# punch-mission/regularizepsf

Measured on AMD Instinct MI355X. Metric: corrected Mpixels/sec + fraction of HBM roofline, 4096^2 image / 256-patch, higher is better.
Workload: dtype f32; 1 GPU; 4096x4096 starfield, 256x256 patches, 1089 patches (whole image on one GPU), coma PSF grid -> Gaussian target, alpha=3 eps=0.1, pad symmetric; patch=256, patches=1089, device= (gfx950:sramecc+:xnack-), compute_units=256, resident=image, output and packed transfer kernel in HBM before the timed region, in_flight=1, frames_in_rotation=1, sync=none (one rank)

## Files before the change

### __graft_entry__.py

```python

from __future__ import annotations

import pathlib
import shutil
import subprocess
import sys

ROOT = pathlib.Path(__file__).resolve().parent
sys.path.insert(0, str(ROOT))


def build() -> None:
    from regularizepsf_amd import build as hip_build

    hip_build.build()
    cores = [ROOT / "regularizepsf_amd" / "csrc" / n for n in ("rpsf_core.hpp", "rpsf_core2.hpp", "rpsf_core3.hpp", "rpsf_plan3.hpp", "rpsf_lattice.hpp", "rpsf_core_builder.hpp", "rpsf_core_builder_sub.hpp", "rpsf_core_builder_wide.hpp", "rpsf_core_cleanup.hpp", "rpsf_core_cleanup_wide.hpp", "rpsf_core_stars.hpp", "rpsf_core_stars_deblend.hpp", "rpsf_core_stars_shape.hpp", "rpsf_core_stars_photometry.hpp", "rpsf_core_stars_refine.hpp", "rpsf_core_stars_fit.hpp", "rpsf_core_stars_fit_weighted.hpp", "rpsf_core_stars_fitpos.hpp", "rpsf_core_stars_render.hpp", "rpsf_core_stars_mesh.hpp", "rpsf_core_saturation.hpp", "rpsf_core_saturation_batch.hpp", "rpsf_core_convert.hpp", "rpsf_core_scale.hpp")]
    for stem in ("emu", "emu2", "emu3", "emu_lattice", "emu_builder", "emu_builder_sub", "emu_builder_wide", "emu_cleanup_wide", "emu_stars", "emu_deblend", "emu_shapes", "emu_photometry", "emu_refine", "emu_fit", "emu_fit_weighted", "emu_fitpos", "emu_render", "emu_stars_mesh", "emu_cleanup", "emu_saturation", "emu_saturation_batch", "emu_mask", "emu_convert", "emu_scale"):
        emu_src = ROOT / "tests" / "emu" / f"{stem}.cpp"
        emu_out = ROOT / "tests" / "emu" / f"lib{stem}.so"
        if not emu_out.exists() or emu_out.stat().st_mtime < max(emu_src.stat().st_mtime, *(c.stat().st_mtime for c in cores)):
            clang = "/opt/rocm/lib/llvm/bin/clang++"
            if not pathlib.Path(clang).exists():
                clang = shutil.which("clang++") or shutil.which("hipcc")
            subprocess.run([clang, "-std=c++20", "-O1", "-shared", "-fPIC", "-o", str(emu_out), str(emu_src)], check=True)
    import regularizepsf_amd
    from regularizepsf_amd import _native

    _native.lib()


def smoke() -> None:
    import numpy as np

    import regularizepsf_amd as rp
    from oracle import regpsf_oracle as orc

    for h, w, n in ((512, 512, 256), (512, 512, 32)):
        coords, k = orc.synthetic_transfer(h, w, n, alpha=3.0, epsilon=0.1)
        image = orc.starfield(h, w, seed=7)
        out = rp.ArrayPSFTransform(rp.IndexedCube(coords, k)).apply(image)
        ref = orc.apply_transfer(image, coords, k)
        d = out - ref
        rel_max = float(np.abs(d).max() / np.abs(ref).max())
        rel_l2 = float(np.linalg.norm(d) / np.linalg.norm(ref))
        print(f"smoke: {h}x{w}/N={n}, {len(coords)} patches: max|d|/max|ref| = {rel_max:.3e}, rel-L2 = {rel_l2:.3e}")
        if not (rel_max <= 1e-5 and rel_l2 <= 1e-5):
            msg = "smoke parity failed"
            raise AssertionError(msg)


if __name__ == "__main__":
    build()
    if "--smoke" in sys.argv:
        smoke()
```

### include/rpsf.h

```cpp
#ifndef RPSF_H
#define RPSF_H

#include <stddef.h>
#include <stdint.h>

#ifdef __cplusplus
extern "C" {
#endif

#define RPSF_OK 0
#define RPSF_E_BADARG (-1)
#define RPSF_E_UNSUPPORTED (-2)
#define RPSF_E_HIP (-3)
#define RPSF_E_NOMEM (-4)
#define RPSF_E_RCCL (-5)
#define RPSF_E_STATE (-6)

#define RPSF_PAD_CONSTANT 0
#define RPSF_PAD_SYMMETRIC 1
#define RPSF_PAD_REFLECT 2
#define RPSF_PAD_EDGE 3
#define RPSF_PAD_WRAP 4

typedef struct rpsf_plan rpsf_plan;

const char* rpsf_last_error(void);
int rpsf_device_count(int* count);
int rpsf_device_info(int device, int* compute_units, char* name, size_t name_len);

int rpsf_plan_create(rpsf_plan** out, int device, int patch_size, int n_patches, const int32_t* coords_rc);
void rpsf_plan_destroy(rpsf_plan* plan);

int rpsf_plan_set_transfer(rpsf_plan* plan, const float* k_c64_host);
int rpsf_plan_set_transfer_device(rpsf_plan* plan, const void* k_c64_device);
int rpsf_plan_set_transfer_spectra_device(rpsf_plan* plan, const void* s_c64_dev, const void* t_c64_dev, double alpha, double epsilon);
int rpsf_plan_set_overlap_mode(rpsf_plan* plan, int mode);
int rpsf_plan_set_sweep_regions(rpsf_plan* plan, int target_regions);
enum {
  RPSF_OPT_PERSIST = 1,
  RPSF_OPT_FUSE = 2,
  RPSF_OPT_K_CACHED = 3,
  RPSF_OPT_PLANE_NT = 4,
  RPSF_OPT_HOST_BANDS = 5,
  RPSF_OPT_STREAM_GROUP = 6,
  RPSF_OPT_STREAM_DEPTH = 7,
  RPSF_OPT_DEBUG_ORPHAN = 8,
  RPSF_OPT_HEAD_KPREFETCH = 9,
  RPSF_OPT_SAT_GROUP = 10
};
int rpsf_plan_set_option(rpsf_plan* plan, int option, int value);
int rpsf_plan_sweep_info(const rpsf_plan* plan, int* regions, long* jobs, long* patch_slots, int* slabs_per_phase);
int rpsf_plan_host_bands(const rpsf_plan* plan, int* bands);
int rpsf_plan_set_stagger(rpsf_plan* plan, int microseconds);
int rpsf_plan_set_reserved_cus(rpsf_plan* plan, int cus);
int rpsf_plan_set_cu_mask(rpsf_plan* plan, const uint32_t* mask, int words);
int rpsf_stream_create(int device, const uint32_t* mask, int words, void** stream);
int rpsf_stream_destroy(void* stream);
int rpsf_plan_set_image_prefetch(rpsf_plan* plan, int on);
int rpsf_plan_debug_stamps(rpsf_plan* plan, unsigned long long* host, size_t count);
int rpsf_plan_transfer_bytes(const rpsf_plan* plan, size_t* bytes);

typedef struct rpsf_geometry {
  int height, width;
  int pad_mode;
  float pad_value;
  int origin_row, origin_col;
  int image_row0, image_rows, ld_image;
  int out_row0, out_rows, ld_out;
} rpsf_geometry;

int rpsf_apply(rpsf_plan* plan, const float* image_host, int height, int width, int pad_mode, float pad_value,
               float* out_host);
int rpsf_apply_host(rpsf_plan* plan, const void* image_host, int image_is_f64, int height, int width, int pad_mode,
                    float pad_value, void* out_host, int out_is_f64);
int rpsf_apply_host_saturated(rpsf_plan* plan, const void* image_host, int image_is_f64, int height, int width, int pad_mode,
                              double threshold, int dilation, int neighborhood_width, void* out_host, int out_is_f64);
int rpsf_apply_frames_host_saturated(rpsf_plan* plan, const void* const* images_host, int image_is_f64, int n_frames, int height,
                                     int width, int pad_mode, double threshold, int dilation, int neighborhood_width,
                                     void* const* outs_host, int out_is_f64);
int rpsf_apply_device_saturated(rpsf_plan* plan, const void* image_dev, void* out_dev, int height, int width, int pad_mode,
                                double threshold, int dilation, int neighborhood_width, void* stream, size_t* n_masked_or_null);
int rpsf_apply_host_saturated_device(rpsf_plan* plan, const void* image_host, int image_is_f64, int height, int width, int pad_mode,
                                     double threshold, int dilation, int neighborhood_width, void* out_host, int out_is_f64);
int rpsf_saturation_kernel_ms(rpsf_plan* plan, double ms[5]);
int rpsf_saturation_fill_device(rpsf_plan* plan, const float* image_host, int height, int width, int pad_mode, double threshold,
                                int dilation, int neighborhood_width, int reverse_groups, float* padded_host, uint8_t* mask_host,
                                int* n_groups_or_null);
int rpsf_apply_batch_device_saturated(rpsf_plan* plan, const void* images_dev, void* outs_dev, int n_frames, size_t image_stride,
                                      size_t out_stride, int height, int width, int pad_mode, double threshold, int dilation,
                                      int neighborhood_width, void* stream, size_t* n_masked_per_frame_or_null);
int rpsf_apply_frames_host_saturated_device(rpsf_plan* plan, const void* const* images_host, int image_is_f64, int n_frames, int height,
                                            int width, int pad_mode, double threshold, int dilation, int neighborhood_width,
                                            void* const* outs_host, int out_is_f64);
int rpsf_saturation_batch_info(rpsf_plan* plan, int info[4]);
int rpsf_saturation_fill_batch_device(rpsf_plan* plan, const float* images_host, int n_frames, int height, int width, int pad_mode,
                                      double threshold, int dilation, int neighborhood_width, int order, float* padded_host,
                                      uint8_t* masks_host, int* groups_per_frame_or_null);
int rpsf_apply_device(rpsf_plan* plan, const void* image_dev, void* out_dev, const rpsf_geometry* geom, void* stream);
int rpsf_apply_device_timed(rpsf_plan* plan, const void* image_dev, void* out_dev, const rpsf_geometry* geom,
                            int iters, float* total_ms, float* kernel_ms);
int rpsf_apply_device_loop_ms(rpsf_plan* plan, const void* image_dev, void* out_dev, const rpsf_geometry* geom, int iters,
// ... 254 lines not shown
```

### regularizepsf_amd/_native.py

```python

from __future__ import annotations

import ctypes
import pathlib
from ctypes import POINTER, c_char_p, c_double, c_float, c_int, c_size_t, c_void_p

import numpy as np

import os

LIB_PATH = pathlib.Path(os.environ.get("RPSF_LIB") or pathlib.Path(__file__).resolve().parent / "librpsf_hip.so")

PAD_MODES = {"constant": 0, "symmetric": 1, "reflect": 2, "edge": 3, "wrap": 4}
SUPPORTED_PATCH_SIZES = (16, 32, 64, 128, 256)

E_BADARG, E_UNSUPPORTED, E_HIP, E_NOMEM, E_RCCL, E_STATE = -1, -2, -3, -4, -5, -6


class NativeError(RuntimeError):

    def __init__(self, code: int, message: str) -> None:
        super().__init__(f"librpsf_hip error {code}: {message}")
        self.code = code

# ... 253 lines not shown
            msg = "upload larger than the device buffer"
            raise ValueError(msg)
        check(lib().rpsf_memcpy_h2d(self.device, c_void_p(self.ptr.value + offset_bytes), _ptr(a), a.nbytes))
        return self

    def download(self, shape, dtype=np.float32, offset_bytes: int = 0) -> np.ndarray:
        out = np.empty(shape, dtype)
        if offset_bytes + out.nbytes > self.nbytes:
            msg = "download larger than the device buffer"
            raise ValueError(msg)
        check(lib().rpsf_memcpy_d2h(self.device, _ptr(out), c_void_p(self.ptr.value + offset_bytes), out.nbytes))
        return out

    def at(self, offset_bytes: int) -> c_void_p:
        return c_void_p(self.ptr.value + offset_bytes)

    def free(self) -> None:
        if self.ptr is not None and self.ptr.value:
            lib().rpsf_dev_free(self.device, self.ptr)
            self.ptr = None

    def __del__(self) -> None:
        try:
            self.free()
        except Exception:
            pass


class Plan:

    def __init__(self, patch_size: int, coordinates, device: int = 0) -> None:
        coords = np.ascontiguousarray(np.asarray(coordinates, dtype=np.int64).reshape(-1, 2).astype(np.int32))
        self.patch_size, self.n_patches, self.device = int(patch_size), len(coords), device
        self._handle = c_void_p()
        check(lib().rpsf_plan_create(ctypes.byref(self._handle), device, self.patch_size, self.n_patches, _ptr(coords)))

    def set_transfer(self, kernel: np.ndarray) -> None:
        k = np.ascontiguousarray(kernel, dtype=np.complex64)
        if k.shape != (self.n_patches, self.patch_size, self.patch_size):
            msg = f"transfer kernel has shape {k.shape}, expected {(self.n_patches, self.patch_size, self.patch_size)}"
            raise ValueError(msg)
        check(lib().rpsf_plan_set_transfer(self._handle, _ptr(k)))

    def set_transfer_device(self, ptr: c_void_p) -> None:
        check(lib().rpsf_plan_set_transfer_device(self._handle, ptr))

    def set_transfer_spectra_device(self, s_ptr: c_void_p, t_ptr: c_void_p, alpha: float, epsilon: float) -> None:
        check(lib().rpsf_plan_set_transfer_spectra_device(self._handle, s_ptr, t_ptr, float(alpha), float(epsilon)))

    def set_overlap_mode(self, mode: str) -> None:
        check(lib().rpsf_plan_set_overlap_mode(self._handle, {"auto": 0, "atomic": 1, "planes": 2, "direct": 3, "sweep": 4}[mode]))

    OPTIONS = {"persist": 1, "fuse": 2, "k_cached": 3, "plane_nt": 4, "host_bands": 5, "stream_group": 6, "stream_depth": 7, "debug_orphan": 8,
               "head_kprefetch": 9, "sat_group": 10}

    def set_option(self, name: str, value: int) -> None:
        check(lib().rpsf_plan_set_option(self._handle, self.OPTIONS[name], int(value)))

    def set_sweep_regions(self, target_regions: int) -> None:
        check(lib().rpsf_plan_set_sweep_regions(self._handle, int(target_regions)))

    def sweep_info(self) -> dict:
        regions, slabs = c_int(0), c_int(0)
        jobs, slots = ctypes.c_long(0), ctypes.c_long(0)
        check(lib().rpsf_plan_sweep_info(self._handle, ctypes.byref(regions), ctypes.byref(jobs), ctypes.byref(slots), ctypes.byref(slabs)))
        return {"regions": regions.value, "jobs": jobs.value, "patch_slots": slots.value, "slabs_per_phase": slabs.value}

    def host_bands(self) -> int:
        n = c_int(0)
        check(lib().rpsf_plan_host_bands(self._handle, ctypes.byref(n)))
        return n.value

    def debug_stamps(self) -> np.ndarray:
        out = np.zeros((self.n_patches, 16), np.uint64)
        check(lib().rpsf_plan_debug_stamps(self._handle, _ptr(out), out.size))
        return out

    def set_stagger(self, microseconds: int) -> None:
        check(lib().rpsf_plan_set_stagger(self._handle, int(microseconds)))

    def set_image_prefetch(self, on: bool) -> None:
        check(lib().rpsf_plan_set_image_prefetch(self._handle, 1 if on else 0))

    def set_reserved_cus(self, cus: int) -> None:
        check(lib().rpsf_plan_set_reserved_cus(self._handle, int(cus)))

    def set_cu_mask(self, mask: np.ndarray) -> None:
        m = np.ascontiguousarray(mask, dtype=np.uint32)
        check(lib().rpsf_plan_set_cu_mask(self._handle, _ptr(m), m.size))

    @property
    def transfer_bytes(self) -> int:
        n = c_size_t(0)
        check(lib().rpsf_plan_transfer_bytes(self._handle, ctypes.byref(n)))
        return n.value

    @property
    def stream(self) -> c_void_p:
        return c_void_p(lib().rpsf_plan_stream(self._handle))

    def apply(self, image: np.ndarray, pad_mode: int, pad_value: float = 0.0) -> np.ndarray:
        img = np.ascontiguousarray(image, dtype=np.float32)
        out = np.empty_like(img)
        check(lib().rpsf_apply(self._handle, _ptr(img), img.shape[0], img.shape[1], pad_mode, pad_value, _ptr(out)))
        return out

    def apply_host(self, image: np.ndarray, pad_mode: int, pad_value: float = 0.0, out_dtype=np.float64,
# ... 573 lines not shown
```

### regularizepsf_amd/csrc/rpsf.hip

```cpp
#include <hip/hip_runtime.h>

#include <dlfcn.h>

#include <algorithm>
#include <cmath>
#include <cstdio>
#include <cstdlib>
#include <cstring>
#include <memory>
#include <mutex>
#include <string>
#include <utility>
#include <vector>

#include "rpsf_plan.hpp"
#include "rpsf_kernels_plan.hpp"

static thread_local std::string g_err;
int rpsf_detail_fail(int code, const std::string& msg) {
  g_err = msg;
  return code;
}

extern "C" const char* rpsf_last_error(void) { return g_err.c_str(); }

template <class F>
static int dispatch_v3(int N, F&& f) {
  switch (N) {
    case 64: return f.template operator()<Cfg3_64>();
    case 32: return f.template operator()<Cfg3_32>();
    case 16: return f.template operator()<Cfg3_16>();
    default: return fail(RPSF_E_UNSUPPORTED, "no third-generation plan for this patch size");
  }
}
static bool has_v3(int N) { return sweep_patch_size(N); }

static int build_sweep_lists(rpsf_plan* p, int target_regions) {
  const int nli = p->nti - 1, nlj = p->ntj - 1;
  Plan3 plan;
  const bool built = dispatch_v3(p->N, [&]<class C>() -> int {
    return plan3_build(C::N, C::KSMAX, C::WAVES, nli, nlj, p->sweep.slot.data(), p->sweep.par_j, target_regions, plan) ? RPSF_OK : RPSF_E_STATE;
  }) == RPSF_OK;
  if (!built) return RPSF_OK;
  SweepPath& sw = p->sweep;
  sw.ok = false;
  HIP_TRY(sw.d_jobs.upload(plan.jobs.data(), plan.jobs.size()));
  HIP_TRY(sw.d_regions.upload(plan.regions.data(), plan.regions.size()));
  if (!sw.d_zero) {
    HIP_TRY(sw.d_zero.alloc(16));
    HIP_TRY(hipMemset(sw.d_zero, 0, 64));
  }
  if (!p->parent && !sw.err) {
    HIP_TRY(hipHostMalloc(reinterpret_cast<void**>(&sw.err.p), 64, hipHostMallocMapped));
    std::memset(sw.err, 0, 64);
    HIP_TRY(hipHostGetDevicePointer(reinterpret_cast<void**>(&sw.d_err), sw.err, 0));
  }
  p->sweep.n_regions = (int)plan.regions.size(), p->sweep.ks = plan.ks, p->sweep.slabs = plan.slabs, p->sweep.patch_slots = plan.patch_slots;
  p->sweep.ok = true;
#if defined(RPSF3_STAMPS) || defined(RPSF3_DUMP)
  HIP_TRY(p->sweep.d_stamps.alloc((size_t)std::max(512, p->sweep.n_regions) * 8 * 8 * 16));
  HIP_TRY(hipMemset(p->sweep.d_stamps, 0, (size_t)std::max(512, p->sweep.n_regions) * 8 * 8 * 16 * sizeof(unsigned long long)));
#endif
  return RPSF_OK;
}

static int setup_lattice(rpsf_plan* p) {
  LatticeKnobs knobs;
  if (const char* e = dev_env("RPSF_STRIPS")) knobs.strips = std::max(1, std::atoi(e));
  if (const char* e = dev_env("RPSF_ORDER_MEET")) knobs.meet = std::atoi(e) != 0;
  if (dev_env("RPSF_NO_RIM_FIRST")) knobs.rim_first = false;
  if (const char* e = dev_env("RPSF_RIM_LAST")) knobs.rim_last = std::atoi(e) != 0;
  const LatticeParent parent = p->parent ? LatticeParent{p->parent->lat_r0, p->parent->lat_c0, p->parent->lattice} : LatticeParent{};
  LatticeTables t = lattice_build(p->N, p->n_patches, p->h_coords.data(), p->k_index.empty() ? nullptr : p->k_index.data(), p->patch.v2,
                                  p->parent ? &parent : nullptr, knobs);
  const size_t n = (size_t)p->n_patches;
  p->lattice = t.lattice, p->patch.direct_ok = t.direct_ok;
  p->h_order = std::move(t.order);
  static_assert(sizeof(PatchDesc) == sizeof(int4) && sizeof(QuadWords) == sizeof(uint4), "uploaded as they are");
  HIP_TRY(p->d_desc.upload(reinterpret_cast<const int4*>(t.desc.data()), n));
  if (!t.lattice) return RPSF_OK;
  p->lat_r0 = t.r0, p->lat_c0 = t.c0, p->nti = t.nti, p->ntj = t.ntj;
  if (!t.sweep_slot.empty()) {
    p->sweep.slot = std::move(t.sweep_slot);
    p->sweep.par_j = t.par_j;
    const int rc3 = build_sweep_lists(p, std::max(8, p->cu_count));
    if (rc3 != RPSF_OK) return rc3;
  }
  HIP_TRY(p->d_cover.upload(t.cover.data(), t.cover.size()));
  if (p->patch.v2) {
    HIP_TRY(p->patch.d_sum_order.upload(t.sum_order.data(), t.sum_order.size()));
    HIP_TRY(p->patch.d_tile_done.alloc(t.sum_order.size()));
    HIP_TRY(hipMemset(p->patch.d_tile_done, 0, t.sum_order.size() * sizeof(uint32_t)));
    HIP_TRY(p->patch.d_sum_queue.alloc(1));
    HIP_TRY(hipMemset(p->patch.d_sum_queue, 0, sizeof(uint32_t)));
    HIP_TRY(p->patch.d_xq.alloc(8 * 32));
    HIP_TRY(hipMemset(p->patch.d_xq, 0, 8 * 32 * sizeof(uint32_t)));
    std::copy_n(t.prefetch_first, 9, p->patch.prefetch_first);
    HIP_TRY(p->patch.d_prefetch_tiles.alloc(std::max<size_t>(1, t.prefetch_tiles.size())));
    HIP_TRY(hipMemcpy(p->patch.d_prefetch_tiles, t.prefetch_tiles.data(), t.prefetch_tiles.size() * sizeof(uint32_t), hipMemcpyHostToDevice));
  }
  if (p->patch.direct_ok) {
    HIP_TRY(p->patch.d_quads.upload(reinterpret_cast<const uint4*>(t.quads.data()), n));
    HIP_TRY(p->patch.d_tile_info.upload(t.tile_info.data(), t.tile_info.size()));
    HIP_TRY(p->patch.d_chunk_xcc.alloc(8));
    HIP_TRY(hipMemset(p->patch.d_chunk_xcc, 0, 8 * sizeof(uint32_t)));
  }
  return RPSF_OK;
}

template <class F>
static int dispatch_patch(bool v2, int N, F&& f) {
  if (!v2) return dispatch_n(N, [&]<class C>() -> int { return f.template operator()<PatchPlan<C, false>>(); });
  switch (N) {
    case 256: return f.template operator()<PatchPlan<Cfg256v2, true>>();
    case 128: return f.template operator()<PatchPlan<Cfg128v2, true>>();
    default: return fail(RPSF_E_UNSUPPORTED, "no second-generation plan for this patch size");
  }
}
static bool has_v2(int N) { return (N == 256 || N == 128) && !dev_env("RPSF_V1"); }

extern "C" int rpsf_device_count(int* count) {
  if (!count) return fail(RPSF_E_BADARG, "count is null");
  HIP_TRY(hipGetDeviceCount(count));
  return RPSF_OK;
}

extern "C" int rpsf_device_info(int device, int* compute_units, char* name, size_t name_len) {
  hipDeviceProp_t prop;
  HIP_TRY(hipGetDeviceProperties(&prop, device));
  if (compute_units) *compute_units = prop.multiProcessorCount;
  if (name && name_len) {
    std::snprintf(name, name_len, "%s (%s)", prop.name, prop.gcnArchName);
  }
  return RPSF_OK;
}


static bool generic_colours(int N, const int32_t* coords_rc, int n, std::vector<uint8_t>& colours) {
  int res[2][2], nres[2] = {0, 0};
  colours.assign((size_t)n, 0);
  std::vector<std::pair<int32_t, int32_t>> seen((size_t)n);
  for (int i = 0; i < n; ++i) {
    seen[(size_t)i] = {coords_rc[2 * i], coords_rc[2 * i + 1]};
    for (int axis = 0; axis < 2; ++axis) {
      const int r = ((coords_rc[2 * i + axis] % N) + N) % N;
      int cls = -1;
      for (int k = 0; k < nres[axis]; ++k)
        if (res[axis][k] == r) cls = k;
      if (cls < 0) {
// ... 105 lines not shown
    }
    {
      hipDeviceProp_t prop;
      HIP_TRY(hipGetDeviceProperties(&prop, device));
      p->cu_count = prop.multiProcessorCount;
    }
    HIP_TRY(p->d_coords.upload(coords_rc, 2 * (size_t)n_patches));
    p->h_coords.assign(coords_rc, coords_rc + 2 * (size_t)n_patches);
    set_corner_extremes(p);
    HIP_TRY(p->patch.d_sink.alloc(128));
#if defined(RPSF_STAMPS)
#if defined(RPSF_WAVE_STAMPS)
    constexpr size_t STAMP_WAVES = 8;
#else
    constexpr size_t STAMP_WAVES = 1;
#endif
    HIP_TRY(p->patch.d_stamps.alloc(16 * STAMP_WAVES * (size_t)n_patches));
    HIP_TRY(hipMemset(p->patch.d_stamps, 0, sizeof(unsigned long long) * 16 * STAMP_WAVES * (size_t)n_patches));
#endif
    p->patch.v2 = has_v2(N);
    p->patch.sum_first = -1;
    if (const char* e = dev_env("RPSF_SUM_FIRST")) p->patch.sum_first = std::max(0, std::atoi(e)) / 8 * 8;
    if (const char* e = dev_env("RPSF_HEAD_PATCHES")) p->patch.head_patches = std::atoi(e) > 0 ? 1 : 0;
    if (const char* e = dev_env("RPSF_PREFETCH")) p->patch.prefetch = std::atoi(e) != 0;
    if (const char* e = dev_env("RPSF_STAGGER_US")) p->patch.stagger_us = std::max(0, std::atoi(e));
    if (const char* e = dev_env("RPSF_RESERVED_CUS")) p->patch.reserved_cus = std::min(128, std::max(0, std::atoi(e)));
    p->patch.fuse_pays = N >= 128 || dev_env("RPSF_FUSE_ALWAYS") != nullptr;
    p->patch.persist = N == 256 || N == 128;
    if (p->patch.persist) {
      if (N == 256)
        HIP_TRY(hipFuncSetAttribute(reinterpret_cast<const void*>(&patch_kernel2_256p), hipFuncAttributeMaxDynamicSharedMemorySize,
                                    (int)Launch2<Cfg256v2>::LDS_BYTES));
      else {
        HIP_TRY(hipFuncSetAttribute(reinterpret_cast<const void*>(&patch_kernel2_128p), hipFuncAttributeMaxDynamicSharedMemorySize,
                                    (int)Launch2<Cfg128v2>::LDS_BYTES));
        HIP_TRY(hipFuncSetAttribute(reinterpret_cast<const void*>(&patch_kernel2_128pc), hipFuncAttributeMaxDynamicSharedMemorySize,
                                    (int)Launch2<Cfg128v2>::LDS_BYTES));
        HIP_TRY(hipFuncSetAttribute(reinterpret_cast<const void*>(&patch_kernel2_128pcs), hipFuncAttributeMaxDynamicSharedMemorySize,
                                    (int)Launch2<Cfg128v2>::LDS_BYTES));
        p->patch.k_cached = (size_t)(parent ? parent->n_patches : n_patches) * Cfg128v2::G_PER_PATCH * sizeof(cf) <= ((size_t)96 << 20);
      }
    }
    int rl = dispatch_patch(p->patch.v2, N, [&]<class T>() -> int {
      HIP_TRY(hipFuncSetAttribute(reinterpret_cast<const void*>(T::kernel()), hipFuncAttributeMaxDynamicSharedMemorySize, (int)T::LDS_BYTES));
      int per_cu = 0;
      HIP_TRY(hipOccupancyMaxActiveBlocksPerMultiprocessor(&per_cu, T::kernel(), T::WG, T::LDS_BYTES));
      p->patch.round_capacity = p->cu_count * std::max(1, per_cu) * T::TEAMS;
      return RPSF_OK;
    });
    if (rl != RPSF_OK) return rl;
    HIP_TRY(hipEventCreateWithFlags(&p->ev_busy, hipEventDisableTiming));
    rl = setup_lattice(p);
    if (rl != RPSF_OK) return rl;
    if (p->sweep.ok) {
      rl = dispatch_v3(N, [&]<class C>() -> int {
        HIP_TRY(hipFuncSetAttribute(reinterpret_cast<const void*>(&sweep_kernel<C>), hipFuncAttributeMaxDynamicSharedMemorySize, (int)C::LDS_BYTES));
        HIP_TRY(hipFuncSetAttribute(reinterpret_cast<const void*>(&sweep_kernel_kc<C>), hipFuncAttributeMaxDynamicSharedMemorySize, (int)C::LDS_BYTES));
        if (!parent) {
          p->sweep.k3_floats = (size_t)C::K_FLOATS * n_patches;
          HIP_TRY(p->sweep.d_k3.alloc(p->sweep.k3_floats));
        }
        return RPSF_OK;
      });
      if (rl != RPSF_OK) return rl;
      if (parent && !parent->sweep.d_k3) p->sweep.ok = false;
    }
    if (parent) {
      p->have_k = parent->have_k;
      p->overlap_mode = parent->overlap_mode, p->patch.stagger_us = parent->patch.stagger_us, p->patch.k_prefetch = parent->patch.k_prefetch;
      return RPSF_OK;
    }
    return dispatch_patch(p->patch.v2, N, [&]<class T>() -> int {
      int r2 = upload_tables<T>(device, p->patch.d_tab, p->patch.d_tw, &p->d_win, &p->patch.d_pairtab);
      if (r2 != RPSF_OK) return r2;
      p->patch.g_elems = (size_t)T::Cfg::G_PER_PATCH * n_patches;
      p->patch.gs_elems = (size_t)T::Cfg::GS_PER_PATCH * n_patches;
      HIP_TRY(p->patch.d_g.alloc(p->patch.g_elems));
      HIP_TRY(p->patch.d_gs.alloc(p->patch.gs_elems + 1));
      return RPSF_OK;
    });
  };
  const int rc = body();
  if (rc != RPSF_OK) {
    std::string keep = g_err;
    delete p;
    g_err = keep;
    return rc;
  }
  *out = p;
  return RPSF_OK;
}

extern "C" int rpsf_plan_create(rpsf_plan** out, int device, int patch_size, int n_patches, const int32_t* coords_rc) {
  return rpsf_detail_plan_create_impl(out, device, patch_size, n_patches, coords_rc, nullptr, nullptr);
}

extern "C" void* rpsf_plan_stream(rpsf_plan* p) { return p ? (void*)p->stream : nullptr; }

extern "C" void rpsf_plan_destroy(rpsf_plan* p) { delete p; }

void rpsf_detail_drop_bands(rpsf_plan* p) {
  p->bands.clear(), p->band_rows.clear(), p->band_in_rows.clear();
  p->bands_h = p->bands_w = 0, p->bands_mode = -1, p->bands_want = -1;
}

struct KSource {
  const cf* k = nullptr;
  hipMemcpyKind k_kind = hipMemcpyDeviceToDevice;
  const cf *s = nullptr, *t = nullptr;
  double alpha = 0.0, epsilon = 0.0;
};

static int install_transfer(rpsf_plan* p, const KSource& src, int first, int count) {
  if (p->parent) return fail(RPSF_E_STATE, "a view shares its parent's transfer kernel");
  const size_t at = (size_t)first * p->N * p->N;
  const cf *k = src.k, *s = src.s, *t = src.t;
  const float alpha = (float)src.alpha, epsilon = (float)src.epsilon;
  auto grid = [](size_t total) { return dim3((unsigned)((total + 255) / 256)); };
  int rc = RPSF_OK;
  if (p->generic) {
    const size_t elems = (size_t)p->N * p->N * count;
    if (k) HIP_TRY(hipMemcpy(p->fft.d_kfull + at, k, elems * sizeof(cf), src.k_kind));
    else rc = rpsf_build_transfer_device(p->device, elems, s, t, 0, src.alpha, src.epsilon, p->fft.d_kfull + at, p->stream);
  } else {
    if (p->sweep.d_k3)
      rc = dispatch_v3(p->N, [&]<class C>() -> int {
        cf* k3 = reinterpret_cast<cf*>(p->sweep.d_k3 + (size_t)first * C::K_FLOATS);
        const dim3 g = grid((size_t)(C::K_FLOATS / 2) * count);
        if (k) pack_kernel3<C><<<g, dim3(256), 0, p->stream>>>(k, count, k3);
        else pack_spectra_kernel3<C><<<g, dim3(256), 0, p->stream>>>(s, t, alpha, epsilon, count, k3);
        HIP_TRY(hipGetLastError());
        return RPSF_OK;
      });
    if (rc == RPSF_OK)
      rc = dispatch_patch(p->patch.v2, p->N, [&]<class T>() -> int {
        using C = typename T::Cfg;
        cf *g = p->patch.d_g + (size_t)first * C::G_PER_PATCH, *gs = p->patch.d_gs + (size_t)first * C::GS_PER_PATCH;
        const dim3 gr = grid(T::PACK_PER_PATCH * count);
        if (k) T::pack()<<<gr, dim3(256), 0, p->stream>>>(k, count, p->patch.d_tab, p->patch.d_pairtab, g, gs);
        else T::pack_spectra()<<<gr, dim3(256), 0, p->stream>>>(s, t, alpha, epsilon, count, p->patch.d_tab, p->patch.d_pairtab, g, gs);
        HIP_TRY(hipGetLastError());
        return RPSF_OK;
      });
  }
  if (rc != RPSF_OK) return rc;
  HIP_TRY(hipStreamSynchronize(p->stream));
  if (first + count == p->n_patches) {
    p->have_k = true;
    for (auto& band : p->bands) band->have_k = true;
  }
  return RPSF_OK;
}

extern "C" int rpsf_plan_set_transfer(rpsf_plan* p, const float* k_host) {
  if (!p || !k_host) return fail(RPSF_E_BADARG, "null argument");
  HIP_TRY(hipSetDevice(p->device));
  const cf* k = reinterpret_cast<const cf*>(k_host);
  if (p->generic) return install_transfer(p, KSource{k, hipMemcpyHostToDevice}, 0, p->n_patches);
  const size_t per = (size_t)p->N * p->N;
  const int chunk = std::min(p->n_patches, (int)std::max<size_t>(1, (size_t)(64u << 20) / (per * sizeof(cf))));
  DevBuf<cf> d_tmp;
  HIP_TRY(d_tmp.alloc(per * chunk));
  for (int first = 0; first < p->n_patches; first += chunk) {
    const int cnt = std::min(chunk, p->n_patches - first);
    HIP_TRY(hipMemcpyAsync(d_tmp, k + (size_t)first * per, per * sizeof(cf) * cnt, hipMemcpyHostToDevice, p->stream));
    const int rc = install_transfer(p, KSource{d_tmp}, first, cnt);
    if (rc != RPSF_OK) return rc;
  }
  return RPSF_OK;
}

extern "C" int rpsf_plan_set_transfer_device(rpsf_plan* p, const void* k_dev) {
  if (!p || !k_dev) return fail(RPSF_E_BADARG, "null argument");
  HIP_TRY(hipSetDevice(p->device));
  return install_transfer(p, KSource{reinterpret_cast<const cf*>(k_dev)}, 0, p->n_patches);
}

extern "C" int rpsf_plan_set_transfer_spectra_device(rpsf_plan* p, const void* s_c64_dev, const void* t_c64_dev, double alpha, double epsilon) {
  if (!p || !s_c64_dev || !t_c64_dev) return fail(RPSF_E_BADARG, "null argument");
  HIP_TRY(hipSetDevice(p->device));
  return install_transfer(p, KSource{nullptr, hipMemcpyDeviceToDevice, reinterpret_cast<const cf*>(s_c64_dev), reinterpret_cast<const cf*>(t_c64_dev),
                                     alpha, epsilon}, 0, p->n_patches);
}

extern "C" int rpsf_plan_transfer_bytes(const rpsf_plan* p, size_t* bytes) {
  if (!p || !bytes) return fail(RPSF_E_BADARG, "null argument");
  if (p->generic) *bytes = (size_t)p->N * p->N * p->n_patches * sizeof(cf);
  else if (p->sweep.ok && rpsf_detail_overlap_kind(p) == OV_SWEEP) *bytes = p->sweep.k3_floats * sizeof(float);
  else *bytes = (p->patch.g_elems + p->patch.gs_elems) * sizeof(cf);
  return RPSF_OK;
}

int rpsf_detail_check_geometry(const rpsf_plan* p, const rpsf_geometry* g) {
  if (!g) return fail(RPSF_E_BADARG, "geometry is null");
  if (g->height <= 0 || g->width <= 0) return fail(RPSF_E_BADARG, "image shape must be positive");
  if (g->pad_mode < 0 || g->pad_mode > RPSF_PAD_WRAP) return fail(RPSF_E_BADARG, "unknown pad mode");
  if (g->ld_image < g->width || g->ld_out < g->width) return fail(RPSF_E_BADARG, "row stride smaller than the image width");
  if (g->image_row0 < 0 || g->image_rows <= 0 || g->image_row0 + g->image_rows > g->height || g->out_row0 < 0 ||
      g->out_rows <= 0 || g->out_row0 + g->out_rows > g->height)
    return fail(RPSF_E_BADARG, "resident row window lies outside the image");
  const int N = p->N;
  const long rlo = (long)p->corner_min[0] + g->origin_row, rhi = (long)p->corner_max[0] + g->origin_row;
  const long clo = (long)p->corner_min[1] + g->origin_col, chi = (long)p->corner_max[1] + g->origin_col;
  if (rlo < -2L * N || rhi > (long)g->height + N || clo < -2L * N || chi > (long)g->width + N) {
    for (int i = 0; i < p->n_patches; ++i) {
      long r = (long)p->h_coords[2 * i] + g->origin_row, c = (long)p->h_coords[2 * i + 1] + g->origin_col;
      if (r < -2L * N || r > (long)g->height + N || c < -2L * N || c > (long)g->width + N)
        return fail(RPSF_E_BADARG, "patch corner (" + std::to_string(r) + ", " + std::to_string(c) +
                                       ") lies outside the 2N-padded image");
    }
  }
  return RPSF_OK;
}

bool rpsf_detail_lattice_covers_window(const rpsf_plan* p, const rpsf_geometry& g) {
  return lattice_covers_window(p->N, p->lat_r0, p->lat_c0, p->nti, p->ntj, g);
}

static int clear_window(float* d_out, const rpsf_geometry& g, Batch b, hipStream_t st) {
  for (int f = 0; f < b.frames; ++f)
    HIP_TRY(hipMemset2DAsync(d_out + (size_t)f * b.out_stride, (size_t)g.ld_out * sizeof(float), 0, (size_t)g.width * sizeof(float), g.out_rows, st));
  return RPSF_OK;
}

template <class F>
static void for_frame_slices(int frames, F&& launch) {
  for (int f0 = 0; f0 < frames; f0 += 65535) launch(f0, (unsigned)std::min(65535, frames - f0));
}

template <class P>
static void fill_plane_sum(P& s, const rpsf_plan* p, float* d_out, const rpsf_geometry& g, Batch b) {
  s.planes = p->patch.d_planes, s.plane_stride = p->patch.planes_floats, s.planes_frame_floats = 4 * p->patch.planes_floats, s.ld_planes = g.width;
  s.out = d_out, s.ld_out = g.ld_out, s.out_frame_floats = b.out_stride;
  s.rows = g.out_rows, s.W = g.width, s.row0 = g.out_row0;
  s.lat_r0 = p->lat_r0 + g.origin_row, s.lat_c0 = p->lat_c0 + g.origin_col, s.ntj = p->ntj;
}

static int sum_first_for(const rpsf_plan* p, int frames) {
  if (p->patch.sum_first >= 0) return p->patch.sum_first;
  const long work = (long)p->n_patches * frames;
  if (p->N == 128) return work >= 4096 ? 160 : work >= 2048 ? 128 : work >= 512 ? 8 : 0;
  return work >= 2048 ? 32 : work >= 1024 ? 16 : work >= 512 ? 8 : 0;
}

static bool hot_geometry(const rpsf_plan* p, const float* d_img, const rpsf_geometry& g, size_t im_stride) {
  const bool aligned16 = im_stride % 4 == 0 && (reinterpret_cast<uintptr_t>(d_img) & 15) == 0 && p->patch.planes_floats % 4 == 0;
  return hot_geometry(g, p->lattice, p->lat_c0, aligned16);
}

struct PatchLaunch {
  enum Form { GEN1, GEN2, FUSED, PERSISTENT } form;
  enum Variant { PLAIN, K_CACHED, K_CACHED_PLANES_NT } variant;
  unsigned grid;
  int chunk;
  int patch_blocks;
  int stagger_ticks, stagger_blocks;
  int sum_first, frame_major, plane_nt;
  int rows, head_patches, prefetch;
  int k_prefetch;
  uint32_t xq_base[8], xq_draws[8];
  uint32_t sum_queue_base, sum_queue_draws;
};

static bool patch_launch_too_large(const rpsf_plan* p, int frames) {
  const int teams = patch_teams(p->N);
  return (size_t)8 * (chunk_patches(p->n_patches, teams) / teams) * frames > 0x7fffffffu;
}

template <class T>
static PatchLaunch patch_launch_for(const rpsf_plan* p, const float* d_img, const rpsf_geometry& g, Batch b, bool fused) {
  constexpr bool N256 = T::V2 && T::Cfg::N == 256, N128 = T::V2 && T::Cfg::N == 128;
  PatchLaunch L{};
  L.chunk = chunk_patches(p->n_patches, T::TEAMS);
  L.stagger_ticks = std::max(0, p->patch.stagger_us) * 100;
  L.grid = (unsigned)((size_t)8 * (L.chunk / T::TEAMS) * b.frames);
  L.form = T::V2 ? PatchLaunch::GEN2 : PatchLaunch::GEN1;
  L.stagger_blocks = T::V2 ? p->patch.round_capacity : p->cu_count * std::max(1, 512 / T::WG);
  L.patch_blocks = T::V2 ? (int)L.grid : 0;
  if (!fused) return L;
  const int count = p->nti * p->ntj * b.frames;
  bool frame_major = N256 && p->patch.persist && b.frames > 1 && p->n_patches >= 1024 &&
                     16.0 * (double)p->patch.planes_floats * b.frames > 256.0 * 1048576.0;
  if (const char* e = dev_env("RPSF_FRAME_MAJOR"))
    frame_major = std::atoi(e) == 2 ? (p->patch.persist && b.frames > 1) : (frame_major && std::atoi(e) != 0);
  L.frame_major = frame_major ? 1 : 0;
  L.plane_nt = N128 && p->patch.k_cached && b.frames > 1 && !frame_major && 16.0 * (double)p->patch.planes_floats * b.frames > 300.0 * 1048576.0;
  if (p->patch.plane_nt_opt >= 0) L.plane_nt = p->patch.plane_nt_opt != 0 && N128 && p->patch.k_cached;
  const int tune_frames = b.frames;
  L.sum_first = sum_first_for(p, tune_frames);
  L.sum_queue_base = p->patch.sum_queue_base;
  const int rows = std::min(L.chunk * b.frames, std::max(1, (p->patch.round_capacity - L.sum_first - p->patch.reserved_cus) / 8));
  if (!(p->patch.persist && rows > 0 && hot_geometry(p, d_img, g, b.im_stride))) {
    L.form = PatchLaunch::FUSED;
    const int nsum = std::max(8, std::min(count, p->patch.round_capacity)) + L.sum_first;
    L.sum_queue_draws = (uint32_t)(count + nsum);
    L.grid += (unsigned)nsum;
    return L;
  }
  L.form = PatchLaunch::PERSISTENT, L.rows = rows;
  L.variant = !p->patch.k_cached ? PatchLaunch::PLAIN : L.plane_nt ? PatchLaunch::K_CACHED_PLANES_NT : PatchLaunch::K_CACHED;
  L.head_patches = p->patch.head_patches;
  L.prefetch = p->patch.prefetch && p->patch.d_prefetch_tiles ? 1 : 0;
  L.k_prefetch = N256 && !L.head_patches ? p->patch.k_prefetch : 0;
  if (p->patch.stagger_us < 0 && (long)p->n_patches * tune_frames >= 256) {
    const long work = (long)p->n_patches * tune_frames;
    L.stagger_ticks = work >= 2048 ? 2400 : (work >= 1024 && N256) ? 1600 : 1200;
    if (N128) L.stagger_ticks = tune_frames == 1 && p->n_patches >= 4096 ? 600 : 0;
  }
  for (int x = 0; x < 8; ++x) {
    L.xq_base[x] = p->patch.xq_base[x];
    const int slots_x = std::min(L.chunk, std::max(0, p->n_patches - x * L.chunk)) * b.frames;
    L.xq_draws[x] = (uint32_t)(std::max(0, slots_x - (L.head_patches ? L.sum_first / 8 : 0)) + rows);
  }
  const int wgs = L.sum_first + 8 * rows;
  L.sum_queue_draws = (uint32_t)(count + wgs);
  L.grid = (unsigned)wgs;
  return L;
}

static PatchParams patch_params(const rpsf_plan* p, const PatchLaunch& L, const float* d_img, float* d_out, const rpsf_geometry& g, OverlapKind kind,
                                Batch b) {
  PatchParams pp{};
  pp.im = ImageView{d_img, g.height, g.width, g.ld_image, g.pad_mode, g.pad_value, g.image_row0, g.image_rows};
  if (kind != OV_ATOMIC)
    pp.ov = OutView{p->patch.d_planes, g.height, g.width, g.width, g.out_row0, g.out_rows, p->patch.planes_floats, p->patch.d_sink};
  else
    pp.ov = OutView{d_out, g.height, g.width, g.ld_out, g.out_row0, g.out_rows, 0, p->patch.d_sink};
  pp.origin_row = g.origin_row, pp.origin_col = g.origin_col;
  pp.desc = p->d_desc, pp.n_patches = p->n_patches, pp.seq_base = 0;
  const rpsf_plan* o = owner(p);
  pp.tab = o->patch.d_tab, pp.pairtab = o->patch.d_pairtab, pp.tw = o->patch.d_tw, pp.win = o->d_win, pp.g = o->patch.d_g, pp.gs = o->patch.d_gs;
  pp.stamps = p->patch.d_stamps;
  pp.chunk = L.chunk, pp.slot0 = 0, pp.patch_blocks = L.patch_blocks;
  pp.stagger_ticks = L.stagger_ticks, pp.stagger_blocks = L.stagger_blocks;
  pp.n_frames = b.frames, pp.im_frame_floats = b.im_stride;
  pp.ov_frame_floats = kind != OV_ATOMIC ? 4 * p->patch.planes_floats : b.out_stride;
  pp.dv = OutView{nullptr, 0, 0, 0, 0, 0, 0, nullptr};
  if (kind == OV_DIRECT) {
    pp.dv = OutView{d_out, g.height, g.width, g.ld_out, g.out_row0, g.out_rows, 0, p->patch.d_sink};
    pp.dv_frame_floats = b.out_stride;
    pp.quads = p->patch.d_quads, pp.flags = p->patch.d_flags, pp.dyn_side = p->patch.d_dyn, pp.chunk_xcc = p->patch.d_chunk_xcc;
    pp.flag_epoch = p->patch.epoch, pp.n_tiles = (uint32_t)(p->nti * p->ntj), pp.orphan_mod = p->patch.orphan_mod;
  }
  if (L.form != PatchLaunch::FUSED && L.form != PatchLaunch::PERSISTENT) return pp;
  const int n_tiles = p->nti * p->ntj;
  pp.tile_done = p->patch.d_tile_done, pp.quads = p->patch.d_quads, pp.n_tiles = (uint32_t)n_tiles;
  pp.sum_first = L.sum_first, pp.frame_major = L.frame_major, pp.plane_nt = L.plane_nt;
  TileSum& ts = pp.ts;
  fill_plane_sum(ts, p, d_out, g, b);
  ts.half = p->N / 2, ts.cover = p->d_cover, ts.tiles = p->patch.d_sum_order, ts.count = n_tiles * b.frames;
  ts.done = p->patch.d_tile_done, ts.epoch = p->patch.done_epoch;
  ts.n_frames = b.frames, ts.n_tiles = (uint32_t)n_tiles, ts.n_tiles_listed = (uint32_t)n_tiles, ts.frame_major = L.frame_major;
  ts.queue = p->patch.d_sum_queue, ts.queue_base = L.sum_queue_base;
  if (L.form != PatchLaunch::PERSISTENT) return pp;
  pp.persist = L.rows, pp.xq = p->patch.d_xq;
  pp.head_patches = L.head_patches, pp.prefetch = L.prefetch, pp.prefetch_tiles = p->patch.d_prefetch_tiles;
  pp.k_prefetch = L.k_prefetch, pp.k_patches = o->n_patches;
  for (int x = 0; x < 9; ++x) pp.prefetch_first[x] = p->patch.prefetch_first[x];
  for (int x = 0; x < 8; ++x) pp.xq_base[x] = L.xq_base[x];
  return pp;
}

static int launch_patches(const rpsf_plan* p, const PatchLaunch& L, const float* d_img, float* d_out, const rpsf_geometry& g, OverlapKind kind,
                          hipStream_t st, Batch b) {
  const PatchParams pp = patch_params(p, L, d_img, d_out, g, kind, b);
  return dispatch_patch(p->patch.v2, p->N, [&]<class T>() -> int {
    const dim3 grid(L.grid), wg(T::WG);
    if (L.form != PatchLaunch::PERSISTENT) T::kernel()<<<grid, wg, T::LDS_BYTES, st>>>(pp);
    else if constexpr (T::V2) {
      using Persistent = PersistentKernel2<typename T::Cfg>;
      switch (L.variant) {
        case PatchLaunch::PLAIN: Persistent::fn<<<grid, wg, T::LDS_BYTES, st>>>(pp); break;
        case PatchLaunch::K_CACHED: Persistent::fn_k_cached<<<grid, wg, T::LDS_BYTES, st>>>(pp); break;
        case PatchLaunch::K_CACHED_PLANES_NT: Persistent::fn_k_cached_planes_nt<<<grid, wg, T::LDS_BYTES, st>>>(pp); break;
      }
    }
    HIP_TRY(hipGetLastError());
    return RPSF_OK;
  });
}

static int launch_fixup(const rpsf_plan* p, float* d_out, const rpsf_geometry& g, hipStream_t st, Batch b) {
  FixParams fp{};
  fill_plane_sum(fp, p, d_out, g, b);
  fp.half = p->N / 2;
  fp.tile_info = p->patch.d_tile_info, fp.flags = p->patch.d_flags, fp.dyn_side = p->patch.d_dyn;
  fp.epoch = p->patch.epoch, fp.n_tiles = (uint32_t)(p->nti * p->ntj);
  for_frame_slices(b.frames, [&](int f0, unsigned frames) {
    FixParams q = fp;
    q.planes += (size_t)f0 * q.planes_frame_floats, q.out += (size_t)f0 * q.out_frame_floats;
    q.flags += (size_t)f0 * q.n_tiles, q.dyn_side += (size_t)f0 * q.n_tiles;
    fixup_kernel<<<dim3(fp.n_tiles * FIX_SUB, frames), dim3(256), 0, st>>>(q);
  });
  HIP_TRY(hipGetLastError());
  return RPSF_OK;
}

static int launch_sum(const rpsf_plan* p, float* d_out, const rpsf_geometry& g, hipStream_t st, Batch b) {
  SumParams sp{};
  fill_plane_sum(sp, p, d_out, g, b);
  sp.row_begin = 0, sp.nti = p->nti, sp.cover = p->d_cover;
  sp.half_shift = 0;
  while ((1 << (sp.half_shift + 1)) < p->N) ++sp.half_shift;
  const size_t total = (size_t)((g.width + 3) / 4) * sp.rows;
  for_frame_slices(b.frames, [&](int f0, unsigned frames) {
    SumParams q = sp;
    q.planes += (size_t)f0 * q.planes_frame_floats, q.out += (size_t)f0 * q.out_frame_floats;
    sum_planes_kernel<<<dim3((unsigned)((total + 255) / 256), frames), dim3(256), 0, st>>>(q);
// ... 41 lines not shown
      generic_multiply_kernel<<<dim3(grid), dim3(256), 0, st>>>(p->fft.d_buf, p->fft.d_kfull + (size_t)first * per, total, scale);
      if (g_hipfft.exec_c2c(p->fft.plan.get(), p->fft.d_buf, p->fft.d_buf,  1) != 0)
        return fail(RPSF_E_HIP, "hipfftExecC2C (inverse) failed");
      if (p->fft.d_colour && rpsf_detail_overlap_kind(p) != OV_ATOMIC) {
        for (int colour = 0; colour < 4; ++colour)
          generic_scatter_kernel<<<dim3(grid), dim3(256), 0, st>>>(gg, p->d_coords, p->fft.d_win, p->fft.d_buf, p->fft.d_colour, colour);
      } else {
        generic_scatter_kernel<<<dim3(grid), dim3(256), 0, st>>>(gg, p->d_coords, p->fft.d_win, p->fft.d_buf, nullptr, -1);
      }
      HIP_TRY(hipGetLastError());
    }
  }
  if (ev_k1) HIP_TRY(hipEventRecord(ev_k1, st));
  if (st != p->stream) {
    HIP_TRY(hipStreamSynchronize(st));
    if (g_hipfft.set_stream(p->fft.plan.get(), p->stream) != 0) return fail(RPSF_E_HIP, "hipfftSetStream failed");
  }
  return RPSF_OK;
}

static int launch_sweep(rpsf_plan* p, const float* d_img, float* d_out, const rpsf_geometry& g, hipStream_t st, hipEvent_t ev_k0, hipEvent_t ev_k1,
                        Batch b) {
  const long r0 = (long)p->lat_r0 + g.origin_row, c0 = (long)p->lat_c0 + g.origin_col;
  if (const int rc = rpsf_detail_lattice_covers_window(p, g) ? RPSF_OK : clear_window(d_out, g, b, st); rc != RPSF_OK) return rc;
  SweepParams sp{};
  sp.im = ImageView{d_img, g.height, g.width, g.ld_image, g.pad_mode, g.pad_value, g.image_row0, g.image_rows};
  const bool col_aligned = (c0 & 3) == 0;
  sp.aligned_in = col_aligned && g.ld_image % 4 == 0 && b.im_stride % 4 == 0 && (reinterpret_cast<uintptr_t>(d_img) & 15) == 0;
  const int aligned_out = col_aligned && g.ld_out % 4 == 0 && b.out_stride % 4 == 0 && (reinterpret_cast<uintptr_t>(d_out) & 15) == 0;
  sp.fl = Flush3{d_out, g.ld_out, g.out_row0, g.out_rows, g.height, g.width, aligned_out};
  sp.lat_r0 = (int)r0, sp.lat_c0 = (int)c0;
  sp.jobs = p->sweep.d_jobs, sp.regions = p->sweep.d_regions, sp.n_regions = p->sweep.n_regions, sp.group = (p->sweep.n_regions + 7) / 8;
  const rpsf_plan* o = owner(p);
  sp.k3 = o->sweep.d_k3, sp.win = o->d_win, sp.zeros = p->sweep.d_zero, sp.err = o->sweep.d_err, sp.stamps = p->sweep.d_stamps;
  sp.im_frame_floats = b.im_stride, sp.out_frame_floats = b.out_stride;
  const bool k_plain = b.frames > 1 || o->sweep.k3_floats * sizeof(float) <= ((size_t)96 << 20);
  if (ev_k0) HIP_TRY(hipEventRecord(ev_k0, st));
  for_frame_slices(b.frames, [&](int f0, unsigned frames) {
    SweepParams q = sp;
    q.im.img += (size_t)f0 * b.im_stride, q.fl.out += (size_t)f0 * b.out_stride;
    const dim3 grid((unsigned)(8 * sp.group), frames);
    (void)dispatch_v3(p->N, [&]<class C>() -> int {
      if (k_plain) sweep_kernel_kc<C><<<grid, dim3(C::WG), C::LDS_BYTES, st>>>(q);
      else sweep_kernel<C><<<grid, dim3(C::WG), C::LDS_BYTES, st>>>(q);
      return RPSF_OK;
    });
  });
  HIP_TRY(hipGetLastError());
  if (ev_k1) HIP_TRY(hipEventRecord(ev_k1, st));
  return RPSF_OK;
}

int rpsf_detail_launch_apply(rpsf_plan* p, const float* d_img, float* d_out, const rpsf_geometry& g, hipStream_t st,
                             hipEvent_t ev_k0, hipEvent_t ev_k1, Batch b) {
  if (p->generic) return launch_apply_generic(p, d_img, d_out, g, st, ev_k0, ev_k1, b);
  const OverlapKind kind = rpsf_detail_overlap_kind(p);
  if (kind == OV_SWEEP) {
    if (!p->sweep.ok) return fail(RPSF_E_STATE, "the sweep kernel needs a 16-, 32- or 64-pixel patch on a complete lattice of at least 2 x 2 patches");
    return launch_sweep(p, d_img, d_out, g, st, ev_k0, ev_k1, b);
  }
  if (kind != OV_ATOMIC && !p->lattice) return fail(RPSF_E_STATE, "colour planes need a regular half-overlap lattice of patch corners");
  if (kind == OV_DIRECT && !p->patch.direct_ok) return fail(RPSF_E_STATE, "direct overlap-add needs a lattice and a 128- or 256-pixel patch");
  if (kind == OV_DIRECT && (size_t)g.out_rows * g.ld_out * sizeof(float) >= ((size_t)1 << 32))
    return fail(RPSF_E_UNSUPPORTED, "direct overlap-add addresses the output through a 32-bit buffer offset: frame too large");
  if (patch_launch_too_large(p, b.frames)) return fail(RPSF_E_BADARG, "batch too large for one launch");
  const bool fused = kind == OV_PLANES && p->patch.v2 && p->patch.fuse_pays && p->patch.d_tile_done && !p->patch.no_fuse && b.frames <= 255 &&
                     fused_geometry(g, p->lat_c0, (reinterpret_cast<uintptr_t>(d_out) & 15) == 0);
  const size_t n_tiles = (size_t)p->nti * p->ntj;
  if (p->busy_valid && st != p->last_stream) {
    if (p->multi_stream) HIP_TRY(hipStreamWaitEvent(st, p->ev_busy, 0));
    else {
      HIP_TRY(hipDeviceSynchronize());
      p->multi_stream = true;
    }
  }
  if (kind != OV_ATOMIC) {
    const size_t need = plane_floats_needed(g);
    if (need > p->patch.planes_floats || (size_t)b.frames > p->patch.planes_frames) {
      const size_t per = std::max(need, p->patch.planes_floats), frames = std::max((size_t)b.frames, p->patch.planes_frames);
      HIP_TRY(hipDeviceSynchronize());
      p->patch.planes_floats = 0, p->patch.planes_frames = 0;
      HIP_TRY(p->patch.d_planes.alloc(4 * per * frames));
      p->patch.planes_floats = per, p->patch.planes_frames = frames;
    }
  }
  if (kind == OV_DIRECT && (size_t)b.frames > p->patch.flag_frames) {
    HIP_TRY(hipDeviceSynchronize());
    p->patch.d_flags.reset(), p->patch.d_dyn.reset(), p->patch.flag_frames = 0;
    HIP_TRY(p->patch.d_flags.alloc(n_tiles * b.frames));
    HIP_TRY(p->patch.d_dyn.alloc(n_tiles * b.frames));
    HIP_TRY(hipMemset(p->patch.d_flags, 0, n_tiles * b.frames * sizeof(uint32_t)));
    HIP_TRY(hipMemset(p->patch.d_dyn, 0, n_tiles * b.frames * sizeof(uint32_t)));
    p->patch.flag_frames = (size_t)b.frames;
  }
  if (fused && (size_t)b.frames > p->patch.done_frames) {
    HIP_TRY(hipDeviceSynchronize());
    HIP_TRY(p->patch.d_tile_done.alloc(n_tiles * b.frames));
    HIP_TRY(hipMemset(p->patch.d_tile_done, 0, n_tiles * b.frames * sizeof(uint32_t)));
    p->patch.done_frames = (size_t)b.frames;
  }
  PatchLaunch L{};
  (void)dispatch_patch(p->patch.v2, p->N, [&]<class T>() -> int {
    L = patch_launch_for<T>(p, d_img, g, b, fused);
    return RPSF_OK;
  });
  if (kind == OV_DIRECT && ++p->patch.epoch >= (1u << 24) - 1) {
    HIP_TRY(hipMemsetAsync(p->patch.d_flags, 0, n_tiles * p->patch.flag_frames * sizeof(uint32_t), st));
    HIP_TRY(hipMemsetAsync(p->patch.d_chunk_xcc, 0, 8 * sizeof(uint32_t), st));
    p->patch.epoch = 1;
  }
  if (fused) {
    const bool restart = b.frames != p->patch.done_last_frames || p->patch.done_epoch + 1 >= (1u << 29);
    if (restart) HIP_TRY(hipMemsetAsync(p->patch.d_tile_done, 0, n_tiles * p->patch.done_frames * sizeof(uint32_t), st));
    p->patch.done_last_frames = b.frames;
    p->patch.done_epoch = restart ? 1 : p->patch.done_epoch + 1;
  }
  for (int x = 0; x < 8; ++x) p->patch.xq_base[x] += L.xq_draws[x];
  p->patch.sum_queue_base += L.sum_queue_draws;
  const bool clear = kind == OV_ATOMIC || ((kind == OV_DIRECT || fused) && !rpsf_detail_lattice_covers_window(p, g));
  if (const int rc = clear ? clear_window(d_out, g, b, st) : RPSF_OK; rc != RPSF_OK) return rc;
  if (ev_k0) HIP_TRY(hipEventRecord(ev_k0, st));
  int rc = launch_patches(p, L, d_img, d_out, g, kind, st, b);
  if (rc != RPSF_OK) return rc;
  if (ev_k1) HIP_TRY(hipEventRecord(ev_k1, st));
  if (kind == OV_PLANES && !fused) rc = launch_sum(p, d_out, g, st, b);
  if (kind == OV_DIRECT) rc = launch_fixup(p, d_out, g, st, b);
  if (rc != RPSF_OK) return rc;
  if (p->multi_stream) HIP_TRY(hipEventRecord(p->ev_busy, st));
  p->last_stream = st, p->busy_valid = true;
  return RPSF_OK;
}

extern "C" int rpsf_plan_set_overlap_mode(rpsf_plan* p, int mode) {
  if (!p || mode < 0 || mode > 4) return fail(RPSF_E_BADARG, "mode must be 0 (auto), 1 (atomics), 2 (colour planes), 3 (direct) or 4 (sweep)");
  if (mode == 4 && !p->sweep.ok) return fail(RPSF_E_STATE, "the sweep kernel needs a 16-, 32- or 64-pixel patch on a complete lattice of at least 2 x 2 patches");
  if (mode == 2 && !p->lattice) return fail(RPSF_E_STATE, "colour planes need a regular half-overlap lattice of patch corners");
  if (mode == 3 && !p->patch.direct_ok) return fail(RPSF_E_STATE, "direct overlap-add needs a regular half-overlap lattice and a 128- or 256-pixel patch");
  p->overlap_mode = mode;
  rpsf_detail_drop_bands(p);
  return RPSF_OK;
}

extern "C" int rpsf_plan_set_option(rpsf_plan* p, int option, int value) {
  if (!p) return fail(RPSF_E_BADARG, "null plan");
  switch (option) {
    case RPSF_OPT_PERSIST:
      if (value != 0 && value != 1) return fail(RPSF_E_BADARG, "RPSF_OPT_PERSIST takes 0 or 1");
      p->patch.persist = value != 0 && (p->N == 256 || p->N == 128);
      break;
    case RPSF_OPT_FUSE:
      if (value != 0 && value != 1) return fail(RPSF_E_BADARG, "RPSF_OPT_FUSE takes 0 or 1");
      p->patch.no_fuse = value == 0;
      break;
    case RPSF_OPT_K_CACHED:
      if (value != 0 && value != 1) return fail(RPSF_E_BADARG, "RPSF_OPT_K_CACHED takes 0 or 1");
      p->patch.k_cached = value != 0;
      break;
    case RPSF_OPT_PLANE_NT:
      if (value < -1 || value > 1) return fail(RPSF_E_BADARG, "RPSF_OPT_PLANE_NT takes -1 (automatic), 0 or 1");
      p->patch.plane_nt_opt = value;
      break;
    case RPSF_OPT_HOST_BANDS:
      if (value < -1 || value > 64) return fail(RPSF_E_BADARG, "RPSF_OPT_HOST_BANDS takes -1 (automatic) or 0..64");
      p->host_bands_opt = value;
      break;
    case RPSF_OPT_STREAM_GROUP:
      if (value < 0 || value > 64) return fail(RPSF_E_BADARG, "RPSF_OPT_STREAM_GROUP takes 0 (automatic) or 1..64");
      p->stream_group_opt = value;
      break;
    case RPSF_OPT_STREAM_DEPTH:
      if (value < 0 || value > 16) return fail(RPSF_E_BADARG, "RPSF_OPT_STREAM_DEPTH takes 0 (automatic) or 1..16");
      p->stream_depth_opt = value;
      break;
    case RPSF_OPT_HEAD_KPREFETCH:
      if (value != 0 && value != 1) return fail(RPSF_E_BADARG, "RPSF_OPT_HEAD_KPREFETCH takes 0 or 1");
      p->patch.k_prefetch = p->N == 256 ? value : 0;
      break;
    case RPSF_OPT_SAT_GROUP:
      if (value < 0 || value > 65535) return fail(RPSF_E_BADARG, "RPSF_OPT_SAT_GROUP takes 0 (automatic) or 1..65535");
      p->sat_group_opt = value;
      return RPSF_OK;
    case RPSF_OPT_DEBUG_ORPHAN:
      if (value < 0) return fail(RPSF_E_BADARG, "RPSF_OPT_DEBUG_ORPHAN takes 0 (off) or a positive modulus");
      p->patch.orphan_mod = value;
      break;
    default: return fail(RPSF_E_BADARG, "unknown plan option");
  }
  rpsf_detail_drop_bands(p);
  return RPSF_OK;
}

extern "C" int rpsf_plan_set_sweep_regions(rpsf_plan* p, int target_regions) {
  if (!p || target_regions < 1 || target_regions > (1 << 20)) return fail(RPSF_E_BADARG, "target_regions must be 1..2^20");
  if (!p->sweep.ok) return fail(RPSF_E_STATE, "the sweep kernel needs a 16-, 32- or 64-pixel patch on a complete lattice of at least 2 x 2 patches");
  HIP_TRY(hipSetDevice(p->device));
  HIP_TRY(hipStreamSynchronize(p->stream));
  HIP_TRY(hipDeviceSynchronize());
  rpsf_detail_drop_bands(p);
  return build_sweep_lists(p, target_regions);
}
extern "C" int rpsf_plan_host_bands(const rpsf_plan* p, int* bands) {
  if (!p || !bands) return fail(RPSF_E_BADARG, "null argument");
  *bands = p->last_host_bands;
  return RPSF_OK;
}
extern "C" int rpsf_plan_sweep_info(const rpsf_plan* p, int* regions, long* jobs, long* patch_slots, int* slabs_per_phase) {
  if (!p) return fail(RPSF_E_BADARG, "null plan");
  if (regions) *regions = p->sweep.ok ? p->sweep.n_regions : 0;
  if (jobs) *jobs = p->sweep.ok ? p->sweep.slabs : 0;
  if (patch_slots) *patch_slots = p->sweep.ok ? p->sweep.patch_slots : 0;
  if (slabs_per_phase) *slabs_per_phase = p->sweep.ok ? p->sweep.ks : 0;
  return RPSF_OK;
}

extern "C" int rpsf_plan_debug_stamps(rpsf_plan* p, unsigned long long* host, size_t count) {
  if (!p || !host) return fail(RPSF_E_BADARG, "null argument");
  if (p->sweep.d_stamps) {
    HIP_TRY(hipSetDevice(p->device));
    HIP_TRY(hipDeviceSynchronize());
    count = std::min(count, (size_t)std::max(512, p->sweep.n_regions) * 8 * 8 * 16);
    HIP_TRY(hipMemcpy(host, p->sweep.d_stamps, count * sizeof(unsigned long long), hipMemcpyDeviceToHost));
    return RPSF_OK;
  }
  if (!p->patch.d_stamps) return fail(RPSF_E_STATE, "phase timestamps exist only in builds with -DRPSF_STAMPS");
  HIP_TRY(hipSetDevice(p->device));
  HIP_TRY(hipDeviceSynchronize());
#if defined(RPSF_WAVE_STAMPS)
  count = std::min(count, (size_t)16 * 8 * p->n_patches);
#else
  count = std::min(count, (size_t)16 * p->n_patches);
#endif
  HIP_TRY(hipMemcpy(host, p->patch.d_stamps, count * sizeof(unsigned long long), hipMemcpyDeviceToHost));
  return RPSF_OK;
}


extern "C" int rpsf_plan_set_reserved_cus(rpsf_plan* p, int cus) {
  if (!p || cus < 0 || cus > 128) return fail(RPSF_E_BADARG, "reserved CUs must be 0..128");
  p->patch.reserved_cus = cus;
  return RPSF_OK;
}

extern "C" int rpsf_plan_set_cu_mask(rpsf_plan* p, const uint32_t* mask, int words) {
  if (!p || !mask || words <= 0) return fail(RPSF_E_BADARG, "bad argument");
  if (p->parent) return fail(RPSF_E_STATE, "a view runs on its parent's stream");
  int cus = 0;
  for (int i = 0; i < words; ++i) cus += __builtin_popcount(mask[i]);
  if (cus < 8) return fail(RPSF_E_BADARG, "the mask must leave the plan at least 8 compute units");
  HIP_TRY(hipSetDevice(p->device));
  HIP_TRY(hipStreamSynchronize(p->stream));
  rpsf_detail_drop_bands(p);
  hipStream_t masked = nullptr;
  HIP_TRY(hipExtStreamCreateWithCUMask(&masked, (uint32_t)words, mask));
  if (p->generic && g_hipfft.set_stream(p->fft.plan.get(), masked) != 0) {
    (void)hipStreamDestroy(masked);
    return fail(RPSF_E_HIP, "hipfftSetStream failed");
  }
  (void)hipStreamDestroy(p->stream);
  p->stream = masked;
  p->busy_valid = false;
  if (p->cu_count > 0) p->patch.round_capacity = p->patch.round_capacity / p->cu_count * cus;
  p->cu_count = cus;
  return RPSF_OK;
}

extern "C" int rpsf_stream_create(int device, const uint32_t* mask, int words, void** stream) {
  if (!stream) return fail(RPSF_E_BADARG, "null argument");
  HIP_TRY(hipSetDevice(device));
  hipStream_t st = nullptr;
  if (mask && words > 0)
    HIP_TRY(hipExtStreamCreateWithCUMask(&st, (uint32_t)words, mask));
  else
    HIP_TRY(hipStreamCreateWithFlags(&st, hipStreamNonBlocking));
  *stream = st;
  return RPSF_OK;
}
extern "C" int rpsf_stream_destroy(void* stream) {
  if (stream) HIP_TRY(hipStreamDestroy(reinterpret_cast<hipStream_t>(stream)));
  return RPSF_OK;
}

extern "C" int rpsf_plan_set_image_prefetch(rpsf_plan* p, int on) {
  if (!p) return fail(RPSF_E_BADARG, "null plan");
  p->patch.prefetch = on != 0;
  return RPSF_OK;
}

extern "C" int rpsf_plan_set_stagger(rpsf_plan* p, int microseconds) {
  if (!p || microseconds < 0 || microseconds > 1000) return fail(RPSF_E_BADARG, "stagger must be 0..1000 us");
  p->patch.stagger_us = microseconds;
  rpsf_detail_drop_bands(p);
  return RPSF_OK;
}


extern "C" int rpsf_apply_device(rpsf_plan* p, const void* image_dev, void* out_dev, const rpsf_geometry* geom,
                                 void* stream) {
  if (!p || !image_dev || !out_dev) return fail(RPSF_E_BADARG, "null argument");
  if (!p->have_k) return fail(RPSF_E_STATE, "no transfer kernel installed (call rpsf_plan_set_transfer first)");
  int rc = rpsf_detail_check_geometry(p, geom);
  if (rc != RPSF_OK) return rc;
  HIP_TRY(hipSetDevice(p->device));
  hipStream_t st = stream ? reinterpret_cast<hipStream_t>(stream) : p->stream;
  return rpsf_detail_launch_apply(p, reinterpret_cast<const float*>(image_dev), reinterpret_cast<float*>(out_dev), *geom, st, nullptr);
}


static int batch_group_frames(const rpsf_plan* p, const rpsf_geometry& g, int n_frames) {
  if (n_frames == 1 || p->generic || rpsf_detail_overlap_kind(p) == OV_ATOMIC || rpsf_detail_overlap_kind(p) == OV_SWEEP) return n_frames;
  size_t free_b = 0, total_b = 0;
  if (hipMemGetInfo(&free_b, &total_b) != hipSuccess) total_b = (size_t)64 << 30;
  const size_t per_frame = 16 * plane_floats_needed(g);
  return (int)std::max<size_t>(1, std::min<size_t>((size_t)n_frames, (total_b / 4) / per_frame));
}

static int check_batch(rpsf_plan* p, const void* a, const void* b, int n_frames, size_t im_stride, size_t out_stride,
                       const rpsf_geometry* geom) {
  if (!p || !a || !b) return fail(RPSF_E_BADARG, "null argument");
  if (n_frames <= 0) return fail(RPSF_E_BADARG, "n_frames must be positive");
  if (!p->have_k) return fail(RPSF_E_STATE, "no transfer kernel installed (call rpsf_plan_set_transfer first)");
  int rc = rpsf_detail_check_geometry(p, geom);
  if (rc != RPSF_OK) return rc;
  if (n_frames > 1 && (im_stride < (size_t)(geom->image_rows - 1) * geom->ld_image + geom->width ||
                       out_stride < (size_t)(geom->out_rows - 1) * geom->ld_out + geom->width))
    return fail(RPSF_E_BADARG, "frame stride smaller than one frame");
  return RPSF_OK;
}

int rpsf_detail_launch_batch(rpsf_plan* p, const float* d_imgs, float* d_outs, int n_frames, size_t im_stride, size_t out_stride,
                             const rpsf_geometry& g, hipStream_t st, hipEvent_t ev_k0, hipEvent_t ev_k1) {
  const int group = batch_group_frames(p, g, n_frames);
  for (int f0 = 0; f0 < n_frames; f0 += group) {
    Batch b;
    b.frames = std::min(group, n_frames - f0), b.im_stride = im_stride, b.out_stride = out_stride;
    const bool first = f0 == 0, last = f0 + group >= n_frames;
    int rc = rpsf_detail_launch_apply(p, d_imgs + (size_t)f0 * im_stride, d_outs + (size_t)f0 * out_stride, g, st,
                          first ? ev_k0 : nullptr, last ? ev_k1 : nullptr, b);
    if (rc != RPSF_OK) return rc;
  }
  return RPSF_OK;
}

extern "C" int rpsf_apply_batch_device(rpsf_plan* p, const void* images_dev, void* outs_dev, int n_frames,
                                       size_t image_stride, size_t out_stride, const rpsf_geometry* geom, void* stream) {
  int rc = check_batch(p, images_dev, outs_dev, n_frames, image_stride, out_stride, geom);
  if (rc != RPSF_OK) return rc;
  HIP_TRY(hipSetDevice(p->device));
  hipStream_t st = stream ? reinterpret_cast<hipStream_t>(stream) : p->stream;
  return rpsf_detail_launch_batch(p, reinterpret_cast<const float*>(images_dev), reinterpret_cast<float*>(outs_dev), n_frames,
                      image_stride, out_stride, *geom, st);
}

template <class Launch>
static int timed_loop(rpsf_plan* p, int iters, float* total_ms, float* kernel_ms, Launch&& launch) {
  std::vector<hipEvent_t> ev((size_t)4 * iters, nullptr);
  auto cleanup = [&] {
    for (auto e : ev)
      if (e) (void)hipEventDestroy(e);
  };
  int rc = RPSF_OK;
  hipError_t err = hipSuccess;
  for (auto& e : ev)
    if (err == hipSuccess) err = hipEventCreate(&e);
  for (int i = 0; i < iters && err == hipSuccess && rc == RPSF_OK; ++i) {
    err = hipEventRecord(ev[4 * i], p->stream);
    if (err == hipSuccess) rc = launch(ev[4 * i + 1], ev[4 * i + 2]);
    if (err == hipSuccess && rc == RPSF_OK) err = hipEventRecord(ev[4 * i + 3], p->stream);
  }
  if (err == hipSuccess && rc == RPSF_OK) err = hipStreamSynchronize(p->stream);
  for (int i = 0; i < iters && err == hipSuccess && rc == RPSF_OK; ++i) {
    float ms = 0.f;
    if (total_ms) {
      err = hipEventElapsedTime(&ms, ev[4 * i], ev[4 * i + 3]);
      total_ms[i] = ms;
    }
    if (kernel_ms && err == hipSuccess) {
      err = hipEventElapsedTime(&ms, ev[4 * i + 1], ev[4 * i + 2]);
      kernel_ms[i] = ms;
    }
  }
  if (err != hipSuccess || rc != RPSF_OK) (void)hipStreamSynchronize(p->stream);
  cleanup();
  if (rc != RPSF_OK) return rc;
  if (err != hipSuccess) return fail(RPSF_E_HIP, std::string("timed applies: ") + hipGetErrorString(err));
  return RPSF_OK;
}

extern "C" int rpsf_apply_batch_device_timed(rpsf_plan* p, const void* images_dev, void* outs_dev, int n_frames,
                                             size_t image_stride, size_t out_stride, const rpsf_geometry* geom, int iters,
                                             float* total_ms, float* kernel_ms) {
  if (iters <= 0) return fail(RPSF_E_BADARG, "bad argument");
  int rc = check_batch(p, images_dev, outs_dev, n_frames, image_stride, out_stride, geom);
  if (rc != RPSF_OK) return rc;
  HIP_TRY(hipSetDevice(p->device));
  return timed_loop(p, iters, total_ms, kernel_ms, [&](hipEvent_t k0, hipEvent_t k1) {
    return rpsf_detail_launch_batch(p, reinterpret_cast<const float*>(images_dev), reinterpret_cast<float*>(outs_dev), n_frames, image_stride,
                        out_stride, *geom, p->stream, k0, k1);
  });
}

int rpsf_detail_sweep_check(rpsf_plan* p) {
  volatile uint32_t* word = owner(p)->sweep.err;
  if (!word || *word == 0) return RPSF_OK;
  *word = 0;
  return fail(RPSF_E_HIP, "sweep kernel: a job waited for the jobs it follows beyond the bound (internal protocol error; the output of this apply is not valid)");
}

int rpsf_detail_drain_after_error(rpsf_plan* p, hipError_t err, const char* where) {
  (void)hipStreamSynchronize(p->pipe->st_in);
  (void)hipStreamSynchronize(p->stream);
  (void)hipStreamSynchronize(p->pipe->st_out);
  if (err == hipErrorUnknown && !g_err.empty()) return RPSF_E_HIP;
  return fail(RPSF_E_HIP, std::string(where) + ": " + hipGetErrorString(err));
}

extern "C" int rpsf_apply_device_timed(rpsf_plan* p, const void* image_dev, void* out_dev, const rpsf_geometry* geom,
                                       int iters, float* total_ms, float* kernel_ms) {
  if (!p || !image_dev || !out_dev || iters <= 0) return fail(RPSF_E_BADARG, "bad argument");
  if (!p->have_k) return fail(RPSF_E_STATE, "no transfer kernel installed (call rpsf_plan_set_transfer first)");
  int rc = rpsf_detail_check_geometry(p, geom);
  if (rc != RPSF_OK) return rc;
  HIP_TRY(hipSetDevice(p->device));
  return timed_loop(p, iters, total_ms, kernel_ms, [&](hipEvent_t k0, hipEvent_t k1) {
    return rpsf_detail_launch_apply(p, reinterpret_cast<const float*>(image_dev), reinterpret_cast<float*>(out_dev), *geom, p->stream, k0, k1);
  });
}

extern "C" int rpsf_apply_device_loop_ms(rpsf_plan* p, const void* image_dev, void* out_dev, const rpsf_geometry* geom, int iters,
                                         double* ms_per_apply) {
  if (!p || !image_dev || !out_dev || iters <= 0 || !ms_per_apply) return fail(RPSF_E_BADARG, "bad argument");
  if (!p->have_k) return fail(RPSF_E_STATE, "no transfer kernel installed (call rpsf_plan_set_transfer first)");
  int rc = rpsf_detail_check_geometry(p, geom);
  if (rc != RPSF_OK) return rc;
  HIP_TRY(hipSetDevice(p->device));
  HIP_TRY(hipEventRecord(p->ev[0], p->stream));
  for (int i = 0; i < iters; ++i) {
    rc = rpsf_detail_launch_apply(p, reinterpret_cast<const float*>(image_dev), reinterpret_cast<float*>(out_dev), *geom, p->stream, nullptr);
    if (rc != RPSF_OK) return rc;
  }
  HIP_TRY(hipEventRecord(p->ev[3], p->stream));
  HIP_TRY(hipEventSynchronize(p->ev[3]));
  float ms = 0.f;
  HIP_TRY(hipEventElapsedTime(&ms, p->ev[0], p->ev[3]));
  *ms_per_apply = (double)ms / iters;
  return rpsf_detail_sweep_check(p);
}
```

### regularizepsf_amd/csrc/rpsf_device.hpp

```cpp
#pragma once
#include <hip/hip_runtime.h>

#include <string>
#include <type_traits>

#include "../../include/rpsf.h"
#include "rpsf_core.hpp"
#include "rpsf_core2.hpp"
#include "rpsf_core3.hpp"
#include "rpsf_plan3.hpp"

using namespace rpsf;

#include "rpsf_kernels.hpp"
#include "rpsf_kernels2.hpp"
#include "rpsf_kernels3.hpp"

#define RPSF_PLANS_V1(X) X(Cfg256) X(Cfg128) X(Cfg64) X(Cfg32) X(Cfg16)
#define RPSF_PLANS_V2(X) X(Cfg256v2) X(Cfg128v2)
#define RPSF_PLANS_V3(X) X(Cfg3_64) X(Cfg3_32) X(Cfg3_16)
#define RPSF_DECL_V1(C)                                                                                        \
  extern template __global__ void patch_kernel<C>(PatchParams);                                                \
  extern template __global__ void pack_kernel<C>(const cf*, int, const uint16_t*, const uint32_t*, cf*, cf*);  \
  extern template __global__ void pack_spectra_kernel<C>(const cf*, const cf*, float, float, int, const uint16_t*, const uint32_t*, cf*, cf*); \
  extern template __global__ void psf_fft_kernel<C>(const float*, int, const uint16_t*, const cf*, cf*);
#define RPSF_DECL_V2(C)                                           \
  extern template __global__ void patch_kernel2<C>(PatchParams); \
  extern template __global__ void pack_kernel2<C>(const cf*, int, const uint16_t*, const uint32_t*, cf*, cf*); \
  extern template __global__ void pack_spectra_kernel2<C>(const cf*, const cf*, float, float, int, const uint16_t*, const uint32_t*, cf*, cf*);
#define RPSF_INST_V1(C)                                                                                \
  template __global__ void patch_kernel<C>(PatchParams);                                               \
  template __global__ void pack_kernel<C>(const cf*, int, const uint16_t*, const uint32_t*, cf*, cf*); \
  template __global__ void pack_spectra_kernel<C>(const cf*, const cf*, float, float, int, const uint16_t*, const uint32_t*, cf*, cf*); \
  template __global__ void psf_fft_kernel<C>(const float*, int, const uint16_t*, const cf*, cf*);
#define RPSF_INST_V2(C)                                    \
  template __global__ void patch_kernel2<C>(PatchParams); \
  template __global__ void pack_kernel2<C>(const cf*, int, const uint16_t*, const uint32_t*, cf*, cf*); \
  template __global__ void pack_spectra_kernel2<C>(const cf*, const cf*, float, float, int, const uint16_t*, const uint32_t*, cf*, cf*);
#define RPSF_DECL_V3(C)                                                                  \
  extern template __global__ void sweep_kernel<C>(SweepParams);                          \
  extern template __global__ void sweep_kernel_kc<C>(SweepParams);                       \
  extern template __global__ void pack_kernel3<C>(const cf*, int, cf*);                  \
  extern template __global__ void pack_spectra_kernel3<C>(const cf*, const cf*, float, float, int, cf*);
#define RPSF_INST_V3(C)                                                           \
  template __global__ void sweep_kernel<C>(SweepParams);                          \
  template __global__ void sweep_kernel_kc<C>(SweepParams);                       \
  template __global__ void pack_kernel3<C>(const cf*, int, cf*);                  \
  template __global__ void pack_spectra_kernel3<C>(const cf*, const cf*, float, float, int, cf*);
```

### regularizepsf_amd/csrc/rpsf_host.hip

```cpp
#include <hip/hip_runtime.h>

#include <algorithm>
#include <atomic>
#include <cctype>
#include <chrono>
#include <cstdio>
#include <cstdlib>
#include <cstring>
#include <memory>
#include <string>
#include <thread>
#include <utility>
#include <vector>

#include "rpsf_plan.hpp"

using rpsf_host::HostPipe;
using rpsf_host::HostPool;

int rpsf_detail_pipe_ensure(rpsf_plan* p, size_t slot_floats, int depth) {
  if (!p->pipe) p->pipe.reset(new HostPipe);
  HostPipe& q = *p->pipe;
  if (!q.st_in) {
    HIP_TRY(hipStreamCreateWithFlags(&q.st_in, hipStreamNonBlocking));
// ... 138 lines not shown
          gb.out_row0 = R0, gb.out_rows = R1 - R0;
          err = hipEventRecord(q.ev_band_in[b], q.st_in);
          if (err == hipSuccess) err = hipStreamWaitEvent(p->stream, q.ev_band_in[b], 0);
          float* const host_out = direct_out ? static_cast<float*>(out) : q.h_out[0];
          if (err == hipSuccess && rpsf_detail_launch_apply(p->bands[b].get(), q.d_in[0], q.d_out[0] + (size_t)R0 * W, gb, p->stream, nullptr) != RPSF_OK)
            err = hipErrorUnknown;
          if (err == hipSuccess) err = hipEventRecord(q.ev_band_k[b], p->stream);
          const hipStream_t so = q.st_out;
          if (err == hipSuccess) err = hipStreamWaitEvent(so, q.ev_band_k[b], 0);
          const int sub = (b + 1 == B && !direct_out) ? 4 : 1;
          const int rows_per_piece = (R1 - R0 + sub - 1) / sub;
          for (int s0 = R0; s0 < R1 && err == hipSuccess; s0 += rows_per_piece) {
            const size_t plo = (size_t)s0 * W, phi = (size_t)std::min(R1, s0 + rows_per_piece) * W;
            err = hipMemcpyAsync(host_out + plo, q.d_out[0] + plo, (phi - plo) * sizeof(float), hipMemcpyDeviceToHost, so);
            if (err == hipSuccess) err = hipEventRecord(q.ev_chunk[landed.size()], so);
            landed.push_back({plo, phi});
          }
        }
        if (++c == chunks.size()) t_enqueued = ms_since(t_start);
        progress = true;
      }
      if (err == hipSuccess && published < landed.size()) {
        const hipError_t qe = c < chunks.size() ? hipEventQuery(q.ev_chunk[published]) : hipEventSynchronize(q.ev_chunk[published]);
        if (qe == hipSuccess) {
          if (published == 0) t_first_out = ms_since(t_start);
          if (!direct_out && inline_mode) {
            rpsf_host::widen_or_copy(out, out_f64 != 0, q.h_out[0], landed[published].lo, landed[published].hi);
          } else if (!direct_out) {
            for (size_t a = landed[published].lo; a < landed[published].hi; a += PIECE) out_pieces[n_avail++] = {a, std::min(landed[published].hi, a + PIECE)};
            out_avail.store(n_avail, std::memory_order_release);
          }
          ++published, progress = true;
        } else if (qe != hipErrorNotReady) {
          err = qe;
        }
      }
      if (!progress) __builtin_ia32_pause();
    }
    t_last_out = ms_since(t_start);
    closed.store(1, std::memory_order_release);
  };
  if (direct_in && direct_out) conductor();
  else if (inline_mode) {
    for (size_t i = 0; i < n_in; ++i) {
      rpsf_host::narrow_or_copy(q.h_in[0], image, in_f64 != 0, in_pieces[i].lo, in_pieces[i].hi);
      chunk_done[piece_chunk[i]].fetch_add(1, std::memory_order_release);
    }
    conductor();
  } else {
    const int every = frame_every > 0 ? frame_every : (pool.width() >= 16 ? 2 : 1);
    pool.run(std::max(1, (frame_workers > 0 ? std::min(frame_workers, pool.width()) : pool.width()) / every), worker, conductor, every);
  }
  if (trace)
    std::fprintf(stderr, "[rpsf host frame] %zu chunks, %d bands, %zu + %zu pieces: last chunk enqueued %.3f ms, first piece back %.3f, last %.3f, total %.3f ms\\n",
                 chunks.size(), B, n_in, (size_t)out_avail.load(), t_enqueued, t_first_out, t_last_out, ms_since(t_start));
  if (err != hipSuccess) return rpsf_detail_drain_after_error(p, err, "host frame");
  return rpsf_detail_sweep_check(p);
}

static int host_one_frame(rpsf_plan* p, const void* image, int in_f64, void* out, int out_f64, const rpsf_geometry& g) {
  const size_t count = (size_t)g.height * g.width, bytes = count * sizeof(float);
  int rc = rpsf_detail_pipe_ensure(p, count, 1);
  if (rc != RPSF_OK) return rc;
  HostPipe& q = *p->pipe;
  HostPool& pool = HostPool::get(p->device);
  const int T = rpsf_detail_host_parts_for(bytes / std::max<size_t>(1, std::min<size_t>(HostPipe::MAX_CHUNKS, std::max<size_t>(1, bytes >> 22))));
  const int n_chunks = (int)std::min<size_t>(HostPipe::MAX_CHUNKS, std::max<size_t>(1, bytes >> 22));
  const size_t per_chunk = ((count + n_chunks - 1) / n_chunks + 1023) & ~(size_t)1023;
  auto chunk_range = [&](int c, size_t& lo, size_t& hi) { lo = std::min(count, c * per_chunk), hi = std::min(count, lo + per_chunk); };
  hipError_t err = hipSuccess;
  static const bool trace = dev_env("RPSF_HOST_TRACE") != nullptr;
  const auto t_start = std::chrono::steady_clock::now();
  auto ms_since = [&](std::chrono::steady_clock::time_point t0) {
    return std::chrono::duration<double, std::milli>(std::chrono::steady_clock::now() - t0).count();
  };
  double t_conv_in = 0.0, t_conv_out = 0.0, t_wait_out = 0.0;
  const bool direct_in = !in_f64 && is_pinned_host(image), direct_out = !out_f64 && is_pinned_host(out);
  int want_bands = bytes >= ((size_t)24 << 20) ? (int)std::min<size_t>(8, bytes >> 23) : 0;
  if (p->host_bands_opt >= 0) want_bands = p->host_bands_opt;
  const int B = ensure_bands(p, g, want_bands);
  p->last_host_bands = B;
  struct OutChunk {
    size_t lo, hi;
  };
  std::vector<OutChunk> out_chunks;
  if (B >= 2) return host_one_frame_banded(p, image, in_f64, out, out_f64, g, B, direct_in, direct_out);
  {
  const bool one_stream = n_chunks == 1;
  const hipStream_t s_in = one_stream ? p->stream : q.st_in, s_out = one_stream ? p->stream : q.st_out;
  if (direct_in) err = hipMemcpyAsync(q.d_in[0], image, bytes, hipMemcpyHostToDevice, s_in);
  for (int c = 0; c < n_chunks && err == hipSuccess && !direct_in; ++c) {
    size_t lo, hi;
    chunk_range(c, lo, hi);
    const auto t0 = std::chrono::steady_clock::now();
    pool.run(T, [&](int t) {
      size_t a, b;
      rpsf_host::split_range(lo, hi, t, T, a, b);
      rpsf_host::narrow_or_copy(q.h_in[0], image, in_f64 != 0, a, b);
    });
    t_conv_in += ms_since(t0);
    if (hi > lo) err = hipMemcpyAsync(q.d_in[0] + lo, q.h_in[0] + lo, (hi - lo) * sizeof(float), hipMemcpyHostToDevice, s_in);
  }
  if (!one_stream) {
    if (err == hipSuccess) err = hipEventRecord(q.ev_in[0], s_in);
    if (err == hipSuccess) err = hipStreamWaitEvent(p->stream, q.ev_in[0], 0);
  }
  float* zc_out = nullptr;
// ... 139 lines not shown
    if (err != hipSuccess) break;
    t_wait += ms_since(t_phase), t_phase = std::chrono::steady_clock::now();
    const int si = next_in % depth, so = next_out % depth;
    const int fi = can_in ? frames_of(next_in) : 0, fo = out_ready ? frames_of(next_out) : 0;
    const int ci = direct_in ? 0 : fi, co = direct_out ? 0 : fo;
    const int to_enqueue = staged;
    double t_meanwhile = 0.0;
    pool.run(ci + co > 0 ? T : 0,
             [&](int t) {
               const size_t total_in = (size_t)ci * count, total_out = (size_t)co * count;
               size_t a, b;
               rpsf_host::split_range(0, total_in, t, T, a, b);
               while (a < b) {
                 const size_t f = a / count, lo = a % count, hi = std::min(count, lo + (b - a));
                 rpsf_host::narrow_or_copy(q.h_in[si] + f * count, images[first[next_in] + f], in_f64 != 0, lo, hi);
                 a += hi - lo;
               }
               rpsf_host::split_range(0, total_out, t, T, a, b);
               while (a < b) {
                 const size_t f = a / count, lo = a % count, hi = std::min(count, lo + (b - a));
                 rpsf_host::widen_or_copy(outs[first[next_out] + f], out_f64 != 0, q.h_out[so] + f * count, lo, hi);
                 a += hi - lo;
               }
             },
             [&] {
               if (to_enqueue >= 0) {
                 const auto t0 = std::chrono::steady_clock::now();
                 enqueue(to_enqueue);
                 t_meanwhile = ms_since(t0);
               }
             });
    if (to_enqueue >= 0) staged = -1, next_enq = to_enqueue + 1;
    t_enqueue += t_meanwhile;
    t_jobs += ms_since(t_phase) - t_meanwhile;
    if (can_in) staged = next_in++;
    if (out_ready) ++next_out;
  }
  if (trace)
    std::fprintf(stderr, "[rpsf streamed] %d frames in %d groups of up to %d, depth %d, %d parts per job: staging jobs %.3f ms, enqueues %.3f ms, waits %.3f ms, total %.3f ms\n",
                 n_frames, n_groups, G, depth, T, t_jobs, t_enqueue, t_wait, ms_since(t_start));
  if (err != hipSuccess) return rpsf_detail_drain_after_error(p, err, "streamed frames");
  return rpsf_detail_sweep_check(p);
}

static int check_host_call(rpsf_plan* p, const void* a, const void* b, int n_frames, int height, int width, int pad_mode, float pad_value,
                           rpsf_geometry* g) {
  if (!p || !a || !b) return fail(RPSF_E_BADARG, "null argument");
  if (n_frames <= 0) return fail(RPSF_E_BADARG, "n_frames must be positive");
  if (!p->have_k) return fail(RPSF_E_STATE, "no transfer kernel installed (call rpsf_plan_set_transfer first)");
  *g = rpsf_geometry{height, width, pad_mode, pad_value, 0, 0, 0, height, width, 0, height, width};
  int rc = rpsf_detail_check_geometry(p, g);
  if (rc != RPSF_OK) return rc;
  HIP_TRY(hipSetDevice(p->device));
  return RPSF_OK;
}

extern "C" int rpsf_apply_frames_host(rpsf_plan* p, const void* const* images_host, int image_is_f64, int n_frames, int height,
                                      int width, int pad_mode, float pad_value, void* const* outs_host, int out_is_f64) {
  rpsf_geometry g;
  int rc = check_host_call(p, images_host, outs_host, n_frames, height, width, pad_mode, pad_value, &g);
  if (rc != RPSF_OK) return rc;
  for (int f = 0; f < n_frames; ++f)
    if (!images_host[f] || !outs_host[f]) return fail(RPSF_E_BADARG, "null frame pointer");
  return host_frames(p, images_host, image_is_f64, outs_host, out_is_f64, n_frames, g);
}

extern "C" int rpsf_apply_batch_host(rpsf_plan* p, const void* images_host, int image_is_f64, int n_frames, int height, int width,
                                     int pad_mode, float pad_value, void* outs_host, int out_is_f64) {
  rpsf_geometry g;
  int rc = check_host_call(p, images_host, outs_host, n_frames, height, width, pad_mode, pad_value, &g);
  if (rc != RPSF_OK) return rc;
  const size_t count = (size_t)height * width;
  std::vector<const void*> in(n_frames);
  std::vector<void*> out(n_frames);
  for (int f = 0; f < n_frames; ++f) {
    in[f] = static_cast<const char*>(images_host) + (size_t)f * count * (image_is_f64 ? 8 : 4);
    out[f] = static_cast<char*>(outs_host) + (size_t)f * count * (out_is_f64 ? 8 : 4);
  }
  return host_frames(p, in.data(), image_is_f64, out.data(), out_is_f64, n_frames, g);
}

extern "C" int rpsf_apply_batch(rpsf_plan* p, const float* images_host, int n_frames, int height, int width, int pad_mode,
                                float pad_value, float* outs_host) {
  return rpsf_apply_batch_host(p, images_host, 0, n_frames, height, width, pad_mode, pad_value, outs_host, 0);
}

extern "C" int rpsf_apply_host(rpsf_plan* p, const void* image_host, int image_is_f64, int height, int width, int pad_mode,
                               float pad_value, void* out_host, int out_is_f64) {
  rpsf_geometry g;
  int rc = check_host_call(p, image_host, out_host, 1, height, width, pad_mode, pad_value, &g);
  if (rc != RPSF_OK) return rc;
  return host_one_frame(p, image_host, image_is_f64, out_host, out_is_f64, g);
}

extern "C" int rpsf_apply(rpsf_plan* p, const float* image_host, int height, int width, int pad_mode, float pad_value,
                          float* out_host) {
  return rpsf_apply_host(p, image_host, 0, height, width, pad_mode, pad_value, out_host, 0);
}

extern "C" int rpsf_host_alloc(int device, size_t bytes, void** out) {
  if (!out) return fail(RPSF_E_BADARG, "null argument");
  HIP_TRY(hipSetDevice(device));
  HIP_TRY(hipHostMalloc(out, bytes ? bytes : 1, hipHostMallocDefault));
  return RPSF_OK;
}
extern "C" int rpsf_host_free(void* ptr) {
// ... 94 lines not shown
```

### regularizepsf_amd/csrc/rpsf_kernels.hpp

```cpp
#pragma once

struct TileSum {
  const float* planes;
  size_t plane_stride;
  int ld_planes;
  float* out;
  int ld_out;
  int rows, W, row0;
  int lat_r0, lat_c0, half;
  int ntj;
  const uint8_t* cover;
  const uint32_t* tiles;
  int count;
  const uint32_t* done;
  uint32_t epoch;
  uint32_t* queue;
  uint32_t queue_base;
  int n_frames;
  uint32_t n_tiles;
  size_t planes_frame_floats, out_frame_floats;
  int frame_major;
  uint32_t n_tiles_listed;
};
__device__ __forceinline__ uint32_t sum_entry(const TileSum& p, uint32_t i) {
  if (p.n_frames <= 1) return p.tiles[i];
  if (p.frame_major) return ((i / p.n_tiles_listed) << 24) | p.tiles[i % p.n_tiles_listed];
  return ((i % (uint32_t)p.n_frames) << 24) | p.tiles[i / (uint32_t)p.n_frames];
}

typedef float rpsf_f4 __attribute__((ext_vector_type(4)));
typedef int rpsf_i4 __attribute__((ext_vector_type(4)));
__device__ __forceinline__ __amdgpu_buffer_rsrc_t plane_rsrc(const float* base) {
  const uint64_t b = reinterpret_cast<uint64_t>(base);
  const uint32_t lo = __builtin_amdgcn_readfirstlane((uint32_t)b), hi = __builtin_amdgcn_readfirstlane((uint32_t)(b >> 32));
  return __builtin_amdgcn_make_buffer_rsrc(reinterpret_cast<float*>(((uint64_t)hi << 32) | lo), 0, -1, 0x00020000);
}
constexpr int PLANE_AUX_STORE = 16;
constexpr int PLANE_AUX_LOAD = 16 | 2;
__device__ __forceinline__ rpsf_f4 plane_load16_wt(__amdgpu_buffer_rsrc_t r, size_t float_offset) {
  const rpsf_i4 q = __builtin_amdgcn_raw_buffer_load_b128(r, (int)(float_offset * sizeof(float)), 0, PLANE_AUX_LOAD);
  return rpsf_f4{__int_as_float(q.x), __int_as_float(q.y), __int_as_float(q.z), __int_as_float(q.w)};
}
template <int AUX>
__device__ __forceinline__ void plane_store16_aux(__amdgpu_buffer_rsrc_t r, size_t float_offset, rpsf_f4 v) {
  const rpsf_i4 q = {__float_as_int(v.x), __float_as_int(v.y), __float_as_int(v.z), __float_as_int(v.w)};
  __builtin_amdgcn_raw_buffer_store_b128(q, r, (int)(float_offset * sizeof(float)), 0, AUX);
}
__device__ __forceinline__ void plane_store16_wt(__amdgpu_buffer_rsrc_t r, size_t float_offset, rpsf_f4 v) {
  const rpsf_i4 q = {__float_as_int(v.x), __float_as_int(v.y), __float_as_int(v.z), __float_as_int(v.w)};
  __builtin_amdgcn_raw_buffer_store_b128(q, r, (int)(float_offset * sizeof(float)), 0, PLANE_AUX_STORE);
}

template <int UN = 8, bool KNOWN_FUSED = false>
__device__ __forceinline__ void sum_tile(const TileSum& p0, uint32_t entry_any_lane, int tid, int nthreads, bool known_complete = false) {
  typedef float f4 __attribute__((ext_vector_type(4)));
#if defined(__HIP_DEVICE_COMPILE__)
  const uint32_t entry = __builtin_amdgcn_readfirstlane(entry_any_lane);
#else
  const uint32_t entry = entry_any_lane;
#endif
  const uint32_t tile = entry & 0xffffffu, frame = entry >> 24;
  TileSum p = p0;
  p.planes += (size_t)frame * p0.planes_frame_floats;
  p.out += (size_t)frame * p0.out_frame_floats;
  if (p.done) p.done += (size_t)frame * p0.n_tiles;
  const int ti = tile / p.ntj, tj = tile % p.ntj;
  const int cov_all = p.cover[tile];
#if defined(RPSF2_SKEL_PRESUM)
  const int cov = cov_all & ((tj & 1) ? 10 : 5);
#else
  const int cov = cov_all;
#endif
  const bool fused = KNOWN_FUSED || p.done != nullptr;
  if (fused && !known_complete) {
    if (tid == 0) {
      const uint32_t want = p.epoch * (uint32_t)__builtin_popcount(cov_all & 15);
      while (__hip_atomic_load(p.done + tile, __ATOMIC_RELAXED, __HIP_MEMORY_SCOPE_AGENT) != want) __builtin_amdgcn_s_sleep(4);
    }
    __syncthreads();
  }
  const int y0 = max(p.lat_r0 + ti * p.half, p.row0), y1 = min(p.lat_r0 + (ti + 1) * p.half, p.row0 + p.rows);
  const int x0 = max(p.lat_c0 + tj * p.half, 0), x1 = min(p.lat_c0 + (tj + 1) * p.half, p.W);
  if (y0 >= y1 || x0 >= x1) return;
  const bool vec = ((x0 | x1 | p.ld_planes | p.ld_out) & 3) == 0 && (p.plane_stride & 3) == 0 &&
                   ((reinterpret_cast<uintptr_t>(p.planes) | reinterpret_cast<uintptr_t>(p.out)) & 15) == 0;
  const int gw = (x1 - x0) >> 2;
  if (vec) {
    const __amdgpu_buffer_rsrc_t rsrc = plane_rsrc(p.planes);
    const int total = gw * (y1 - y0);
    if ((gw & (gw - 1)) == 0) {
      const int sh = 31 - __builtin_clz((unsigned)gw);
      auto row_of = [&](int i) RPSF_AI { return i >> sh; };
      auto col_of = [&](int i) RPSF_AI { return i & (gw - 1); };
      for (int i0 = tid; i0 < total; i0 += UN * nthreads) {
        f4 v[UN][4];
#pragma unroll
        for (int u = 0; u < UN; ++u) {
          const int i = min(i0 + u * nthreads, total - 1);
          const size_t off = (size_t)(y0 + row_of(i) - p.row0) * p.ld_planes + x0 + (col_of(i) << 2);
#pragma unroll
          for (int k = 0; k < 4; ++k) {
            const size_t o = ((cov >> k) & 1) ? off + k * p.plane_stride : off;
            v[u][k] = fused ? plane_load16_wt(rsrc, o) : __builtin_nontemporal_load(reinterpret_cast<const f4*>(p.planes + o));
          }
        }
#pragma unroll
        for (int u = 0; u < UN; ++u) {
          const int i = i0 + u * nthreads;
          if (i >= total) break;
          f4 acc = {0.f, 0.f, 0.f, 0.f};
#pragma unroll
          for (int k = 0; k < 4; ++k)
            if ((cov >> k) & 1) acc += v[u][k];
          __builtin_nontemporal_store(acc, reinterpret_cast<f4*>(p.out + (size_t)(y0 + row_of(i) - p.row0) * p.ld_out + x0 + (col_of(i) << 2)));
        }
      }
    } else {
      for (int i = tid; i < total; i += nthreads) {
        const int row = i / gw, col = i - row * gw;
        const size_t off = (size_t)(y0 + row - p.row0) * p.ld_planes + x0 + (col << 2);
        f4 acc = {0.f, 0.f, 0.f, 0.f};
#pragma unroll
        for (int k = 0; k < 4; ++k)
          if ((cov >> k) & 1) {
            const size_t o = off + k * p.plane_stride;
            acc += fused ? plane_load16_wt(rsrc, o) : __builtin_nontemporal_load(reinterpret_cast<const f4*>(p.planes + o));
          }
        __builtin_nontemporal_store(acc, reinterpret_cast<f4*>(p.out + (size_t)(y0 + row - p.row0) * p.ld_out + x0 + (col << 2)));
      }
    }
  } else {
    const int w = x1 - x0, total = w * (y1 - y0);
    for (int i = tid; i < total; i += nthreads) {
      const size_t yl = (size_t)(y0 + i / w - p.row0);
      const int x = x0 + i % w;
      float acc = 0.f;
#pragma unroll
      for (int k = 0; k < 4; ++k)
        if ((cov >> k) & 1) {
          const float* src = p.planes + k * p.plane_stride + yl * p.ld_planes + x;
          acc += fused ? __uint_as_float(__hip_atomic_load(reinterpret_cast<const unsigned*>(src), __ATOMIC_RELAXED, __HIP_MEMORY_SCOPE_AGENT)) : *src;
        }
      p.out[yl * p.ld_out + x] = acc;
    }
  }
}
struct NoSideJob {
  __device__ __forceinline__ bool operator()() const { return false; }
};
template <class BETWEEN = NoSideJob, int UN = 8, bool KNOWN_FUSED = false>
__device__ __forceinline__ void sum_tiles_worker(const TileSum& p, int block, int nblocks, BETWEEN&& between = BETWEEN()) {
  if (!p.queue) {
    for (int i = block; i < p.count; i += nblocks) sum_tile<UN, KNOWN_FUSED>(p, p.tiles[i], threadIdx.x, blockDim.x);
    return;
  }
#define RPSF_SUM_LOOKAHEAD 4
  constexpr int SUM_LOOKAHEAD = RPSF_SUM_LOOKAHEAD;
  __shared__ uint32_t pend[SUM_LOOKAHEAD];
  __shared__ uint32_t pick;
  int npend = 0;
  bool exhausted = false;
  bool side_job = true;
  for (;;) {
    if (side_job) side_job = between();
    if (threadIdx.x == 0) {
      uint32_t chosen = 0xffffffffu;
      for (;;) {
        for (int j = 0; j < npend; ++j) {
          const uint32_t tile = pend[j];
          const uint32_t want = p.epoch * (uint32_t)__builtin_popcount(p.cover[tile & 0xffffffu] & 15);
          if (__hip_atomic_load(p.done + (size_t)(tile >> 24) * p.n_tiles + (tile & 0xffffffu), __ATOMIC_RELAXED, __HIP_MEMORY_SCOPE_AGENT) == want) {
            chosen = tile;
            for (int m = j + 1; m < npend; ++m) pend[m - 1] = pend[m];
            --npend;
            break;
          }
        }
        if (chosen != 0xffffffffu) break;
        if (!exhausted && npend < SUM_LOOKAHEAD) {
          const uint32_t i = __hip_atomic_fetch_add(p.queue, 1u, __ATOMIC_RELAXED, __HIP_MEMORY_SCOPE_AGENT) - p.queue_base;
          if (i >= (uint32_t)p.count) exhausted = true; else pend[npend++] = sum_entry(p, i);
          continue;
        }
        if (npend == 0) break;
        if (side_job) {
          chosen = 0xfffffffeu;
          break;
        }
        __builtin_amdgcn_s_sleep(4);
      }
      pick = chosen;
    }
    __syncthreads();
    const uint32_t tile = pick;
    __syncthreads();
    if (tile == 0xffffffffu) return;
    if (tile == 0xfffffffeu) continue;
    sum_tile<UN, KNOWN_FUSED>(p, tile, threadIdx.x, blockDim.x, true);
  }
}

struct PatchParams {
  ImageView im;
  OutView ov;
  int origin_row, origin_col;
  const int4* desc;
  int chunk;
  int seq_base;
  int slot0;
  int sum_first;
  int patch_blocks;
  TileSum ts;
  uint32_t* tile_done;
  unsigned long long* stamps;
  int stagger_ticks;
  int stagger_blocks;
  int n_patches;
  int n_frames;
  size_t im_frame_floats;
  size_t ov_frame_floats;
  const uint16_t* tab;
  const uint32_t* pairtab;
  const cf* tw;
  const float* win;
  const cf* g;
  const cf* gs;
  OutView dv;
  size_t dv_frame_floats;
  const uint4* quads;
  uint32_t* flags;
  uint32_t* dyn_side;
  uint32_t* chunk_xcc;
  uint32_t flag_epoch;
  uint32_t n_tiles;
  int orphan_mod;
  int frame_major;
  int plane_nt;
  int persist;
  uint32_t* xq;
  uint32_t xq_base[8];
  int prefetch;
  const uint32_t* prefetch_tiles;
  uint32_t prefetch_first[9];
  int head_patches;
  int k_prefetch;
  int k_patches;
};

template <class C>
struct Launch {
  static constexpr int WG = C::T < 64 ? 64 : C::T;
// ... 406 lines not shown
```

### regularizepsf_amd/csrc/rpsf_kernels2.hpp

```cpp
#pragma once

template <class C>
struct Launch2 {
  static constexpr int WG = C::T;
  static constexpr int OT_WORDS = C::ORBIT_ROUNDS * 64;
  static constexpr int TABLE_FLOATS = 3 * C::N + OT_WORDS;
  static constexpr size_t LDS_BYTES = (size_t)TABLE_FLOATS * sizeof(float) + (size_t)C::LDS_UNITS * sizeof(cf);
  static_assert(TABLE_FLOATS % 4 == 0, "the exchange buffer must stay 16-byte aligned");
};

__device__ __forceinline__ f32x4 load16_sc1(const float* base, size_t span_bytes, const float* p) {
  typedef int i32x4 __attribute__((ext_vector_type(4)));
  const __amdgpu_buffer_rsrc_t r = __builtin_amdgcn_make_buffer_rsrc(const_cast<float*>(base), 0, span_bytes < 0x7fffffffu ? (int)span_bytes : -1, 0x00020000);
  const i32x4 q = __builtin_amdgcn_raw_buffer_load_b128(r, (int)((p - base) * sizeof(float)), 0,  16);
  return f32x4{__int_as_float(q.x), __int_as_float(q.y), __int_as_float(q.z), __int_as_float(q.w)};
}

namespace dev {
#if defined(RPSF2_ABL_NOGATHER)
constexpr bool NOGATHER = true;
#else
constexpr bool NOGATHER = false;
#endif
#if defined(RPSF2_ABL_NOK)
// ... 125 lines not shown
__device__ __forceinline__ void prefetch_first_round_k(const PatchParams& p, int blk) {
  constexpr int PF = 8;
  constexpr int CHUNK_FLOATS = C::KCH * C::T * 4;
  constexpr int GS_LINES = C::GS_PER_PATCH * 8 / 128;
  static_assert(CHUNK_FLOATS == C::T * 32, "one 128-byte line per thread, patch and word chunk");
  static_assert(C::GS_PER_PATCH * 8 % 128 == 0 && C::T % GS_LINES == 0, "whole lines; whole patches per pass over the side arrays");
  const int x = blk & 7, e0 = blk >> 3, step = p.sum_first >> 3;
  int cnt = p.n_frames <= 1 || p.frame_major ? p.persist : (p.persist + p.n_frames - 1) / p.n_frames;
  cnt = min(cnt, min(p.chunk - p.slot0, p.n_patches - x * p.chunk - p.slot0));
  const int mine = cnt > e0 ? (cnt - e0 + step - 1) / step : 0;
  typedef const int __attribute__((address_space(4))) cint_as4;
  auto patch_of = [&](int i) RPSF_AI {
    const int seq = x * p.chunk + p.slot0 + e0 + i * step;
    const int patch = ((const cint_as4*)(const void*)(p.desc + (p.seq_base + seq)))[2];
    return patch >= 0 && patch < p.k_patches ? patch : -1;
  };
  auto touch = [](const float* a) RPSF_AI {
    return *reinterpret_cast<const volatile float*>(a);
  };
  float d[PF] = {};
  float sink = 0.f;
  const int t = (int)threadIdx.x;
  for (int i0 = 0; i0 < mine; i0 += C::T / GS_LINES) {
    const int i = i0 + t / GS_LINES;
    const int patch = i < mine ? patch_of(i) : -1;
    if (patch >= 0) sink += touch(reinterpret_cast<const float*>(p.gs + (size_t)patch * C::GS_PER_PATCH) + (t % GS_LINES) * 32);
  }
  for (int c = 0; c < C::NCHUNK; ++c)
    for (int i0 = 0; i0 < mine; i0 += PF)
      StaticFor<0, PF>::run([&]<int U>() RPSF_AI {
        const int patch = i0 + U < mine ? patch_of(i0 + U) : -1;
        sink += d[U], d[U] = 0.f;
        if (patch >= 0) d[U] = touch(reinterpret_cast<const float*>(p.g + (size_t)patch * C::G_PER_PATCH) + (size_t)c * CHUNK_FLOATS + t * 32);
      });
  StaticFor<0, PF>::run([&]<int U>() RPSF_AI { sink += d[U]; });
  asm volatile("" ::"v"(sink));
}



template <class C>
__global__ void pack_spectra_kernel2(const cf* __restrict__ s_fft, const cf* __restrict__ t_fft, float alpha, float eps, int n_patches,
                                     const uint16_t* __restrict__ tab, const uint32_t* __restrict__ ot, cf* __restrict__ g, cf* __restrict__ gs);

template <class C, class REENTER, bool HOT = false, bool KNT = true, bool PLANE_NT = false>
__device__ __forceinline__ void patch_body2(const PatchParams& p, REENTER&& reenter) {
  extern __shared__ __attribute__((aligned(16))) float smem[];
  constexpr int T = C::T, N = C::N;
  constexpr bool PERSIST = std::remove_reference_t<REENTER>::enabled;
  const int tu = threadIdx.x, t = tu;
  if constexpr (dev::STAMPS)
    if (threadIdx.x == 0) *reinterpret_cast<unsigned long long*>(reinterpret_cast<cf*>(smem + Launch2<C>::TABLE_FLOATS) + C::BUF_UNITS + 4) = __builtin_amdgcn_s_memrealtime();
  constexpr bool SUM_KNOWN_FUSED = HOT;
  const bool again = PERSIST && ((blockIdx.x >> 30) & 1u);
  if constexpr (dev::STAMPS)
    if (threadIdx.x == 0 && !again) reinterpret_cast<uint32_t*>(smem + 3 * C::N)[Launch2<C>::OT_WORDS - 1] = blockIdx.x;
  const int blk = (int)(blockIdx.x & 0x3fffffffu);
  const bool head_patch = PERSIST && !again && blk < p.sum_first && p.head_patches > 0;
  const int pb = head_patch ? (blk & 7) : blk - p.sum_first;
  bool patchy = pb >= 0 && pb < p.patch_blocks;
  int frame = 0, xrow = 0, seq = 0;
  if (patchy) {
    xrow = p.slot0 + (pb >> 3);
    if constexpr (PERSIST) {
      if (head_patch) {
        xrow = blk >> 3;
      } else if (!again) {
        unsigned* const word = reinterpret_cast<unsigned*>(reinterpret_cast<cf*>(smem + Launch2<C>::TABLE_FLOATS) + C::BUF_UNITS);
        if (tu == 0) *word = __hip_atomic_fetch_add(p.xq + (pb & 7) * 32, 1u, __ATOMIC_RELAXED, __HIP_MEMORY_SCOPE_AGENT) - p.xq_base[pb & 7];
        lds_barrier();
        xrow = (int)__builtin_amdgcn_readfirstlane(*word);
        if (xrow < 0 || xrow > 0x0fffffff) xrow = 0x0fffffff;
        xrow += p.head_patches ? p.sum_first >> 3 : 0;
      }
    }
    if (p.n_frames > 1) {
      if (p.frame_major) {
        const int left = p.n_patches - (pb & 7) * p.chunk, mine = left < p.chunk ? (left > 0 ? left : 1) : p.chunk;
        frame = xrow / mine;
        xrow = frame < p.n_frames ? xrow % mine : p.chunk;
      } else {
        frame = xrow % p.n_frames;
        xrow /= p.n_frames;
      }
    }
    seq = (pb & 7) * p.chunk + xrow;
    if (xrow >= p.chunk || seq >= p.n_patches) {
      if constexpr (!PERSIST) return;
      patchy = false;
    }
  }
  cf* const lds = reinterpret_cast<cf*>(smem + Launch2<C>::TABLE_FLOATS);
  cf* const park = lds + C::BUF_UNITS;
  [[maybe_unused]] auto count_previous = [&]() RPSF_AI {
    if (tu < 4) __hip_atomic_fetch_add(p.tile_done + reinterpret_cast<const unsigned*>(park)[1 + t], 1u, __ATOMIC_RELAXED, __HIP_MEMORY_SCOPE_AGENT);
  };
  if (!patchy) {
    if constexpr (PERSIST) {
      if (again) {
        asm volatile("s_waitcnt vmcnt(0)" ::: "memory");
        lds_barrier();
        count_previous();
      }
    }
    if constexpr (PERSIST && C::T == 512) {
      if (!again && blk < p.sum_first) {
        if (p.k_prefetch && p.head_patches == 0) prefetch_first_round_k<C>(p, blk);
        ImagePrefetch<C> prefetch(p, blk, p.prefetch && p.n_frames <= 1);
        sum_tiles_worker<ImagePrefetch<C>&, 8, SUM_KNOWN_FUSED>(p.ts, 0, 1, prefetch);
        prefetch.finish();
        return;
      }
    }
    sum_tiles_worker<NoSideJob, 8, SUM_KNOWN_FUSED>(p.ts, 0, 1);
    return;
  }
  ImageView im = p.im;
  OutView ov = p.ov;
  im.img += (size_t)frame * p.im_frame_floats;
  ov.out += (size_t)frame * p.ov_frame_floats;
  typedef const int __attribute__((address_space(4))) cint_as4;
  const cint_as4* dptr = (const cint_as4*)(const void*)(p.desc + (p.seq_base + seq));
  const int4 dsc = make_int4(dptr[0], dptr[1], dptr[2], dptr[3]);
  const int patch = dsc.z;
  if (p.stagger_ticks > 0 && pb < p.stagger_blocks && !again && !head_patch) {
    const unsigned long long t0 = __builtin_amdgcn_s_memrealtime();
    const unsigned long long wait = (unsigned long long)(__brev((unsigned)pb >> 3) >> 22) * p.stagger_ticks >> 10;
    while (__builtin_amdgcn_s_memrealtime() - t0 < wait) __builtin_amdgcn_s_sleep(32);
  }
  STAMP(0);
  if constexpr (dev::STAMPS) {
    if (threadIdx.x == 0) p.stamps[(size_t)patch * 16 + 14] = *reinterpret_cast<const unsigned long long*>(reinterpret_cast<cf*>(smem + Launch2<C>::TABLE_FLOATS) + C::BUF_UNITS + 4);
    if (threadIdx.x == 0) p.stamps[(size_t)patch * 16 + 15] = 1 + (again ? reinterpret_cast<const uint32_t*>(smem + 3 * C::N)[Launch2<C>::OT_WORDS - 1] : blockIdx.x);
  }
  const int pr = dsc.x + p.origin_row, pc = dsc.y + p.origin_col;
  const int kpatch = patch;
  const cf* g = p.g + (size_t)kpatch * C::G_PER_PATCH;
  cf* tw = reinterpret_cast<cf*>(smem);
  float* win = smem + 2 * N;
  uint32_t* ot = reinterpret_cast<uint32_t*>(smem + 3 * N);
  static_assert(N <= 2 * T && Launch2<C>::OT_WORDS <= T, "one or two table entries per thread");
  cf tw0 = {0.f, 0.f}, tw1 = {0.f, 0.f};
  float wn0 = 0.f, wn1 = 0.f;
  uint32_t ot0 = 0;
  if (!again) {
    tw0 = p.tw[t < N ? t : 0], tw1 = p.tw[t + T < N ? t + T : 0];
    wn0 = p.win[t < N ? t : 0], wn1 = p.win[t + T < N ? t + T : 0];
    ot0 = p.pairtab[t < Launch2<C>::OT_WORDS ? t : 0];
  }
  GroupIds<C> gids;
  gids.load(p.tab, t);
  cf v[64];
  const bool fast = patch_inside2<C>(pr, pc, im.H, im.W, im.row0, im.rows) && quads_aligned(im.img, im.ld, pc);
  int* maps = reinterpret_cast<int*>(lds);
  if (!fast) {
    build_pad_maps<C>(t, maps, im, pr, pc);
    lds_barrier();
  }
  if constexpr (dev::NOGATHER) {
#pragma unroll
    for (int j = 0; j < 64; ++j) v[j] = cf{(float)(t + j), (float)(t - j)};
  } else {
    load_raw2<C, HOT>(t, v, im, pr, pc, fast, maps);
  }
  if (!again) {
    if (t < N) tw[t] = tw0, win[t] = wn0;
    if (t + T < N) tw[t + T] = tw1, win[t + T] = wn1;
    if (t < Launch2<C>::OT_WORDS) ot[t] = ot0;
  }
  if (!(PERSIST && again && fast)) lds_barrier();
  if constexpr (dev::STAMPS)
    if (PERSIST && !again && t == 0) ot[Launch2<C>::OT_WORDS - 1] = blockIdx.x & 0x3fffffffu;
  constexpr bool EARLY_DRAW = PERSIST && C::SPLIT_ROWS;
  constexpr bool MID_DRAW = PERSIST && !EARLY_DRAW;
  unsigned drawn = 0, qword = 0;
  [[maybe_unused]] auto draw_next = [&]() RPSF_AI {
    if constexpr (PERSIST) {
      if (HOT || p.tile_done) {
        if (tu < 4) qword = reinterpret_cast<const uint32_t*>(p.quads + (p.seq_base + seq))[tu];
        if (tu == 0 && !head_patch)
          drawn = __hip_atomic_fetch_add(p.xq + (pb & 7) * 32, 1u, __ATOMIC_RELAXED, __HIP_MEMORY_SCOPE_AGENT) - p.xq_base[pb & 7] +
                  (p.head_patches ? (unsigned)(p.sum_first >> 3) : 0u);
      }
    }
  };
  window_patch2<C>(t, v, win);
  STAMP(1);
  ABL_VALU(stage1h<C, 0, false>(t, v, tw));
  ABL_LDS(x1_write2<C, 0>(t, v, lds));
  ABL_VALU(stage1h<C, 1, false>(t, v, tw));
  wave_lds_sync();
  ABL_LDS(x1_read2<C, 0>(t, v, lds));
  asm volatile("" ::: "memory");
  ABL_LDS(x1_write2<C, 1>(t, v, lds));
  STAMP(2);
  ABL_VALU(stage2h<C, 0, false>(t, v, tw));
  wave_lds_sync();
  ABL_LDS(x1_read2<C, 1>(t, v, lds));
  STAMP(3);
  cf k[2 * C::KCH];
  if constexpr (dev::NOK) {
#pragma unroll
    for (int j = 0; j < 2 * C::KCH; ++j) k[j] = cf{1.0f + j, 0.5f * t};
  } else {
    load_k_chunk2<C, 0, KNT>(t, k, g);
  }
  cf ko[2 * C::ORBIT_ROUNDS];
  if (t < 64) {
    const cf* gs = p.gs + (size_t)kpatch * C::GS_PER_PATCH;
    StaticFor<0, C::ORBIT_ROUNDS>::run([&]<int R>() RPSF_AI { load_stream16(gs + (size_t)(R * 64 + t) * 2, ko[2 * R], ko[2 * R + 1]); });
  }
  asm volatile("" ::: "memory");
  ABL_LDS(x2_mid_write2<C, 0>(t, v, lds));
  ABL_VALU(stage2h<C, 1, false>(t, v, tw));
  ABL_BARI(2);
  if constexpr (PERSIST) {
    if (again) count_previous();
  }
  ABL_LDS(x2_last_read2<C, 0>(gids, v, lds));
  ABL_BARI(3);
  ABL_LDS(x2_mid_write2<C, 1>(t, v, lds));
  if constexpr (C::SPLIT_ROWS) ABL_VALU(stage3_rows<C, false, 0, 0>(t, gids, v));
  ABL_BARI(4);
  ABL_LDS(x2_last_read2<C, 1>(gids, v, lds));
  STAMP(4);
  if constexpr (C::SPLIT_ROWS) ABL_VALU(stage3_rows<C, false, 1, 0>(t, gids, v));
  ABL_VALU(freq_a<C>(t, gids, v, park));
  if (t < 64) {
    wave_lds_sync();
    StaticFor<0, C::ORBIT_ROUNDS>::run([&]<int R>() RPSF_AI { self_orbit<C>(t, R, ot, ko[2 * R], ko[2 * R + 1], tw, park); });
    wave_lds_sync();
  }
  STAMP(5);
  if constexpr (dev::NOVALU) {
    StaticFor<1, C::NCHUNK>::run([&]<int CI>() RPSF_AI {
// ... 26 lines not shown
  ABL_LDS(x2_mid_read2<C, 1>(t, v, lds));
  if constexpr (EARLY_DRAW) park_draw();
  if constexpr (MID_DRAW) draw_next();
  STAMP(7);
  asm volatile("" ::: "memory");
  ABL_LDS(x1_write2<C, 0>(t, v, lds));
  ABL_VALU(stage2h<C, 1, true>(t, v, tw));
  wave_lds_sync();
  ABL_LDS(x1_read2<C, 0>(t, v, lds));
  asm volatile("" ::: "memory");
  ABL_LDS(x1_write2<C, 1>(t, v, lds));
  STAMP(8);
  ABL_VALU(stage1h<C, 0, true>(t, v, tw));
  wave_lds_sync();
  ABL_LDS(x1_read2<C, 1>(t, v, lds));
  ABL_VALU(stage1h<C, 1, true>(t, v, tw));
  STAMP(9);
  if constexpr (dev::NOSTORE) {
    if (!p.tile_done) {
      float acc = 0.f;
#pragma unroll
      for (int j = 0; j < 64; ++j) acc += v[j].x * v[j].y;
      if (acc == 123456.789f) ov.out[threadIdx.x] = acc;
      return;
    }
  }
  const int plane = HOT || ov.plane_stride ? dsc.w : 0;
  auto add = [](float* a, float val) { unsafeAtomicAdd(a, val); };
  auto pstore4 = [](float* a, f32x4 val) RPSF_AI { __builtin_nontemporal_store(val, reinterpret_cast<f32x4*>(a)); };
  auto pstore1 = [](float* a, float val) RPSF_AI { *a = val; };
  if (!HOT && p.dv.out) {
    OutView dv = p.dv;
    dv.out += (size_t)frame * p.dv_frame_floats;
    uint32_t qw[4];
    direct_begin(p, frame, seq, qw, reinterpret_cast<uint32_t*>(park));
    STAMP(10);
    const float* dbase = dv.out;
    const size_t dspan = ((size_t)(dv.rows - 1) * dv.ld + dv.W) * sizeof(float);
    store_patch2<C>(
        t, v, ov, dv, plane, pr, pc, win, qw, add, [=]<int R1, int C1>(const float* a) RPSF_AI { return load16_sc1(dbase, dspan, a); },
        [](const float* a) { return __uint_as_float(__hip_atomic_load(reinterpret_cast<const unsigned*>(a), __ATOMIC_RELAXED, __HIP_MEMORY_SCOPE_AGENT)); },
        pstore4, pstore1);
    STAMP(11);
    direct_end(p, frame, plane, qw);
    STAMP(12);
  } else if (HOT || p.tile_done) {
    const float* pbase = ov.out;
    const __amdgpu_buffer_rsrc_t rsrc = plane_rsrc(pbase);
    if constexpr (!EARLY_DRAW && !MID_DRAW) draw_next();
    if constexpr (MID_DRAW) {
      if (tu == 0) *reinterpret_cast<unsigned*>(park) = drawn;
      if (tu < 4) reinterpret_cast<unsigned*>(park)[1 + tu] = (unsigned)frame * p.n_tiles + quad_tile(qword);
    }
    store_patch2<C, HOT>(
        t, v, ov, ov, plane, pr, pc, win, nullptr, add, []<int R1, int C1>(const float* a) RPSF_AI { return *reinterpret_cast<const f32x4*>(a); },
        [](const float* a) { return *a; },
        [=](float* a, f32x4 val) RPSF_AI {
          if constexpr (dev::NOSTORE) asm volatile("" ::"v"(val.x), "v"(val.y), "v"(val.z), "v"(val.w), "v"(a));
          else if constexpr (PLANE_NT) plane_store16_aux<16 | 2>(rsrc, (size_t)(a - pbase), val);
          else plane_store16_wt(rsrc, (size_t)(a - pbase), val);
        },
        [](float* a, float val) RPSF_AI { __hip_atomic_store(reinterpret_cast<unsigned*>(a), __float_as_uint(val), __ATOMIC_RELAXED, __HIP_MEMORY_SCOPE_AGENT); });
    STAMP(10);
    if constexpr (PERSIST) {
      if constexpr (!EARLY_DRAW && !MID_DRAW) {
        if (tu == 0) *reinterpret_cast<unsigned*>(park) = drawn;
        if (tu < 4) reinterpret_cast<unsigned*>(park)[1 + tu] = (unsigned)frame * p.n_tiles + quad_tile(qword);
      }
      lds_barrier();
      STAMP(12);
      const unsigned nx = __builtin_amdgcn_readfirstlane(*reinterpret_cast<const unsigned*>(park));
      const int left = p.n_patches - (pb & 7) * p.chunk;
      const bool more = (int)nx < (left < p.chunk ? left : p.chunk) * (p.n_frames > 1 ? p.n_frames : 1);
      reenter(0x40000000u | (head_patch ? (unsigned)blk : (unsigned)p.sum_first + (more ? ((nx << 3) | (unsigned)(pb & 7)) : (unsigned)p.patch_blocks)),
              (unsigned)tu);
    }
    asm volatile("s_waitcnt vmcnt(0)" ::: "memory");
    lds_barrier();
    if (t < 4) {
      const uint4 q4 = p.quads[p.seq_base + seq];
      const uint32_t w = t == 0 ? q4.x : t == 1 ? q4.y : t == 2 ? q4.z : q4.w;
      __hip_atomic_fetch_add(p.tile_done + (size_t)frame * p.n_tiles + quad_tile(w), 1u, __ATOMIC_RELAXED, __HIP_MEMORY_SCOPE_AGENT);
    }
    STAMP(12);
  } else {
    store_patch2<C>(t, v, ov, ov, plane, pr, pc, win, nullptr, add, []<int R1, int C1>(const float* a) RPSF_AI { return *reinterpret_cast<const f32x4*>(a); },
                    [](const float* a) { return *a; }, pstore4, pstore1);
  }
  STAMP(13);
}

template <class C>
__global__ __launch_bounds__(Launch2<C>::WG, 2) void patch_kernel2(PatchParams p) {
  patch_body2<C>(p, NoReenter());
}
#define RPSF_VGPR_ATTR
extern "C" __global__ __launch_bounds__(512, 2) RPSF_VGPR_ATTR void patch_kernel2_256p(PatchParams p);
extern "C" __global__ __launch_bounds__(128, 2) void patch_kernel2_128p(PatchParams p);
extern "C" __global__ __launch_bounds__(128, 2) void patch_kernel2_128pc(PatchParams p);
extern "C" __global__ __launch_bounds__(128, 2) void patch_kernel2_128pcs(PatchParams p);
template <class C>
struct PersistentKernel2;
template <>
struct PersistentKernel2<Cfg256v2> {
  static constexpr auto fn = &patch_kernel2_256p;
  static constexpr auto fn_k_cached = &patch_kernel2_256p;
// ... 45 lines not shown
```

### regularizepsf_amd/csrc/rpsf_plan.hpp

```cpp
#pragma once
#include <hip/hip_runtime.h>

#include <algorithm>
#include <cmath>
#include <cstdlib>
#include <memory>
#include <string>
#include <utility>
#include <vector>

#include "rpsf_device.hpp"
#include "rpsf_hostpipe.hpp"
#include "rpsf_lattice.hpp"
#include "rpsf_saturation.hpp"
#include "rpsf_side_unit.hpp"

RPSF_PLANS_V1(RPSF_DECL_V1)
RPSF_PLANS_V2(RPSF_DECL_V2)
RPSF_PLANS_V3(RPSF_DECL_V3)

static const char* dev_env(const char* name) {
#if defined(RPSF_DEV_ENV)
  return std::getenv(name);
#else
  (void)name;
  return nullptr;
#endif
}

template <class T, hipError_t (*Free)(void*) = hipFree>
struct DevBuf {
  T* p = nullptr;
  DevBuf() = default;
  DevBuf(DevBuf&& o) noexcept : p(std::exchange(o.p, nullptr)) {}
  DevBuf& operator=(DevBuf&& o) noexcept {
    std::swap(p, o.p);
    return *this;
  }
  ~DevBuf() { reset(); }
  void reset() {
    if (p) (void)Free(p);
    p = nullptr;
  }
  hipError_t alloc(size_t count) {
    reset();
    return hipMalloc(&p, count * sizeof(T));
  }
  hipError_t upload(const T* host, size_t count) {
    const hipError_t e = alloc(count);
    return e != hipSuccess ? e : hipMemcpy(p, host, count * sizeof(T), hipMemcpyHostToDevice);
  }
  operator T*() const { return p; }
};

struct PipeRelease {
  void operator()(rpsf_host::HostPipe* q) const {
    q->destroy();
    delete q;
  }
};
struct FftPlanRelease {
  void operator()(void* h) const;
};
struct SatDeviceRelease {
  void operator()(SatDevice* d) const { rpsf_sat_destroy(d); }
};

struct SatScratch {
  std::vector<double> padded;
  std::vector<uint8_t> mask;
  struct Raw {
    int64_t idx;
    double value;
  };
  std::vector<Raw> raw;
};

struct FftPath {
  DevBuf<cf> d_kfull;
  DevBuf<cf> d_buf;
  DevBuf<float> d_win;
  DevBuf<uint8_t> d_colour;
  std::unique_ptr<void, FftPlanRelease> plan;
  int chunk = 0;
};

struct PatchPath {
  DevBuf<uint16_t> d_tab;
  DevBuf<uint32_t> d_pairtab;
  DevBuf<cf> d_tw;
  DevBuf<cf> d_g, d_gs;
  size_t g_elems = 0, gs_elems = 0;
  DevBuf<unsigned long long> d_stamps;
  DevBuf<float> d_sink;
  int stagger_us = -1;
  int round_capacity = 0;
  bool direct_ok = false;
  bool v2 = false;
  DevBuf<uint32_t> d_tile_done;
  DevBuf<uint32_t> d_sum_order;
  uint32_t done_epoch = 0;
  size_t done_frames = 1;
  int done_last_frames = 1;
  DevBuf<uint32_t> d_sum_queue;
  uint32_t sum_queue_base = 0;
  bool no_fuse = false;
  int sum_first = -1;
  bool prefetch = false;
  DevBuf<uint32_t> d_prefetch_tiles;
  uint32_t prefetch_first[9] = {0, 0, 0, 0, 0, 0, 0, 0, 0};
  int k_prefetch = 0;
  int head_patches = 0;
  bool fuse_pays = false;
  bool persist = false;
  bool k_cached = false;
  int reserved_cus = 0;
  DevBuf<uint32_t> d_xq;
  uint32_t xq_base[8] = {0, 0, 0, 0, 0, 0, 0, 0};
  DevBuf<uint4> d_quads;
  DevBuf<uint8_t> d_tile_info;
  DevBuf<uint32_t> d_flags;
  DevBuf<uint32_t> d_dyn;
  DevBuf<uint32_t> d_chunk_xcc;
  size_t flag_frames = 0;
  uint32_t epoch = 0;
  int orphan_mod = 0;
  int plane_nt_opt = -1;
  DevBuf<float> d_planes;
  size_t planes_floats = 0;
  size_t planes_frames = 0;
};

struct SweepPath {
  bool ok = false;
  DevBuf<Job3> d_jobs;
  DevBuf<Region3> d_regions;
  int n_regions = 0, ks = 0, par_j = 0;
  std::vector<int32_t> slot;
  long slabs = 0, patch_slots = 0;
  DevBuf<float> d_k3;
  size_t k3_floats = 0;
  DevBuf<float> d_zero;
  DevBuf<uint32_t, hipHostFree> err;
  uint32_t* d_err = nullptr;
  DevBuf<unsigned long long> d_stamps;
};

struct PlanStream {
  hipStream_t stream = nullptr;
  bool borrowed_stream = false;
  hipEvent_t ev[4] = {nullptr, nullptr, nullptr, nullptr};
  hipEvent_t ev_busy = nullptr;
  ~PlanStream() {
    if (ev_busy) (void)hipEventDestroy(ev_busy);
    for (auto& e : ev)
      if (e) (void)hipEventDestroy(e);
    if (stream && !borrowed_stream) (void)hipStreamDestroy(stream);
  }
};

struct rpsf_plan : PlanStream {
  int device = 0, N = 0, n_patches = 0;
  DevBuf<int32_t> d_coords;
  DevBuf<float> d_win;
  std::unique_ptr<rpsf_host::HostPipe, PipeRelease> pipe;
  std::unique_ptr<SatDevice, SatDeviceRelease> sat_dev;
  std::vector<SatScratch> sat;
  rpsf_plan* parent = nullptr;
  std::vector<int32_t> k_index;
  std::vector<std::unique_ptr<rpsf_plan>> bands;
  std::vector<int> band_rows;
  std::vector<int> band_in_rows;
  int bands_h = 0, bands_w = 0, bands_mode = -1, bands_want = -1;
  bool have_k = false;
  std::vector<int32_t> h_coords;
  int overlap_mode = 0;
  int cu_count = 256;
  bool lattice = false;
  int host_bands_opt = -1, stream_group_opt = 0, stream_depth_opt = 0;
  int sat_group_opt = 0;
  int sat_batch_info[4] = {};
  DevBuf<float> d_view_in, d_view_out;
  size_t view_in_floats = 0, view_out_floats = 0;
  DevBuf<uint8_t> d_host_masks;
  size_t host_mask_bytes = 0;
  hipEvent_t ev_view = nullptr;
  hipStream_t view_stream = nullptr;
  bool view_busy = false;
  int last_host_bands = 0;
  hipStream_t last_stream = nullptr;
  bool busy_valid = false;
  bool multi_stream = false;
  int lat_r0 = 0, lat_c0 = 0, nti = 0, ntj = 0;
  DevBuf<uint8_t> d_cover;
  DevBuf<int4> d_desc;
  std::vector<int32_t> h_order;
  int corner_min[2] = {0, 0}, corner_max[2] = {0, 0};
  bool generic = false;
  FftPath fft;
  PatchPath patch;
  SweepPath sweep;

  ~rpsf_plan() {
    (void)hipSetDevice(device);
    if (stream) (void)hipStreamSynchronize(stream);
    if (ev_view) (void)hipEventDestroy(ev_view);
    bands.clear();
  }
};

static const rpsf_plan* owner(const rpsf_plan* p) { return p->parent ? p->parent : p; }

enum OverlapKind { OV_ATOMIC = 0, OV_PLANES = 1, OV_DIRECT = 2, OV_SWEEP = 3 };

template <class F>
static int dispatch_n(int N, F&& f) {
  switch (N) {
    case 256: return f.template operator()<Cfg256>();
    case 128: return f.template operator()<Cfg128>();
    case 64: return f.template operator()<Cfg64>();
    case 32: return f.template operator()<Cfg32>();
    case 16: return f.template operator()<Cfg16>();
    default: return fail(RPSF_E_UNSUPPORTED, "patch size " + std::to_string(N) + " has no compiled plan (16..256, powers of two)");
  }
}

template <class C, bool Gen2>
struct PatchPlan {
  using Cfg = C;
  using L = std::conditional_t<Gen2, Launch2<C>, Launch<C>>;
  static constexpr bool V2 = Gen2;
  static constexpr int WG = L::WG, TEAMS = WG / C::T;
  static constexpr size_t LDS_BYTES = L::LDS_BYTES;
  static constexpr size_t PACK_PER_PATCH = C::G_PER_PATCH + (Gen2 ? C::GS_PER_PATCH : 0);
  static_assert(TEAMS == patch_teams(C::N), "lattice_build cuts the chunks by patch_teams()");
  static constexpr auto kernel() { if constexpr (Gen2) return &patch_kernel2<C>; else return &patch_kernel<C>; }
  static constexpr auto pack() { if constexpr (Gen2) return &pack_kernel2<C>; else return &pack_kernel<C>; }
  static constexpr auto pack_spectra() { if constexpr (Gen2) return &pack_spectra_kernel2<C>; else return &pack_spectra_kernel<C>; }
};

static void host_tables(int N, std::vector<cf>& tw, std::vector<float>& win) {
  tw.resize(N);
  win.resize(N);
  for (int k = 0; k < N; ++k) {
    double a = -2.0 * M_PI * k / N;
    tw[k] = cf{(float)std::cos(a), (float)std::sin(a)};
    win[k] = (float)std::sin((k + 0.5) * (M_PI / N));
  }
}

template <class T>
static int upload_tables(int device, DevBuf<uint16_t>& d_tab, DevBuf<cf>& d_tw, DevBuf<float>* d_win = nullptr, DevBuf<uint32_t>* d_pairtab = nullptr) {
  using C = typename T::Cfg;
  std::vector<uint16_t> tab((size_t)C::T * C::NSLOT * 2);
  std::vector<uint32_t> pt;
  if constexpr (T::V2) {
    build_slot_table2<C>(tab.data());
    pt.resize((size_t)C::ORBIT_ROUNDS * 64);
    if (special_slots2<C>() > 64 || build_orbit_table2<C>(tab.data(), pt.data()) != C::NORBIT)
      return fail(RPSF_E_STATE, "slot / orbit table inconsistent (internal)");
  } else {
    build_slot_table<C>(tab.data());
    pt.resize((size_t)C::PT_WORDS + 1);
    if (d_pairtab && build_pair_table<C>(tab.data(), pt.data()) > C::NP) return fail(RPSF_E_STATE, "pair table overflow (internal)");
  }
  std::vector<cf> tw;
  std::vector<float> win;
  host_tables(C::N, tw, win);
  HIP_TRY(hipSetDevice(device));
  if (d_pairtab) HIP_TRY(d_pairtab->upload(pt.data(), pt.size()));
  HIP_TRY(d_tab.upload(tab.data(), tab.size()));
  HIP_TRY(d_tw.upload(tw.data(), tw.size()));
  if (d_win) HIP_TRY(d_win->upload(win.data(), win.size()));
  return RPSF_OK;
}

struct Batch {
  int frames = 1;
  size_t im_stride = 0, out_stride = 0;
};

RPSF_HIDDEN OverlapKind rpsf_detail_overlap_kind(const rpsf_plan* p);
RPSF_HIDDEN int rpsf_detail_check_geometry(const rpsf_plan* p, const rpsf_geometry* g);
RPSF_HIDDEN bool rpsf_detail_lattice_covers_window(const rpsf_plan* p, const rpsf_geometry& g);
RPSF_HIDDEN int rpsf_detail_launch_apply(rpsf_plan* p, const float* d_img, float* d_out, const rpsf_geometry& g, hipStream_t st,
                                         hipEvent_t ev_k0, hipEvent_t ev_k1 = nullptr, Batch b = Batch());
RPSF_HIDDEN int rpsf_detail_launch_batch(rpsf_plan* p, const float* d_imgs, float* d_outs, int n_frames, size_t im_stride, size_t out_stride,
                                         const rpsf_geometry& g, hipStream_t st, hipEvent_t ev_k0 = nullptr, hipEvent_t ev_k1 = nullptr);
RPSF_HIDDEN int rpsf_detail_plan_create_impl(rpsf_plan** out, int device, int patch_size, int n_patches, const int32_t* coords_rc, rpsf_plan* parent,
                                             const int32_t* k_index);
RPSF_HIDDEN void rpsf_detail_drop_bands(rpsf_plan* p);
RPSF_HIDDEN int rpsf_detail_sweep_check(rpsf_plan* p);
RPSF_HIDDEN int rpsf_detail_drain_after_error(rpsf_plan* p, hipError_t err, const char* where);
RPSF_HIDDEN int rpsf_detail_pipe_ensure(rpsf_plan* p, size_t slot_floats, int depth);
RPSF_HIDDEN int rpsf_detail_host_parts_for(size_t bytes);
```

### regularizepsf_amd/csrc/rpsf_saturated.hip

```cpp
#include <hip/hip_runtime.h>

#include <algorithm>
#include <cmath>
#include <cstdlib>
#include <cstring>
#include <limits>
#include <string>
#include <vector>

#include "rpsf_plan.hpp"
#include "rpsf_core_saturation_batch.hpp"
#include "rpsf_convert.hpp"
#include "rpsf_core_convert.hpp"

using rpsf_host::HostPipe;
using rpsf_host::HostPool;

static void py_slice(long start, long stop, long n, long* lo, long* hi) {
  if (start < 0) start = std::max(start + n, 0L);
  if (stop < 0) stop = std::max(stop + n, 0L);
  *lo = std::min(start, n);
  *hi = std::min(stop, n);
}

// ... 106 lines not shown
    }
    const size_t in_lo = (size_t)r_lo * PW, in_hi = (size_t)r_hi * PW;
    const int T = rpsf_detail_host_parts_for((in_hi - in_lo) * sizeof(float));
    pool.run(T, [&](int t) {
      size_t a, b;
      rpsf_host::split_range(in_lo, in_hi, t, T, a, b);
      rpsf_host::narrow_or_copy(q.h_in[s], padded, true, a, b);
    });
  }

  hipError_t enqueue(int s) {
    HostPipe& q = *p->pipe;
    const size_t in_lo = (size_t)r_lo * PW, in_hi = (size_t)r_hi * PW, out_lo = (size_t)o_lo * PW, out_hi = out_lo + (size_t)o_rows * PW;
    hipError_t err = hipMemcpyAsync(q.d_in[s], q.h_in[s] + in_lo, (in_hi - in_lo) * sizeof(float), hipMemcpyHostToDevice, p->stream);
    if (err == hipSuccess && rpsf_detail_launch_apply(p, q.d_in[s], q.d_out[s], g, p->stream, nullptr) != RPSF_OK) err = hipErrorUnknown;
    if (err == hipSuccess) err = hipMemcpyAsync(q.h_out[s] + out_lo, q.d_out[s], (out_hi - out_lo) * sizeof(float), hipMemcpyDeviceToHost, p->stream);
    if (err == hipSuccess) err = hipEventRecord(q.ev_out[s], p->stream);
    return err;
  }

  hipError_t finish(int s, void* out_host) {
    HostPipe& q = *p->pipe;
    HostPool& pool = HostPool::get(p->device);
    hipError_t err = hipEventSynchronize(q.ev_out[s]);
    if (err != hipSuccess) return err;
    const int rows_parts = std::min(H, pool.width() * 4);
    pool.run(rows_parts, [&](int part) {
      const long ra = (long)H * part / rows_parts, rb = (long)H * (part + 1) / rows_parts;
      for (long r = ra; r < rb; ++r) {
        const float* src = q.h_out[s] + (size_t)(2 * N + r) * PW + 2 * N;
        if (out_f64) {
          double* dst = static_cast<double*>(out_host) + (size_t)r * W;
          for (long c = 0; c < W; ++c) dst[c] = (double)src[c];
        } else {
          std::memcpy(static_cast<float*>(out_host) + (size_t)r * W, src, (size_t)W * sizeof(float));
        }
      }
    });
    for (const SatScratch::Raw& x : p->sat[s].raw) {
      const long r = x.idx / PW - 2L * N, c = x.idx % PW - 2L * N;
      if (out_f64) static_cast<double*>(out_host)[(size_t)r * W + c] = x.value;
      else static_cast<float*>(out_host)[(size_t)r * W + c] = (float)x.value;
    }
    return hipSuccess;
  }
};

static int check_saturated_call(rpsf_plan* p, const void* a, const void* b, int height, int width, int pad_mode, int dilation, int neighborhood_width) {
  if (!p || !a || !b) return fail(RPSF_E_BADARG, "null argument");
  if (height <= 0 || width <= 0) return fail(RPSF_E_BADARG, "image shape must be positive");
  if (pad_mode < 0 || pad_mode > RPSF_PAD_WRAP) return fail(RPSF_E_BADARG, "unknown pad mode");
  if (dilation < 1 || neighborhood_width < 0) return fail(RPSF_E_BADARG, "dilation must be >= 1 and the neighbourhood width >= 0 (other values: the NumPy route)");
  if (!p->have_k) return fail(RPSF_E_STATE, "no transfer kernel installed (call rpsf_plan_set_transfer first)");
  return RPSF_OK;
}

extern "C" int rpsf_apply_host_saturated(rpsf_plan* p, const void* image_host, int image_is_f64, int height, int width, int pad_mode,
                                         double threshold, int dilation, int neighborhood_width, void* out_host, int out_is_f64) {
  int rc = check_saturated_call(p, image_host, out_host, height, width, pad_mode, dilation, neighborhood_width);
  if (rc != RPSF_OK) return rc;
  SatRun run;
  rc = run.init(p, height, width, pad_mode, threshold, dilation, neighborhood_width, image_is_f64, out_is_f64, 1);
  if (rc != RPSF_OK) return rc;
  run.prepare(0, image_host);
  hipError_t err = run.enqueue(0);
  if (err == hipSuccess) err = run.finish(0, out_host);
  if (err != hipSuccess) return rpsf_detail_drain_after_error(p, err, "saturated host frame");
  return rpsf_detail_sweep_check(p);
}

extern "C" int rpsf_apply_frames_host_saturated(rpsf_plan* p, const void* const* images_host, int image_is_f64, int n_frames, int height, int width,
                                                int pad_mode, double threshold, int dilation, int neighborhood_width, void* const* outs_host,
                                                int out_is_f64) {
  int rc = check_saturated_call(p, images_host, outs_host, height, width, pad_mode, dilation, neighborhood_width);
  if (rc != RPSF_OK) return rc;
  if (n_frames <= 0) return fail(RPSF_E_BADARG, "n_frames must be positive");
  for (int f = 0; f < n_frames; ++f)
    if (!images_host[f] || !outs_host[f]) return fail(RPSF_E_BADARG, "null frame pointer");
  SatRun run;
  rc = run.init(p, height, width, pad_mode, threshold, dilation, neighborhood_width, image_is_f64, out_is_f64, std::min(2, n_frames));
  if (rc != RPSF_OK) return rc;
  hipError_t err = hipSuccess;
  for (int f = 0; f < n_frames && err == hipSuccess; ++f) {
    run.prepare(f & 1, images_host[f]);
    err = run.enqueue(f & 1);
    if (err == hipSuccess && f > 0) err = run.finish((f - 1) & 1, outs_host[f - 1]);
  }
  if (err == hipSuccess) err = run.finish((n_frames - 1) & 1, outs_host[n_frames - 1]);
  if (err != hipSuccess) return rpsf_detail_drain_after_error(p, err, "saturated host frames");
  return rpsf_detail_sweep_check(p);
}

struct SatDeviceRun {
  SatCall call;
  rpsf_geometry g;
  int r_lo, r_hi;
};

static int sat_device_init(rpsf_plan* p, int height, int width, int pad_mode, double threshold, int dilation, int neighborhood_width,
                           SatDeviceRun* run) {
  if (neighborhood_width / 2 < 1) return fail(RPSF_E_BADARG, "the device route needs neighborhood_width // 2 >= 1 (an always-empty window: the host route)");
  int o_lo, o_rows;
  const int rc = padded_geometry(p, height, width, &run->r_lo, &run->r_hi, &o_lo, &o_rows, &run->g);
  if (rc != RPSF_OK) return rc;
  run->call = SatCall{height, width, p->N, pad_mode, dilation, neighborhood_width, threshold, run->r_lo, o_lo, o_rows};
  HIP_TRY(hipSetDevice(p->device));
// ... 229 lines not shown
    if (v[f].dtype != v[0].dtype || v[f].row_stride != v[0].row_stride || v[f].col_stride != v[0].col_stride ||
        static_cast<char*>(v[f].data) - static_cast<char*>(v[0].data) != (int64_t)f * s.frame_bytes)
      s.direct = s.uniform = false;
  }
  if (n > 1 && (s.frame_bytes <= 0 || s.frame_bytes % 4 || s.frame_bytes < (int64_t)(v[0].rows - 1) * v[0].row_stride + 4 * (int64_t)v[0].cols))
    s.direct = false;
  return s;
}

static int view_staging(DevBuf<float>& buf, size_t& cap, size_t floats) {
  if (floats <= cap) return RPSF_OK;
  HIP_TRY(hipDeviceSynchronize());
  cap = 0;
  HIP_TRY(buf.alloc(floats));
  cap = floats;
  return RPSF_OK;
}

static int apply_views(rpsf_plan* p, const rpsf_view* images, const rpsf_view* outs, int n, int pad_mode, float pad_value, double threshold, int dilation,
                       int neighborhood_width, void* stream, int* route_or_null, bool batch, const SatMasks* masks = nullptr) {
  if (route_or_null) *route_or_null = 0;
  if (!p) return fail(RPSF_E_BADARG, "null plan");
  if (n < 0) return fail(RPSF_E_BADARG, "n_frames must not be negative");
  if (n == 0) return RPSF_OK;
  if (!images || !outs) return fail(RPSF_E_BADARG, "null argument");
  bool empty = false;
  for (int f = 0; f < n; ++f) {
    bool e_in, e_out;
    if (const char* why = rpsfconv::view_problem(images + f, false, &e_in)) return fail(RPSF_E_BADARG, std::string("image: ") + why);
    if (const char* why = rpsfconv::view_problem(outs + f, true, &e_out)) return fail(RPSF_E_BADARG, std::string("out: ") + why);
    if (images[f].rows != images[0].rows || images[f].cols != images[0].cols || outs[f].rows != images[0].rows || outs[f].cols != images[0].cols)
      return fail(RPSF_E_BADARG, "every image and every out view must have one shape");
    empty = e_in;
  }
  if (empty) return RPSF_OK;
  if (pad_mode < 0 || pad_mode > RPSF_PAD_WRAP) return fail(RPSF_E_BADARG, "unknown pad mode");
  if (!p->have_k) return fail(RPSF_E_STATE, "no transfer kernel installed (call rpsf_plan_set_transfer first)");
  const int H = images[0].rows, W = images[0].cols;
  const bool saturated = masks || !(threshold == std::numeric_limits<double>::infinity());
  if (masks)
    if (const int bad = check_masks(*masks, n, H, W)) return bad;
  const ViewSide in = view_side(images, n, saturated), out = view_side(outs, n, saturated);
  rpsf_geometry g{H, W, pad_mode, pad_value, 0, 0, 0, H, in.direct ? (int)(images[0].row_stride / 4) : W, 0, H, out.direct ? (int)(outs[0].row_stride / 4) : W};
  SatDeviceRun run;
  int rc;
  if (saturated) {
    if (dilation < 1 || neighborhood_width < 0) return fail(RPSF_E_BADARG, "dilation must be >= 1 and the neighbourhood width >= 0 (other values: the NumPy route)");
    rc = sat_device_init(p, H, W, pad_mode, threshold, dilation, neighborhood_width, &run);
  } else {
    rc = rpsf_detail_check_geometry(p, &g);
  }
  if (rc != RPSF_OK) return rc;
  HIP_TRY(hipSetDevice(p->device));
  hipStream_t st = stream ? reinterpret_cast<hipStream_t>(stream) : p->stream;
  const size_t npix = (size_t)H * W, stage_stride = (npix + 3) / 4 * 4;
  const bool staged = !in.direct || !out.direct;
  if (!in.direct && (rc = view_staging(p->d_view_in, p->view_in_floats, stage_stride * n)) != RPSF_OK) return rc;
  if (!out.direct && (rc = view_staging(p->d_view_out, p->view_out_floats, stage_stride * n)) != RPSF_OK) return rc;
  if (staged) {
    if (!p->ev_view) HIP_TRY(hipEventCreateWithFlags(&p->ev_view, hipEventDisableTiming));
    if (p->view_busy && st != p->view_stream) HIP_TRY(hipStreamWaitEvent(st, p->ev_view, 0));
  }
  const float* d_in = static_cast<const float*>(images[0].data);
  float* d_out = static_cast<float*>(outs[0].data);
  size_t in_stride = (size_t)(in.frame_bytes / 4), out_stride = (size_t)(out.frame_bytes / 4);
  if (!in.direct) {
    if (in.uniform) rc = rpsf_conv_gather(images[0], n, in.frame_bytes, p->d_view_in, (int64_t)stage_stride, st);
    for (int f = 0; !in.uniform && f < n && rc == RPSF_OK; ++f) rc = rpsf_conv_gather(images[f], 1, 0, p->d_view_in + f * stage_stride, 0, st);
    if (rc != RPSF_OK) return rc;
    d_in = p->d_view_in, in_stride = stage_stride;
  }
  if (!out.direct) d_out = p->d_view_out, out_stride = stage_stride;
  if (!saturated) {
    rc = rpsf_detail_launch_batch(p, d_in, d_out, n, in_stride, out_stride, g, st);
  } else {
    const int G = batch ? sat_group_frames(p, run, masks != nullptr) : 1;
    SatBatchStats stats;
    stats.frames = n;
    for (int f0 = 0; f0 < n && rc == RPSF_OK; f0 += G)
      rc = sat_device_apply_group(p, run, std::min(G, n - f0), d_in + (size_t)f0 * in_stride, in_stride, d_out + (size_t)f0 * out_stride, out_stride,
                                  batch ? rpsfsatb::ORDER_LONGEST_FIRST : rpsfsatb::ORDER_FRAMES, st, &stats, nullptr, masks, f0);
    if (batch && rc == RPSF_OK) stats.store(p);
  }
  if (rc == RPSF_OK && !out.direct) {
    if (out.uniform) rc = rpsf_conv_scatter(p->d_view_out, (int64_t)stage_stride, outs[0], n, out.frame_bytes, st);
    for (int f = 0; !out.uniform && f < n && rc == RPSF_OK; ++f) rc = rpsf_conv_scatter(p->d_view_out + f * stage_stride, 0, outs[f], 1, 0, st);
  }
  if (staged) {
    HIP_TRY(hipEventRecord(p->ev_view, st));
    p->view_stream = st, p->view_busy = true;
  }
  if (rc == RPSF_OK && route_or_null)
    *route_or_null = (in.direct ? 0 : RPSF_ROUTE_C1 | (batch ? RPSF_ROUTE_STAGED : 0)) | (out.direct ? 0 : RPSF_ROUTE_C2) | (saturated ? RPSF_ROUTE_SATURATED : 0);
  return rc;
}

extern "C" int rpsf_apply_view(rpsf_plan* p, const rpsf_view* image, const rpsf_view* out, int pad_mode, float pad_value, double threshold, int dilation,
                               int neighborhood_width, void* stream, int* route_or_null) {
  return apply_views(p, image, out, 1, pad_mode, pad_value, threshold, dilation, neighborhood_width, stream, route_or_null, false);
}

extern "C" int rpsf_apply_batch_view(rpsf_plan* p, const rpsf_view* images, const rpsf_view* outs, int n_frames, int pad_mode, float pad_value,
                                     double threshold, int dilation, int neighborhood_width, void* stream, int* route_or_null) {
  return apply_views(p, images, outs, n_frames, pad_mode, pad_value, threshold, dilation, neighborhood_width, stream, route_or_null, true);
}

// ... 85 lines not shown
  if (!masks_host_or_null) n_masks = 0;
  if (n_masks < 0 || (n_masks > 1 && n_masks != n_frames)) return fail(RPSF_E_BADARG, "mask: no mask, one mask or one mask per frame");
  for (int f = 0; f < n_masks; ++f)
    if (!masks_host_or_null[f]) return fail(RPSF_E_BADARG, "mask: null mask pointer");
  SatDeviceRun run;
  rc = sat_device_init(p, height, width, pad_mode, threshold, dilation, neighborhood_width, &run);
  if (rc != RPSF_OK) return rc;
  const size_t npix = (size_t)height * width;
  const int G = std::min(sat_group_frames(p, run, true), n_frames);
  rc = rpsf_detail_pipe_ensure(p, npix * G, 1);
  if (rc != RPSF_OK) return rc;
  const int T = rpsf_detail_host_parts_for(npix * G * sizeof(float));
  SatBatchStats stats;
  stats.frames = n_frames;
  std::vector<rpsf_view> views;
  if (n_masks == 1 && (rc = upload_host_masks(p, masks_host_or_null, 1, height, width, &views)) != RPSF_OK) return rc;
  for (int f0 = 0; f0 < n_frames; f0 += G) {
    const int fg = std::min(G, n_frames - f0);
    if (n_masks > 1 && (rc = upload_host_masks(p, masks_host_or_null + f0, fg, height, width, &views)) != RPSF_OK) return rc;
    const SatMasks masks{views.empty() ? nullptr : views.data(), (int)views.size(), fill_nonfinite};
    rc = sat_host_group(p, run, fg, images_host + f0, image_is_f64, outs_host + f0, out_is_f64, rpsfsatb::ORDER_LONGEST_FIRST, T, &stats, &masks);
    if (rc != RPSF_OK) return rc;
  }
  stats.store(p);
  return rpsf_detail_sweep_check(p);
}

extern "C" int rpsf_saturation_kernel_ms(rpsf_plan* p, double ms[5]) {
  if (!p || !ms) return fail(RPSF_E_BADARG, "null argument");
  for (int i = 0; i < 5; ++i) ms[i] = 0.0;
  if (!p->sat_dev) return RPSF_OK;
  HIP_TRY(hipSetDevice(p->device));
  return rpsf_sat_kernel_ms(p->sat_dev.get(), ms);
}

extern "C" int rpsf_saturation_batch_info(rpsf_plan* p, int info[4]) {
  if (!p || !info) return fail(RPSF_E_BADARG, "null argument");
  for (int i = 0; i < 4; ++i) info[i] = p->sat_batch_info[i];
  return RPSF_OK;
}

static int sat_fill_frames(rpsf_plan* p, const float* images_host, int n_frames, int height, int width, int pad_mode, double threshold, int dilation,
                           int neighborhood_width, int order, float* padded_host, uint8_t* masks_host, int* groups_per_frame_or_null,
                           SatBatchStats* stats, const SatMasks* masks = nullptr, int* masked_per_frame_or_null = nullptr) {
  if (!p || !images_host || !padded_host || !masks_host) return fail(RPSF_E_BADARG, "null argument");
  if (n_frames < 1) return fail(RPSF_E_BADARG, "n_frames must be positive");
  if (height <= 0 || width <= 0) return fail(RPSF_E_BADARG, "image shape must be positive");
  if (pad_mode < 0 || pad_mode > RPSF_PAD_WRAP) return fail(RPSF_E_BADARG, "unknown pad mode");
  if (dilation < 1 || neighborhood_width / 2 < 1) return fail(RPSF_E_BADARG, "dilation must be >= 1 and neighborhood_width // 2 >= 1");
  if (order < rpsfsatb::ORDER_LONGEST_FIRST || order > rpsfsatb::ORDER_FRAMES) return fail(RPSF_E_BADARG, "order must be 0, 1 or 2");
  const long PH = (long)height + 4L * p->N, PW = (long)width + 4L * p->N;
  if (PH * PW >= ((long)1 << 31)) return fail(RPSF_E_UNSUPPORTED, "padded frame too large for this entry point");
  HIP_TRY(hipSetDevice(p->device));
  if (!p->sat_dev) p->sat_dev.reset(rpsf_sat_create());
  SatDevice* sd = p->sat_dev.get();
  const SatCall call{height, width, p->N, pad_mode, dilation, neighborhood_width, threshold, 0, 0, 1};
  const size_t npix = (size_t)height * width, np = (size_t)PH * PW;
  const int G = std::min(n_frames, p->sat_group_opt > 0 ? p->sat_group_opt : rpsfsatb::auto_group_frames(np, (size_t)height * PW, masks != nullptr));
  DevBuf<float> d_images;
  HIP_TRY(d_images.upload(images_host, npix * n_frames));
  stats->frames = n_frames;
  for (int f0 = 0; f0 < n_frames; f0 += G) {
    const int fg = std::min(G, n_frames - f0);
    float *padded = nullptr, *corrected = nullptr;
    size_t p_stride = 0, c_stride = 0;
    const float* d_first = d_images;
    int rc;
    if (!masks) {
      rc = rpsf_sat_fill_batch(sd, call, fg, d_first + (size_t)f0 * npix, npix, order, p->stream, &padded, &p_stride, &corrected, &c_stride);
    } else {
      const std::vector<rpsfsat::MaskView> views = group_views(*masks, f0, fg);
      rc = rpsf_sat_fill_batch_masked(sd, call, fg, d_first + (size_t)f0 * npix, npix, views.empty() ? nullptr : views.data(), masks->fill_nonfinite,
                                      order, p->stream, &padded, &p_stride, &corrected, &c_stride);
    }
    if (rc == RPSF_OK) rc = rpsf_sat_masks_batch(sd, call, p->stream, masks_host + (size_t)f0 * np);
    if (rc != RPSF_OK) {
      (void)hipStreamSynchronize(p->stream);
      return rc;
    }
    for (int f = 0; f < fg; ++f) {
      HIP_TRY(hipMemcpy(padded_host + (size_t)(f0 + f) * np, padded + f * p_stride, np * sizeof(float), hipMemcpyDeviceToHost));
      int n_hot, n_mask, n_groups;
      rpsf_sat_frame_counts(sd, f, &n_hot, &n_mask, &n_groups);
      if (groups_per_frame_or_null) groups_per_frame_or_null[f0 + f] = n_groups;
      if (masked_per_frame_or_null) masked_per_frame_or_null[f0 + f] = n_mask;
    }
    long groups = 0, masked = 0;
    rpsf_sat_batch_totals(sd, &groups, &masked);
    stats->frame_groups += 1, stats->groups += groups, stats->masked += masked;
  }
  return RPSF_OK;
}

extern "C" int rpsf_saturation_fill_device(rpsf_plan* p, const float* image_host, int height, int width, int pad_mode, double threshold, int dilation,
                                           int neighborhood_width, int reverse_groups, float* padded_host, uint8_t* mask_host, int* n_groups_or_null) {
  SatBatchStats stats;
  return sat_fill_frames(p, image_host, 1, height, width, pad_mode, threshold, dilation, neighborhood_width,
                         reverse_groups ? rpsfsatb::ORDER_REVERSED : rpsfsatb::ORDER_FRAMES, padded_host, mask_host, n_groups_or_null, &stats);
}

extern "C" int rpsf_saturation_fill_batch_device(rpsf_plan* p, const float* images_host, int n_frames, int height, int width, int pad_mode,
                                                 double threshold, int dilation, int neighborhood_width, int order, float* padded_host,
                                                 uint8_t* masks_host, int* groups_per_frame_or_null) {
  SatBatchStats stats;
  const int rc = sat_fill_frames(p, images_host, n_frames, height, width, pad_mode, threshold, dilation, neighborhood_width, order, padded_host,
                                 masks_host, groups_per_frame_or_null, &stats);
  if (rc == RPSF_OK) stats.store(p);
  return rc;
}

extern "C" int rpsf_saturation_fill_masked_device(rpsf_plan* p, const float* images_host, int n_frames, int height, int width, int pad_mode,
                                                  double threshold, int dilation, int neighborhood_width, int order, const uint8_t* masks_in_host,
                                                  int n_masks, size_t mask_frame_bytes, int64_t mask_row_stride, int64_t mask_col_stride,
                                                  int fill_nonfinite, float* padded_host, uint8_t* masks_host, int* groups_per_frame_or_null,
                                                  int* masked_per_frame_or_null) {
  if (!p) return fail(RPSF_E_BADARG, "null argument");
  if (!masks_in_host) n_masks = 0;
  if (n_masks < 0 || (n_masks > 1 && n_masks != n_frames)) return fail(RPSF_E_BADARG, "mask: no mask, one mask or one mask per frame");
  if (n_masks && (height <= 0 || width <= 0 || mask_row_stride <= 0 || mask_col_stride <= 0 ||
                  (size_t)(height - 1) * mask_row_stride + (size_t)(width - 1) * mask_col_stride + 1 > mask_frame_bytes))
    return fail(RPSF_E_BADARG, "mask: the strides do not fit mask_frame_bytes");
  HIP_TRY(hipSetDevice(p->device));
  DevBuf<uint8_t> d_masks;
  std::vector<rpsf_view> views((size_t)n_masks);
  if (n_masks) HIP_TRY(d_masks.upload(masks_in_host, mask_frame_bytes * n_masks));
  for (int f = 0; f < n_masks; ++f) views[f] = rpsf_view{d_masks + f * mask_frame_bytes, RPSF_DTYPE_UINT8, height, width, mask_row_stride, mask_col_stride};
  const SatMasks masks{views.empty() ? nullptr : views.data(), n_masks, fill_nonfinite};
  SatBatchStats stats;
  return sat_fill_frames(p, images_host, n_frames, height, width, pad_mode, threshold, dilation, neighborhood_width, order, padded_host, masks_host,
                         groups_per_frame_or_null, &stats, &masks, masked_per_frame_or_null);
}


extern "C" int rpsf_saturation_fill(double* padded, int rows, int cols, const uint8_t* mask, int neighborhood_width) {
  if (!padded || !mask || rows <= 0 || cols <= 0) return fail(RPSF_E_BADARG, "bad argument");
  const long h = neighborhood_width / 2;
  const double nan = std::nan("");
  for (long i = 0; i < rows; ++i)
    for (long j = 0; j < cols; ++j) {
      if (!mask[i * cols + j]) continue;
      long r0, r1, c0, c1;
      py_slice(i - h, i + h, rows, &r0, &r1);
      py_slice(j - h, j + h, cols, &c0, &c1);
      double sum = 0.0;
      long cnt = 0;
      for (long r = r0; r < r1; ++r)
        for (long c = c0; c < c1; ++c) {
          double v = padded[r * cols + c];
          if (v == v) sum += v, ++cnt;
        }
      padded[i * cols + j] = cnt ? sum / (double)cnt : nan;
    }
  return RPSF_OK;
}
```

Measured before the change: 92400 Mpixels/s.

## Pipeline consecutive 256-patch applies across two alternating streams with device gating

Adds a second stream lane for persistent 256-pixel patch launches, so back-to-back single-frame applies alternate lanes and can overlap. Per-lane work-queue counters and a per-tile summed sequence gate keep the overlap-add ordered on the device. A mapped error word reports gate problems. Lanes are joined whenever the caller touches the stream, transfer or options. This removes the launch gap and tail between frames, at the cost of added bookkeeping, cross-kernel spinning and extra complexity.

```diff
diff --git a/__graft_entry__.py b/__graft_entry__.py
--- a/__graft_entry__.py
+++ b/__graft_entry__.py
@@ -14,8 +14,8 @@
     from regularizepsf_amd import build as hip_build
 
     hip_build.build()
-    cores = [ROOT / "regularizepsf_amd" / "csrc" / n for n in ("rpsf_core.hpp", "rpsf_core2.hpp", "rpsf_core3.hpp", "rpsf_plan3.hpp", "rpsf_lattice.hpp", "rpsf_core_builder.hpp", "rpsf_core_builder_sub.hpp", "rpsf_core_builder_wide.hpp", "rpsf_core_cleanup.hpp", "rpsf_core_cleanup_wide.hpp", "rpsf_core_stars.hpp", "rpsf_core_stars_deblend.hpp", "rpsf_core_stars_shape.hpp", "rpsf_core_stars_photometry.hpp", "rpsf_core_stars_refine.hpp", "rpsf_core_stars_fit.hpp", "rpsf_core_stars_fit_weighted.hpp", "rpsf_core_stars_fitpos.hpp", "rpsf_core_stars_render.hpp", "rpsf_core_stars_mesh.hpp", "rpsf_core_saturation.hpp", "rpsf_core_saturation_batch.hpp", "rpsf_core_convert.hpp", "rpsf_core_scale.hpp")]
-    for stem in ("emu", "emu2", "emu3", "emu_lattice", "emu_builder", "emu_builder_sub", "emu_builder_wide", "emu_cleanup_wide", "emu_stars", "emu_deblend", "emu_shapes", "emu_photometry", "emu_refine", "emu_fit", "emu_fit_weighted", "emu_fitpos", "emu_render", "emu_stars_mesh", "emu_cleanup", "emu_saturation", "emu_saturation_batch", "emu_mask", "emu_convert", "emu_scale"):
+    cores = [ROOT / "regularizepsf_amd" / "csrc" / n for n in ("rpsf_core.hpp", "rpsf_core2.hpp", "rpsf_core3.hpp", "rpsf_plan3.hpp", "rpsf_lattice.hpp", "rpsf_lanes.hpp", "rpsf_core_builder.hpp", "rpsf_core_builder_sub.hpp", "rpsf_core_builder_wide.hpp", "rpsf_core_cleanup.hpp", "rpsf_core_cleanup_wide.hpp", "rpsf_core_stars.hpp", "rpsf_core_stars_deblend.hpp", "rpsf_core_stars_shape.hpp", "rpsf_core_stars_photometry.hpp", "rpsf_core_stars_refine.hpp", "rpsf_core_stars_fit.hpp", "rpsf_core_stars_fit_weighted.hpp", "rpsf_core_stars_fitpos.hpp", "rpsf_core_stars_render.hpp", "rpsf_core_stars_mesh.hpp", "rpsf_core_saturation.hpp", "rpsf_core_saturation_batch.hpp", "rpsf_core_convert.hpp", "rpsf_core_scale.hpp")]
+    for stem in ("emu", "emu2", "emu3", "emu_lattice", "emu_lanes", "emu_builder", "emu_builder_sub", "emu_builder_wide", "emu_cleanup_wide", "emu_stars", "emu_deblend", "emu_shapes", "emu_photometry", "emu_refine", "emu_fit", "emu_fit_weighted", "emu_fitpos", "emu_render", "emu_stars_mesh", "emu_cleanup", "emu_saturation", "emu_saturation_batch", "emu_mask", "emu_convert", "emu_scale"):
         emu_src = ROOT / "tests" / "emu" / f"{stem}.cpp"
         emu_out = ROOT / "tests" / "emu" / f"lib{stem}.so"
         if not emu_out.exists() or emu_out.stat().st_mtime < max(emu_src.stat().st_mtime, *(c.stat().st_mtime for c in cores)):
diff --git a/include/rpsf.h b/include/rpsf.h
--- a/include/rpsf.h
+++ b/include/rpsf.h
@@ -46,7 +46,8 @@
   RPSF_OPT_STREAM_DEPTH = 7,
   RPSF_OPT_DEBUG_ORPHAN = 8,
   RPSF_OPT_HEAD_KPREFETCH = 9,
-  RPSF_OPT_SAT_GROUP = 10
+  RPSF_OPT_SAT_GROUP = 10,
+  RPSF_OPT_PIPELINE = 11
 };
 int rpsf_plan_set_option(rpsf_plan* plan, int option, int value);
 int rpsf_plan_sweep_info(const rpsf_plan* plan, int* regions, long* jobs, long* patch_slots, int* slabs_per_phase);
diff --git a/regularizepsf_amd/_native.py b/regularizepsf_amd/_native.py
--- a/regularizepsf_amd/_native.py
+++ b/regularizepsf_amd/_native.py
@@ -329,7 +329,7 @@
         check(lib().rpsf_plan_set_overlap_mode(self._handle, {"auto": 0, "atomic": 1, "planes": 2, "direct": 3, "sweep": 4}[mode]))
 
     OPTIONS = {"persist": 1, "fuse": 2, "k_cached": 3, "plane_nt": 4, "host_bands": 5, "stream_group": 6, "stream_depth": 7, "debug_orphan": 8,
-               "head_kprefetch": 9, "sat_group": 10}
+               "head_kprefetch": 9, "sat_group": 10, "pipeline": 11}
 
     def set_option(self, name: str, value: int) -> None:
         check(lib().rpsf_plan_set_option(self._handle, self.OPTIONS[name], int(value)))
diff --git a/regularizepsf_amd/csrc/rpsf.hip b/regularizepsf_amd/csrc/rpsf.hip
--- a/regularizepsf_amd/csrc/rpsf.hip
+++ b/regularizepsf_amd/csrc/rpsf.hip
@@ -34,6 +34,15 @@
   }
 }
 static bool has_v3(int N) { return sweep_patch_size(N); }
+
+static int ensure_error_word(rpsf_plan* p) {
+  SweepPath& sw = p->sweep;
+  if (p->parent || sw.err) return RPSF_OK;
+  HIP_TRY(hipHostMalloc(reinterpret_cast<void**>(&sw.err.p), 64, hipHostMallocMapped));
+  std::memset(sw.err, 0, 64);
+  HIP_TRY(hipHostGetDevicePointer(reinterpret_cast<void**>(&sw.d_err), sw.err, 0));
+  return RPSF_OK;
+}
 
 static int build_sweep_lists(rpsf_plan* p, int target_regions) {
   const int nli = p->nti - 1, nlj = p->ntj - 1;
@@ -50,11 +59,7 @@
     HIP_TRY(sw.d_zero.alloc(16));
     HIP_TRY(hipMemset(sw.d_zero, 0, 64));
   }
-  if (!p->parent && !sw.err) {
-    HIP_TRY(hipHostMalloc(reinterpret_cast<void**>(&sw.err.p), 64, hipHostMallocMapped));
-    std::memset(sw.err, 0, 64);
-    HIP_TRY(hipHostGetDevicePointer(reinterpret_cast<void**>(&sw.d_err), sw.err, 0));
-  }
+  if (const int rc = ensure_error_word(p); rc != RPSF_OK) return rc;
   p->sweep.n_regions = (int)plan.regions.size(), p->sweep.ks = plan.ks, p->sweep.slabs = plan.slabs, p->sweep.patch_slots = plan.patch_slots;
   p->sweep.ok = true;
 #if defined(RPSF3_STAMPS) || defined(RPSF3_DUMP)
@@ -91,10 +96,12 @@
     HIP_TRY(p->patch.d_sum_order.upload(t.sum_order.data(), t.sum_order.size()));
     HIP_TRY(p->patch.d_tile_done.alloc(t.sum_order.size()));
     HIP_TRY(hipMemset(p->patch.d_tile_done, 0, t.sum_order.size() * sizeof(uint32_t)));
-    HIP_TRY(p->patch.d_sum_queue.alloc(1));
-    HIP_TRY(hipMemset(p->patch.d_sum_queue, 0, sizeof(uint32_t)));
-    HIP_TRY(p->patch.d_xq.alloc(8 * 32));
-    HIP_TRY(hipMemset(p->patch.d_xq, 0, 8 * 32 * sizeof(uint32_t)));
+    HIP_TRY(p->patch.d_sum_queue.alloc(2 * 32));
+    HIP_TRY(hipMemset(p->patch.d_sum_queue, 0, 2 * 32 * sizeof(uint32_t)));
+    HIP_TRY(p->patch.d_xq.alloc(2 * 8 * 32));
+    HIP_TRY(hipMemset(p->patch.d_xq, 0, 2 * 8 * 32 * sizeof(uint32_t)));
+    HIP_TRY(p->patch.d_tile_summed.alloc(t.sum_order.size()));
+    HIP_TRY(hipMemset(p->patch.d_tile_summed, 0, t.sum_order.size() * sizeof(uint32_t)));
     std::copy_n(t.prefetch_first, 9, p->patch.prefetch_first);
     HIP_TRY(p->patch.d_prefetch_tiles.alloc(std::max<size_t>(1, t.prefetch_tiles.size())));
     HIP_TRY(hipMemcpy(p->patch.d_prefetch_tiles, t.prefetch_tiles.data(), t.prefetch_tiles.size() * sizeof(uint32_t), hipMemcpyHostToDevice));
@@ -306,6 +313,16 @@
     HIP_TRY(hipEventCreateWithFlags(&p->ev_busy, hipEventDisableTiming));
     rl = setup_lattice(p);
     if (rl != RPSF_OK) return rl;
+    if (p->patch.v2 && N == 256) {
+      rl = ensure_error_word(p);
+      if (rl != RPSF_OK) return rl;
+      if (!parent && p->lattice) {
+        HIP_TRY(hipStreamCreateWithFlags(&p->lane1, hipStreamNonBlocking));
+        HIP_TRY(hipEventCreateWithFlags(&p->ev_lane, hipEventDisableTiming));
+        HIP_TRY(hipEventCreateWithFlags(&p->ev_fork, hipEventDisableTiming));
+        p->patch.lanes.enabled = true;
+      }
+    }
     if (p->sweep.ok) {
       rl = dispatch_v3(N, [&]<class C>() -> int {
         HIP_TRY(hipFuncSetAttribute(reinterpret_cast<const void*>(&sweep_kernel<C>), hipFuncAttributeMaxDynamicSharedMemorySize, (int)C::LDS_BYTES));
@@ -349,7 +366,29 @@
   return rpsf_detail_plan_create_impl(out, device, patch_size, n_patches, coords_rc, nullptr, nullptr);
 }
 
-extern "C" void* rpsf_plan_stream(rpsf_plan* p) { return p ? (void*)p->stream : nullptr; }
+int rpsf_detail_join_lanes(rpsf_plan* p) {
+  rpsf_plan* r = p->parent ? p->parent : p;
+  if (!r->patch.lanes.join()) return RPSF_OK;
+  HIP_TRY(hipSetDevice(r->device));
+  HIP_TRY(hipEventRecord(r->ev_lane, r->lane1));
+  HIP_TRY(hipStreamWaitEvent(r->stream, r->ev_lane, 0));
+  return RPSF_OK;
+}
+
+void rpsf_detail_clear_error(rpsf_plan* p) {
+  rpsf_plan* r = p->parent ? p->parent : p;
+  volatile uint32_t* word = r->sweep.err;
+  if (!word) return;
+  if (r->busy_valid && r->stream) (void)hipStreamSynchronize(r->stream);
+  *word = 0;
+}
+
+extern "C" void* rpsf_plan_stream(rpsf_plan* p) {
+  if (!p) return nullptr;
+  (void)rpsf_detail_join_lanes(p);
+  (p->parent ? p->parent : p)->patch.lanes.exposed = true;
+  return (void*)p->stream;
+}
 
 extern "C" void rpsf_plan_destroy(rpsf_plan* p) { delete p; }
 
@@ -409,6 +448,7 @@
 extern "C" int rpsf_plan_set_transfer(rpsf_plan* p, const float* k_host) {
   if (!p || !k_host) return fail(RPSF_E_BADARG, "null argument");
   HIP_TRY(hipSetDevice(p->device));
+  if (const int jrc = rpsf_detail_join_lanes(p); jrc != RPSF_OK) return jrc;
   const cf* k = reinterpret_cast<const cf*>(k_host);
   if (p->generic) return install_transfer(p, KSource{k, hipMemcpyHostToDevice}, 0, p->n_patches);
   const size_t per = (size_t)p->N * p->N;
@@ -427,12 +467,14 @@
 extern "C" int rpsf_plan_set_transfer_device(rpsf_plan* p, const void* k_dev) {
   if (!p || !k_dev) return fail(RPSF_E_BADARG, "null argument");
   HIP_TRY(hipSetDevice(p->device));
+  if (const int jrc = rpsf_detail_join_lanes(p); jrc != RPSF_OK) return jrc;
   return install_transfer(p, KSource{reinterpret_cast<const cf*>(k_dev)}, 0, p->n_patches);
 }
 
 extern "C" int rpsf_plan_set_transfer_spectra_device(rpsf_plan* p, const void* s_c64_dev, const void* t_c64_dev, double alpha, double epsilon) {
   if (!p || !s_c64_dev || !t_c64_dev) return fail(RPSF_E_BADARG, "null argument");
   HIP_TRY(hipSetDevice(p->device));
+  if (const int jrc = rpsf_detail_join_lanes(p); jrc != RPSF_OK) return jrc;
   return install_transfer(p, KSource{nullptr, hipMemcpyDeviceToDevice, reinterpret_cast<const cf*>(s_c64_dev), reinterpret_cast<const cf*>(t_c64_dev),
                                      alpha, epsilon}, 0, p->n_patches);
 }
@@ -514,6 +556,9 @@
   int k_prefetch;
   uint32_t xq_base[8], xq_draws[8];
   uint32_t sum_queue_base, sum_queue_draws;
+  int lane;
+  bool gate;
+  uint32_t seq;
 };
 
 static bool patch_launch_too_large(const rpsf_plan* p, int frames) {
@@ -542,9 +587,9 @@
   if (p->patch.plane_nt_opt >= 0) L.plane_nt = p->patch.plane_nt_opt != 0 && N128 && p->patch.k_cached;
   const int tune_frames = b.frames;
   L.sum_first = sum_first_for(p, tune_frames);
-  L.sum_queue_base = p->patch.sum_queue_base;
   const int rows = std::min(L.chunk * b.frames, std::max(1, (p->patch.round_capacity - L.sum_first - p->patch.reserved_cus) / 8));
-  if (!(p->patch.persist && rows > 0 && hot_geometry(p, d_img, g, b.im_stride))) {
+  const bool out_span_ok = !N256 || (size_t)g.out_rows * g.ld_out * sizeof(float) < ((size_t)1 << 32);
+  if (!(p->patch.persist && rows > 0 && out_span_ok && hot_geometry(p, d_img, g, b.im_stride))) {
     L.form = PatchLaunch::FUSED;
     const int nsum = std::max(8, std::min(count, p->patch.round_capacity)) + L.sum_first;
     L.sum_queue_draws = (uint32_t)(count + nsum);
@@ -562,7 +607,6 @@
     if (N128) L.stagger_ticks = tune_frames == 1 && p->n_patches >= 4096 ? 600 : 0;
   }
   for (int x = 0; x < 8; ++x) {
-    L.xq_base[x] = p->patch.xq_base[x];
     const int slots_x = std::min(L.chunk, std::max(0, p->n_patches - x * L.chunk)) * b.frames;
     L.xq_draws[x] = (uint32_t)(std::max(0, slots_x - (L.head_patches ? L.sum_first / 8 : 0)) + rows);
   }
@@ -603,11 +647,13 @@
   TileSum& ts = pp.ts;
   fill_plane_sum(ts, p, d_out, g, b);
   ts.half = p->N / 2, ts.cover = p->d_cover, ts.tiles = p->patch.d_sum_order, ts.count = n_tiles * b.frames;
-  ts.done = p->patch.d_tile_done, ts.epoch = p->patch.done_epoch;
+  ts.done = p->patch.d_tile_done, ts.epoch = p->patch.lanes.done_epoch;
   ts.n_frames = b.frames, ts.n_tiles = (uint32_t)n_tiles, ts.n_tiles_listed = (uint32_t)n_tiles, ts.frame_major = L.frame_major;
-  ts.queue = p->patch.d_sum_queue, ts.queue_base = L.sum_queue_base;
+  ts.queue = p->patch.d_sum_queue + L.lane * 32, ts.queue_base = L.sum_queue_base;
+  ts.summed = p->patch.d_tile_summed, ts.seq = L.seq;
+  ts.gate_on = L.gate ? 1u : 0u, ts.gate_want = L.seq - 1, ts.err = o->sweep.d_err;
   if (L.form != PatchLaunch::PERSISTENT) return pp;
-  pp.persist = L.rows, pp.xq = p->patch.d_xq;
+  pp.persist = L.rows, pp.xq = p->patch.d_xq + L.lane * 8 * 32;
   pp.head_patches = L.head_patches, pp.prefetch = L.prefetch, pp.prefetch_tiles = p->patch.d_prefetch_tiles;
   pp.k_prefetch = L.k_prefetch, pp.k_patches = o->n_patches;
   for (int x = 0; x < 9; ++x) pp.prefetch_first[x] = p->patch.prefetch_first[x];
@@ -755,7 +801,9 @@
 }
 
 int rpsf_detail_launch_apply(rpsf_plan* p, const float* d_img, float* d_out, const rpsf_geometry& g, hipStream_t st,
-                             hipEvent_t ev_k0, hipEvent_t ev_k1, Batch b) {
+                             hipEvent_t ev_k0, hipEvent_t ev_k1, Batch b, bool may_pipeline) {
+  if (!may_pipeline || p->parent || !p->patch.lanes.enabled)
+    if (const int rc = rpsf_detail_join_lanes(p); rc != RPSF_OK) return rc;
   if (p->generic) return launch_apply_generic(p, d_img, d_out, g, st, ev_k0, ev_k1, b);
   const OverlapKind kind = rpsf_detail_overlap_kind(p);
   if (kind == OV_SWEEP) {
@@ -807,23 +855,52 @@
     L = patch_launch_for<T>(p, d_img, g, b, fused);
     return RPSF_OK;
   });
+  const bool clear = kind == OV_ATOMIC || ((kind == OV_DIRECT || fused) && !rpsf_detail_lattice_covers_window(p, g));
+  const bool gated_kernel = L.form == PatchLaunch::PERSISTENT && p->patch.v2 && p->N == 256;
+  const bool hot = may_pipeline && gated_kernel && !p->parent && b.frames == 1 && st == p->stream && !p->multi_stream && !clear && !ev_k0 && !ev_k1 &&
+                   !p->patch.lanes.epoch_restarts(b.frames);
+  const LaneRange img_range{reinterpret_cast<uintptr_t>(d_img),
+                            reinterpret_cast<uintptr_t>(d_img + (size_t)std::max(0, g.image_rows - 1) * g.ld_image + g.width)};
+  const LaneRange out_range{reinterpret_cast<uintptr_t>(d_out), reinterpret_cast<uintptr_t>(d_out + (size_t)std::max(0, g.out_rows - 1) * g.ld_out + g.width)};
+  LaneLayout layout;
+  layout.v[0] = g.width, layout.v[1] = g.out_row0, layout.v[2] = g.out_rows, layout.v[3] = g.origin_row, layout.v[4] = g.origin_col;
+  layout.v[5] = (int64_t)p->patch.planes_floats;
+  const LaneBook book_before = p->patch.lanes;
+  const LanePick pick = p->patch.lanes.begin(hot, gated_kernel, img_range, out_range, layout);
+  {
+    hipError_t e = hipSuccess;
+    if (pick.join) {
+      e = hipEventRecord(p->ev_lane, p->lane1);
+      if (e == hipSuccess) e = hipStreamWaitEvent(p->stream, p->ev_lane, 0);
+    }
+    if (e == hipSuccess && pick.fork) e = hipEventRecord(p->ev_fork, p->stream);
+    if (e == hipSuccess && pick.wait_fork) e = hipStreamWaitEvent(p->lane1, p->ev_fork, 0);
+    if (e != hipSuccess) {
+      p->patch.lanes = book_before;
+      (void)hipDeviceSynchronize();
+      p->patch.lanes.join();
+      return fail(RPSF_E_HIP, std::string("launch lanes: ") + hipGetErrorString(e));
+    }
+  }
+  hipStream_t run = pick.lane == 1 ? p->lane1 : st;
+  L.lane = pick.lane, L.gate = pick.gate, L.seq = pick.seq, L.sum_queue_base = pick.sum_queue_base;
+  for (int x = 0; x < 8; ++x) L.xq_base[x] = pick.xq_base[x];
+  LaneDraws draws;
+  for (int x = 0; x < 8; ++x) draws.xq[x] = L.xq_draws[x];
+  draws.sum = L.sum_queue_draws;
+  p->patch.lanes.commit(pick, draws);
   if (kind == OV_DIRECT && ++p->patch.epoch >= (1u << 24) - 1) {
     HIP_TRY(hipMemsetAsync(p->patch.d_flags, 0, n_tiles * p->patch.flag_frames * sizeof(uint32_t), st));
     HIP_TRY(hipMemsetAsync(p->patch.d_chunk_xcc, 0, 8 * sizeof(uint32_t), st));
     p->patch.epoch = 1;
   }
   if (fused) {
-    const bool restart = b.frames != p->patch.done_last_frames || p->patch.done_epoch + 1 >= (1u << 29);
-    if (restart) HIP_TRY(hipMemsetAsync(p->patch.d_tile_done, 0, n_tiles * p->patch.done_frames * sizeof(uint32_t), st));
-    p->patch.done_last_frames = b.frames;
-    p->patch.done_epoch = restart ? 1 : p->patch.done_epoch + 1;
-  }
-  for (int x = 0; x < 8; ++x) p->patch.xq_base[x] += L.xq_draws[x];
-  p->patch.sum_queue_base += L.sum_queue_draws;
-  const bool clear = kind == OV_ATOMIC || ((kind == OV_DIRECT || fused) && !rpsf_detail_lattice_covers_window(p, g));
+    if (p->patch.lanes.next_epoch(b.frames).restart)
+      HIP_TRY(hipMemsetAsync(p->patch.d_tile_done, 0, n_tiles * p->patch.done_frames * sizeof(uint32_t), st));
+  }
   if (const int rc = clear ? clear_window(d_out, g, b, st) : RPSF_OK; rc != RPSF_OK) return rc;
   if (ev_k0) HIP_TRY(hipEventRecord(ev_k0, st));
-  int rc = launch_patches(p, L, d_img, d_out, g, kind, st, b);
+  int rc = launch_patches(p, L, d_img, d_out, g, kind, run, b);
   if (rc != RPSF_OK) return rc;
   if (ev_k1) HIP_TRY(hipEventRecord(ev_k1, st));
   if (kind == OV_PLANES && !fused) rc = launch_sum(p, d_out, g, st, b);
@@ -839,6 +916,7 @@
   if (mode == 4 && !p->sweep.ok) return fail(RPSF_E_STATE, "the sweep kernel needs a 16-, 32- or 64-pixel patch on a complete lattice of at least 2 x 2 patches");
   if (mode == 2 && !p->lattice) return fail(RPSF_E_STATE, "colour planes need a regular half-overlap lattice of patch corners");
   if (mode == 3 && !p->patch.direct_ok) return fail(RPSF_E_STATE, "direct overlap-add needs a regular half-overlap lattice and a 128- or 256-pixel patch");
+  if (const int jrc = rpsf_detail_join_lanes(p); jrc != RPSF_OK) return jrc;
   p->overlap_mode = mode;
   rpsf_detail_drop_bands(p);
   return RPSF_OK;
@@ -846,6 +924,7 @@
 
 extern "C" int rpsf_plan_set_option(rpsf_plan* p, int option, int value) {
   if (!p) return fail(RPSF_E_BADARG, "null plan");
+  if (const int rc = rpsf_detail_join_lanes(p); rc != RPSF_OK) return rc;
   switch (option) {
     case RPSF_OPT_PERSIST:
       if (value != 0 && value != 1) return fail(RPSF_E_BADARG, "RPSF_OPT_PERSIST takes 0 or 1");
@@ -883,6 +962,12 @@
       if (value < 0 || value > 65535) return fail(RPSF_E_BADARG, "RPSF_OPT_SAT_GROUP takes 0 (automatic) or 1..65535");
       p->sat_group_opt = value;
       return RPSF_OK;
+    case RPSF_OPT_PIPELINE:
+      if (value != 0 && value != 1) return fail(RPSF_E_BADARG, "RPSF_OPT_PIPELINE takes 0 or 1");
+      if (p->parent) return fail(RPSF_E_STATE, "a view runs on its parent's stream");
+      p->patch.lanes.enabled = value != 0 && p->lane1 != nullptr;
+      if (value != 0) p->patch.lanes.exposed = false;
+      break;
     case RPSF_OPT_DEBUG_ORPHAN:
       if (value < 0) return fail(RPSF_E_BADARG, "RPSF_OPT_DEBUG_ORPHAN takes 0 (off) or a positive modulus");
       p->patch.orphan_mod = value;
@@ -897,6 +982,7 @@
   if (!p || target_regions < 1 || target_regions > (1 << 20)) return fail(RPSF_E_BADARG, "target_regions must be 1..2^20");
   if (!p->sweep.ok) return fail(RPSF_E_STATE, "the sweep kernel needs a 16-, 32- or 64-pixel patch on a complete lattice of at least 2 x 2 patches");
   HIP_TRY(hipSetDevice(p->device));
+  if (const int jrc = rpsf_detail_join_lanes(p); jrc != RPSF_OK) return jrc;
   HIP_TRY(hipStreamSynchronize(p->stream));
   HIP_TRY(hipDeviceSynchronize());
   rpsf_detail_drop_bands(p);
@@ -951,6 +1037,7 @@
   for (int i = 0; i < words; ++i) cus += __builtin_popcount(mask[i]);
   if (cus < 8) return fail(RPSF_E_BADARG, "the mask must leave the plan at least 8 compute units");
   HIP_TRY(hipSetDevice(p->device));
+  if (const int jrc = rpsf_detail_join_lanes(p); jrc != RPSF_OK) return jrc;
   HIP_TRY(hipStreamSynchronize(p->stream));
   rpsf_detail_drop_bands(p);
   hipStream_t masked = nullptr;
@@ -962,6 +1049,12 @@
   (void)hipStreamDestroy(p->stream);
   p->stream = masked;
   p->busy_valid = false;
+  p->patch.lanes.enabled = false;
+  if (p->lane1) {
+    (void)hipStreamSynchronize(p->lane1);
+    (void)hipStreamDestroy(p->lane1);
+    p->lane1 = nullptr;
+  }
   if (p->cu_count > 0) p->patch.round_capacity = p->patch.round_capacity / p->cu_count * cus;
   p->cu_count = cus;
   return RPSF_OK;
@@ -1005,7 +1098,8 @@
   if (rc != RPSF_OK) return rc;
   HIP_TRY(hipSetDevice(p->device));
   hipStream_t st = stream ? reinterpret_cast<hipStream_t>(stream) : p->stream;
-  return rpsf_detail_launch_apply(p, reinterpret_cast<const float*>(image_dev), reinterpret_cast<float*>(out_dev), *geom, st, nullptr);
+  return rpsf_detail_launch_apply(p, reinterpret_cast<const float*>(image_dev), reinterpret_cast<float*>(out_dev), *geom, st, nullptr, nullptr, Batch(),
+                                   stream == nullptr);
 }
 
 
@@ -1049,6 +1143,7 @@
   int rc = check_batch(p, images_dev, outs_dev, n_frames, image_stride, out_stride, geom);
   if (rc != RPSF_OK) return rc;
   HIP_TRY(hipSetDevice(p->device));
+  if (const int jrc = rpsf_detail_join_lanes(p); jrc != RPSF_OK) return jrc;
   hipStream_t st = stream ? reinterpret_cast<hipStream_t>(stream) : p->stream;
   return rpsf_detail_launch_batch(p, reinterpret_cast<const float*>(images_dev), reinterpret_cast<float*>(outs_dev), n_frames,
                       image_stride, out_stride, *geom, st);
@@ -1096,6 +1191,7 @@
   int rc = check_batch(p, images_dev, outs_dev, n_frames, image_stride, out_stride, geom);
   if (rc != RPSF_OK) return rc;
   HIP_TRY(hipSetDevice(p->device));
+  if (const int jrc = rpsf_detail_join_lanes(p); jrc != RPSF_OK) return jrc;
   return timed_loop(p, iters, total_ms, kernel_ms, [&](hipEvent_t k0, hipEvent_t k1) {
     return rpsf_detail_launch_batch(p, reinterpret_cast<const float*>(images_dev), reinterpret_cast<float*>(outs_dev), n_frames, image_stride,
                         out_stride, *geom, p->stream, k0, k1);
@@ -1105,7 +1201,10 @@
 int rpsf_detail_sweep_check(rpsf_plan* p) {
   volatile uint32_t* word = owner(p)->sweep.err;
   if (!word || *word == 0) return RPSF_OK;
+  const uint32_t what = *word;
   *word = 0;
+  if (what == 2)
+    return fail(RPSF_E_HIP, "patch kernel: an apply waited for the tile sums of the plan's previous apply beyond the bound (internal protocol error; the output of this apply is not valid)");
   return fail(RPSF_E_HIP, "sweep kernel: a job waited for the jobs it follows beyond the bound (internal protocol error; the output of this apply is not valid)");
 }
 
@@ -1124,6 +1223,7 @@
   int rc = rpsf_detail_check_geometry(p, geom);
   if (rc != RPSF_OK) return rc;
   HIP_TRY(hipSetDevice(p->device));
+  if (const int jrc = rpsf_detail_join_lanes(p); jrc != RPSF_OK) return jrc;
   return timed_loop(p, iters, total_ms, kernel_ms, [&](hipEvent_t k0, hipEvent_t k1) {
     return rpsf_detail_launch_apply(p, reinterpret_cast<const float*>(image_dev), reinterpret_cast<float*>(out_dev), *geom, p->stream, k0, k1);
   });
@@ -1136,11 +1236,16 @@
   int rc = rpsf_detail_check_geometry(p, geom);
   if (rc != RPSF_OK) return rc;
   HIP_TRY(hipSetDevice(p->device));
+  rc = rpsf_detail_join_lanes(p);
+  if (rc != RPSF_OK) return rc;
   HIP_TRY(hipEventRecord(p->ev[0], p->stream));
   for (int i = 0; i < iters; ++i) {
-    rc = rpsf_detail_launch_apply(p, reinterpret_cast<const float*>(image_dev), reinterpret_cast<float*>(out_dev), *geom, p->stream, nullptr);
+    rc = rpsf_detail_launch_apply(p, reinterpret_cast<const float*>(image_dev), reinterpret_cast<float*>(out_dev), *geom, p->stream, nullptr, nullptr,
+                                  Batch(),  true);
     if (rc != RPSF_OK) return rc;
   }
+  rc = rpsf_detail_join_lanes(p);
+  if (rc != RPSF_OK) return rc;
   HIP_TRY(hipEventRecord(p->ev[3], p->stream));
   HIP_TRY(hipEventSynchronize(p->ev[3]));
   float ms = 0.f;
diff --git a/regularizepsf_amd/csrc/rpsf_device.hpp b/regularizepsf_amd/csrc/rpsf_device.hpp
--- a/regularizepsf_amd/csrc/rpsf_device.hpp
+++ b/regularizepsf_amd/csrc/rpsf_device.hpp
@@ -9,6 +9,7 @@
 #include "rpsf_core2.hpp"
 #include "rpsf_core3.hpp"
 #include "rpsf_plan3.hpp"
+#include "rpsf_lanes.hpp"
 
 using namespace rpsf;
 
diff --git a/regularizepsf_amd/csrc/rpsf_host.hip b/regularizepsf_amd/csrc/rpsf_host.hip
--- a/regularizepsf_amd/csrc/rpsf_host.hip
+++ b/regularizepsf_amd/csrc/rpsf_host.hip
@@ -214,7 +214,7 @@
     pool.run(std::max(1, (frame_workers > 0 ? std::min(frame_workers, pool.width()) : pool.width()) / every), worker, conductor, every);
   }
   if (trace)
-    std::fprintf(stderr, "[rpsf host frame] %zu chunks, %d bands, %zu + %zu pieces: last chunk enqueued %.3f ms, first piece back %.3f, last %.3f, total %.3f ms\\n",
+    std::fprintf(stderr, "[rpsf host frame] %zu chunks, %d bands, %zu + %zu pieces: last chunk enqueued %.3f ms, first piece back %.3f, last %.3f, total %.3f ms\n",
                  chunks.size(), B, n_in, (size_t)out_avail.load(), t_enqueued, t_first_out, t_last_out, ms_since(t_start));
   if (err != hipSuccess) return rpsf_detail_drain_after_error(p, err, "host frame");
   return rpsf_detail_sweep_check(p);
@@ -460,6 +460,8 @@
   int rc = rpsf_detail_check_geometry(p, g);
   if (rc != RPSF_OK) return rc;
   HIP_TRY(hipSetDevice(p->device));
+  if (const int jrc = rpsf_detail_join_lanes(p); jrc != RPSF_OK) return jrc;
+  rpsf_detail_clear_error(p);
   return RPSF_OK;
 }
 
diff --git a/regularizepsf_amd/csrc/rpsf_kernels.hpp b/regularizepsf_amd/csrc/rpsf_kernels.hpp
--- a/regularizepsf_amd/csrc/rpsf_kernels.hpp
+++ b/regularizepsf_amd/csrc/rpsf_kernels.hpp
@@ -21,6 +21,10 @@
   size_t planes_frame_floats, out_frame_floats;
   int frame_major;
   uint32_t n_tiles_listed;
+  uint32_t* summed;
+  uint32_t seq;
+  uint32_t gate_on, gate_want;
+  uint32_t* err;
 };
 __device__ __forceinline__ uint32_t sum_entry(const TileSum& p, uint32_t i) {
   if (p.n_frames <= 1) return p.tiles[i];
@@ -51,8 +55,10 @@
   __builtin_amdgcn_raw_buffer_store_b128(q, r, (int)(float_offset * sizeof(float)), 0, PLANE_AUX_STORE);
 }
 
-template <int UN = 8, bool KNOWN_FUSED = false>
-__device__ __forceinline__ void sum_tile(const TileSum& p0, uint32_t entry_any_lane, int tid, int nthreads, bool known_complete = false) {
+__device__ __forceinline__ void out_store16_wt(__amdgpu_buffer_rsrc_t r, size_t float_offset, rpsf_f4 v) { plane_store16_aux<16 | 2>(r, float_offset, v); }
+
+template <int UN, bool KNOWN_FUSED, bool GATED>
+__device__ __forceinline__ void sum_tile_values(const TileSum& p0, uint32_t entry_any_lane, int tid, int nthreads, bool known_complete) {
   typedef float f4 __attribute__((ext_vector_type(4)));
 #if defined(__HIP_DEVICE_COMPILE__)
   const uint32_t entry = __builtin_amdgcn_readfirstlane(entry_any_lane);
@@ -87,6 +93,11 @@
   const int gw = (x1 - x0) >> 2;
   if (vec) {
     const __amdgpu_buffer_rsrc_t rsrc = plane_rsrc(p.planes);
+    [[maybe_unused]] const __amdgpu_buffer_rsrc_t orsrc = plane_rsrc(GATED ? p.out : p.planes);
+    auto ostore = [&](size_t o, f4 acc) RPSF_AI {
+      if constexpr (GATED) out_store16_wt(orsrc, o, acc);
+      else __builtin_nontemporal_store(acc, reinterpret_cast<f4*>(p.out + o));
+    };
     const int total = gw * (y1 - y0);
     if ((gw & (gw - 1)) == 0) {
       const int sh = 31 - __builtin_clz((unsigned)gw);
@@ -112,7 +123,7 @@
 #pragma unroll
           for (int k = 0; k < 4; ++k)
             if ((cov >> k) & 1) acc += v[u][k];
-          __builtin_nontemporal_store(acc, reinterpret_cast<f4*>(p.out + (size_t)(y0 + row_of(i) - p.row0) * p.ld_out + x0 + (col_of(i) << 2)));
+          ostore((size_t)(y0 + row_of(i) - p.row0) * p.ld_out + x0 + (col_of(i) << 2), acc);
         }
       }
     } else {
@@ -126,7 +137,7 @@
             const size_t o = off + k * p.plane_stride;
             acc += fused ? plane_load16_wt(rsrc, o) : __builtin_nontemporal_load(reinterpret_cast<const f4*>(p.planes + o));
           }
-        __builtin_nontemporal_store(acc, reinterpret_cast<f4*>(p.out + (size_t)(y0 + row - p.row0) * p.ld_out + x0 + (col << 2)));
+        ostore((size_t)(y0 + row - p.row0) * p.ld_out + x0 + (col << 2), acc);
       }
     }
   } else {
@@ -141,17 +152,48 @@
           const float* src = p.planes + k * p.plane_stride + yl * p.ld_planes + x;
           acc += fused ? __uint_as_float(__hip_atomic_load(reinterpret_cast<const unsigned*>(src), __ATOMIC_RELAXED, __HIP_MEMORY_SCOPE_AGENT)) : *src;
         }
-      p.out[yl * p.ld_out + x] = acc;
-    }
+      if constexpr (GATED) __hip_atomic_store(reinterpret_cast<unsigned*>(p.out + yl * p.ld_out + x), __float_as_uint(acc), __ATOMIC_RELAXED, __HIP_MEMORY_SCOPE_AGENT);
+      else p.out[yl * p.ld_out + x] = acc;
+    }
+  }
+}
+template <int UN = 8, bool KNOWN_FUSED = false, bool GATED = false, bool PUBLISH = true>
+__device__ __forceinline__ void sum_tile(const TileSum& p, uint32_t entry_any_lane, int tid, int nthreads, bool known_complete = false) {
+#if defined(__HIP_DEVICE_COMPILE__)
+  if constexpr (GATED) {
+    const uint32_t tile = __builtin_amdgcn_readfirstlane(entry_any_lane) & 0xffffffu;
+    if (p.gate_on && (p.cover[tile] & 15) == 0) {
+      if (tid == 0) {
+        const unsigned long long t0 = __builtin_amdgcn_s_memrealtime();
+        while (!lane_seq_reached(__hip_atomic_load(p.summed + tile, __ATOMIC_RELAXED, __HIP_MEMORY_SCOPE_AGENT), p.gate_want)) {
+          if (__builtin_amdgcn_s_memrealtime() - t0 > 40000000ull) {
+            __hip_atomic_store(p.err, 2u, __ATOMIC_RELAXED, __HIP_MEMORY_SCOPE_SYSTEM);
+            break;
+          }
+          __builtin_amdgcn_s_sleep(8);
+        }
+      }
+      __syncthreads();
+    }
+  }
+#endif
+  sum_tile_values<UN, KNOWN_FUSED, GATED>(p, entry_any_lane, tid, nthreads, known_complete);
+  if constexpr (GATED && PUBLISH) {
+#if defined(__HIP_DEVICE_COMPILE__)
+    asm volatile("s_waitcnt vmcnt(0)" ::: "memory");
+    __syncthreads();
+    if (tid == 0 && p.summed)
+      __hip_atomic_store(p.summed + (__builtin_amdgcn_readfirstlane(entry_any_lane) & 0xffffffu), p.seq, __ATOMIC_RELAXED, __HIP_MEMORY_SCOPE_AGENT);
+#endif
   }
 }
 struct NoSideJob {
   __device__ __forceinline__ bool operator()() const { return false; }
 };
-template <class BETWEEN = NoSideJob, int UN = 8, bool KNOWN_FUSED = false>
+template <class BETWEEN = NoSideJob, int UN = 8, bool KNOWN_FUSED = false, bool GATED = false>
 __device__ __forceinline__ void sum_tiles_worker(const TileSum& p, int block, int nblocks, BETWEEN&& between = BETWEEN()) {
   if (!p.queue) {
-    for (int i = block; i < p.count; i += nblocks) sum_tile<UN, KNOWN_FUSED>(p, p.tiles[i], threadIdx.x, blockDim.x);
+    for (int i = block; i < p.count; i += nblocks) sum_tile<UN, KNOWN_FUSED, GATED>(p, p.tiles[i], threadIdx.x, blockDim.x);
     return;
   }
 #define RPSF_SUM_LOOKAHEAD 4
@@ -161,7 +203,12 @@
   int npend = 0;
   bool exhausted = false;
   bool side_job = true;
+  [[maybe_unused]] uint32_t unpublished = 0xffffffffu;
   for (;;) {
+#if defined(__HIP_DEVICE_COMPILE__)
+    if constexpr (GATED)
+      if (unpublished != 0xffffffffu) asm volatile("s_waitcnt vmcnt(0)" ::: "memory");
+#endif
     if (side_job) side_job = between();
     if (threadIdx.x == 0) {
       uint32_t chosen = 0xffffffffu;
@@ -193,10 +240,16 @@
     }
     __syncthreads();
     const uint32_t tile = pick;
+    if constexpr (GATED) {
+      if (unpublished != 0xffffffffu && threadIdx.x == 0 && p.summed)
+        __hip_atomic_store(p.summed + (unpublished & 0xffffffu), p.seq, __ATOMIC_RELAXED, __HIP_MEMORY_SCOPE_AGENT);
+      unpublished = 0xffffffffu;
+    }
     __syncthreads();
     if (tile == 0xffffffffu) return;
     if (tile == 0xfffffffeu) continue;
-    sum_tile<UN, KNOWN_FUSED>(p, tile, threadIdx.x, blockDim.x, true);
+    sum_tile<UN, KNOWN_FUSED, GATED, false>(p, tile, threadIdx.x, blockDim.x, true);
+    if constexpr (GATED) unpublished = tile;
   }
 }
 
diff --git a/regularizepsf_amd/csrc/rpsf_kernels2.hpp b/regularizepsf_amd/csrc/rpsf_kernels2.hpp
--- a/regularizepsf_amd/csrc/rpsf_kernels2.hpp
+++ b/regularizepsf_amd/csrc/rpsf_kernels2.hpp
@@ -201,6 +201,7 @@
   if constexpr (dev::STAMPS)
     if (threadIdx.x == 0) *reinterpret_cast<unsigned long long*>(reinterpret_cast<cf*>(smem + Launch2<C>::TABLE_FLOATS) + C::BUF_UNITS + 4) = __builtin_amdgcn_s_memrealtime();
   constexpr bool SUM_KNOWN_FUSED = HOT;
+  constexpr bool GATED = HOT && PERSIST && C::SPLIT_ROWS;
   const bool again = PERSIST && ((blockIdx.x >> 30) & 1u);
   if constexpr (dev::STAMPS)
     if (threadIdx.x == 0 && !again) reinterpret_cast<uint32_t*>(smem + 3 * C::N)[Launch2<C>::OT_WORDS - 1] = blockIdx.x;
@@ -256,12 +257,12 @@
       if (!again && blk < p.sum_first) {
         if (p.k_prefetch && p.head_patches == 0) prefetch_first_round_k<C>(p, blk);
         ImagePrefetch<C> prefetch(p, blk, p.prefetch && p.n_frames <= 1);
-        sum_tiles_worker<ImagePrefetch<C>&, 8, SUM_KNOWN_FUSED>(p.ts, 0, 1, prefetch);
+        sum_tiles_worker<ImagePrefetch<C>&, 8, SUM_KNOWN_FUSED, GATED>(p.ts, 0, 1, prefetch);
         prefetch.finish();
         return;
       }
     }
-    sum_tiles_worker<NoSideJob, 8, SUM_KNOWN_FUSED>(p.ts, 0, 1);
+    sum_tiles_worker<NoSideJob, 8, SUM_KNOWN_FUSED, GATED>(p.ts, 0, 1);
     return;
   }
   ImageView im = p.im;
@@ -323,6 +324,10 @@
   constexpr bool EARLY_DRAW = PERSIST && C::SPLIT_ROWS;
   constexpr bool MID_DRAW = PERSIST && !EARLY_DRAW;
   unsigned drawn = 0, qword = 0;
+  [[maybe_unused]] auto gate_tile = [&]() RPSF_AI {
+    const int li = (pr - p.ts.lat_r0) / (N / 2), lj = (pc - p.ts.lat_c0) / (N / 2);
+    return (li + ((tu >> 1) & 1)) * p.ts.ntj + lj + (tu & 1);
+  };
   [[maybe_unused]] auto draw_next = [&]() RPSF_AI {
     if constexpr (PERSIST) {
       if (HOT || p.tile_done) {
@@ -330,6 +335,8 @@
         if (tu == 0 && !head_patch)
           drawn = __hip_atomic_fetch_add(p.xq + (pb & 7) * 32, 1u, __ATOMIC_RELAXED, __HIP_MEMORY_SCOPE_AGENT) - p.xq_base[pb & 7] +
                   (p.head_patches ? (unsigned)(p.sum_first >> 3) : 0u);
+        if constexpr (GATED)
+          if (p.ts.gate_on && (tu & 60) == 4) drawn = __hip_atomic_load(p.ts.summed + gate_tile(), __ATOMIC_RELAXED, __HIP_MEMORY_SCOPE_AGENT);
       }
     }
   };
@@ -462,6 +469,24 @@
       if (tu == 0) *reinterpret_cast<unsigned*>(park) = drawn;
       if (tu < 4) reinterpret_cast<unsigned*>(park)[1 + tu] = (unsigned)frame * p.n_tiles + quad_tile(qword);
     }
+    if constexpr (GATED) {
+      if (p.ts.gate_on) {
+        bool late = (tu & 60) == 4 && !lane_seq_reached(drawn, p.ts.gate_want);
+        if (__builtin_expect(__builtin_amdgcn_ballot_w64(late) != 0, 0)) {
+          const unsigned long long t0 = __builtin_amdgcn_s_memrealtime();
+          const int tile = gate_tile();
+          do {
+            __builtin_amdgcn_s_sleep(8);
+            if (late) late = !lane_seq_reached(__hip_atomic_load(p.ts.summed + tile, __ATOMIC_RELAXED, __HIP_MEMORY_SCOPE_AGENT), p.ts.gate_want);
+            if (__builtin_amdgcn_s_memrealtime() - t0 > 40000000ull) {
+              if (late) __hip_atomic_store(p.ts.err, 2u, __ATOMIC_RELAXED, __HIP_MEMORY_SCOPE_SYSTEM);
+              break;
+            }
+          } while (__builtin_amdgcn_ballot_w64(late) != 0);
+        }
+        asm volatile("" ::: "memory");
+      }
+    }
     store_patch2<C, HOT>(
         t, v, ov, ov, plane, pr, pc, win, nullptr, add, []<int R1, int C1>(const float* a) RPSF_AI { return *reinterpret_cast<const f32x4*>(a); },
         [](const float* a) { return *a; },
diff --git a/regularizepsf_amd/csrc/rpsf_lanes.hpp b/regularizepsf_amd/csrc/rpsf_lanes.hpp
--- /dev/null
+++ b/regularizepsf_amd/csrc/rpsf_lanes.hpp
@@ -0,0 +1,104 @@
+#pragma once
+#include <cstddef>
+#include <cstdint>
+
+namespace rpsf {
+
+constexpr bool lane_seq_reached(uint32_t have, uint32_t want) { return (int32_t)(have - want) >= 0; }
+
+constexpr uint32_t LANE_EPOCH_LIMIT = 1u << 29;
+
+struct LaneRange {
+  uintptr_t lo = 0, hi = 0;
+  bool overlaps(const LaneRange& o) const { return lo < o.hi && o.lo < hi; }
+};
+
+struct LaneLayout {
+  int64_t v[6] = {-1, -1, -1, -1, -1, -1};
+  bool operator==(const LaneLayout& o) const {
+    for (int i = 0; i < 6; ++i)
+      if (v[i] != o.v[i]) return false;
+    return true;
+  }
+};
+
+struct LaneDraws {
+  uint32_t xq[8] = {0, 0, 0, 0, 0, 0, 0, 0};
+  uint32_t sum = 0;
+};
+
+struct LanePick {
+  int lane = 0;
+  bool join = false;
+  bool fork = false;
+  bool wait_fork = false;
+  bool gate = false;
+  uint32_t seq = 0;
+  uint32_t xq_base[8] = {0, 0, 0, 0, 0, 0, 0, 0};
+  uint32_t sum_queue_base = 0;
+};
+
+struct LaneEpoch {
+  uint32_t epoch = 0;
+  bool restart = false;
+};
+
+struct LaneBook {
+  bool enabled = false;
+  bool exposed = false;
+  uint32_t xq_base[2][8] = {{0, 0, 0, 0, 0, 0, 0, 0}, {0, 0, 0, 0, 0, 0, 0, 0}};
+  uint32_t sum_queue_base[2] = {0, 0};
+  uint32_t seq = 0;
+  uint32_t done_epoch = 0;
+  int done_last_frames = 1;
+  int last_lane = -1;
+  bool lane1_busy = false;
+  bool public_dirty = true;
+  bool lane1_forked = false;
+  LaneRange last_img, last_out;
+  LaneLayout last_layout;
+
+  bool join() {
+    const bool due = lane1_busy;
+    lane1_busy = false, last_lane = -1, public_dirty = true;
+    return due;
+  }
+
+  bool epoch_restarts(int frames) const { return frames != done_last_frames || done_epoch + 1 >= LANE_EPOCH_LIMIT; }
+  LaneEpoch next_epoch(int frames) {
+    LaneEpoch e;
+    e.restart = epoch_restarts(frames);
+    done_last_frames = frames;
+    e.epoch = done_epoch = e.restart ? 1 : done_epoch + 1;
+    return e;
+  }
+
+  LanePick begin(bool hot, bool gated_kernel, LaneRange img, LaneRange out, const LaneLayout& layout = LaneLayout()) {
+    LanePick k;
+    const bool pipelined = hot && gated_kernel && enabled && !exposed;
+    if (!pipelined) {
+      k.join = join();
+    } else {
+      if (last_lane >= 0 && (img.overlaps(last_out) || out.overlaps(last_img) || !(layout == last_layout))) k.join = join();
+      k.lane = last_lane < 0 ? 0 : 1 - last_lane;
+      k.gate = last_lane >= 0;
+      if (k.lane == 0 && public_dirty) k.fork = true, public_dirty = false, lane1_forked = false;
+      if (k.lane == 1) {
+        k.wait_fork = !lane1_forked;
+        lane1_forked = true, lane1_busy = true;
+      }
+      last_lane = k.lane, last_img = img, last_out = out, last_layout = layout;
+    }
+    if (gated_kernel) k.seq = ++seq;
+    for (int x = 0; x < 8; ++x) k.xq_base[x] = xq_base[k.lane][x];
+    k.sum_queue_base = sum_queue_base[k.lane];
+    return k;
+  }
+
+  void commit(const LanePick& k, const LaneDraws& draws) {
+    for (int x = 0; x < 8; ++x) xq_base[k.lane][x] += draws.xq[x];
+    sum_queue_base[k.lane] += draws.sum;
+  }
+};
+
+}
diff --git a/regularizepsf_amd/csrc/rpsf_plan.hpp b/regularizepsf_amd/csrc/rpsf_plan.hpp
--- a/regularizepsf_amd/csrc/rpsf_plan.hpp
+++ b/regularizepsf_amd/csrc/rpsf_plan.hpp
@@ -11,6 +11,7 @@
 
 #include "rpsf_device.hpp"
 #include "rpsf_hostpipe.hpp"
+#include "rpsf_lanes.hpp"
 #include "rpsf_lattice.hpp"
 #include "rpsf_saturation.hpp"
 #include "rpsf_side_unit.hpp"
@@ -99,11 +100,10 @@
   bool v2 = false;
   DevBuf<uint32_t> d_tile_done;
   DevBuf<uint32_t> d_sum_order;
-  uint32_t done_epoch = 0;
   size_t done_frames = 1;
-  int done_last_frames = 1;
   DevBuf<uint32_t> d_sum_queue;
-  uint32_t sum_queue_base = 0;
+  LaneBook lanes;
+  DevBuf<uint32_t> d_tile_summed;
   bool no_fuse = false;
   int sum_first = -1;
   bool prefetch = false;
@@ -116,7 +116,6 @@
   bool k_cached = false;
   int reserved_cus = 0;
   DevBuf<uint32_t> d_xq;
-  uint32_t xq_base[8] = {0, 0, 0, 0, 0, 0, 0, 0};
   DevBuf<uint4> d_quads;
   DevBuf<uint8_t> d_tile_info;
   DevBuf<uint32_t> d_flags;
@@ -151,8 +150,13 @@
   bool borrowed_stream = false;
   hipEvent_t ev[4] = {nullptr, nullptr, nullptr, nullptr};
   hipEvent_t ev_busy = nullptr;
+  hipStream_t lane1 = nullptr;
+  hipEvent_t ev_lane = nullptr, ev_fork = nullptr;
   ~PlanStream() {
     if (ev_busy) (void)hipEventDestroy(ev_busy);
+    if (ev_lane) (void)hipEventDestroy(ev_lane);
+    if (ev_fork) (void)hipEventDestroy(ev_fork);
+    if (lane1) (void)hipStreamDestroy(lane1);
     for (auto& e : ev)
       if (e) (void)hipEventDestroy(e);
     if (stream && !borrowed_stream) (void)hipStreamDestroy(stream);
@@ -204,6 +208,7 @@
   ~rpsf_plan() {
     (void)hipSetDevice(device);
     if (stream) (void)hipStreamSynchronize(stream);
+    if (lane1) (void)hipStreamSynchronize(lane1);
     if (ev_view) (void)hipEventDestroy(ev_view);
     bands.clear();
   }
@@ -284,7 +289,9 @@
 RPSF_HIDDEN int rpsf_detail_check_geometry(const rpsf_plan* p, const rpsf_geometry* g);
 RPSF_HIDDEN bool rpsf_detail_lattice_covers_window(const rpsf_plan* p, const rpsf_geometry& g);
 RPSF_HIDDEN int rpsf_detail_launch_apply(rpsf_plan* p, const float* d_img, float* d_out, const rpsf_geometry& g, hipStream_t st,
-                                         hipEvent_t ev_k0, hipEvent_t ev_k1 = nullptr, Batch b = Batch());
+                                         hipEvent_t ev_k0, hipEvent_t ev_k1 = nullptr, Batch b = Batch(), bool may_pipeline = false);
+RPSF_HIDDEN int rpsf_detail_join_lanes(rpsf_plan* p);
+RPSF_HIDDEN void rpsf_detail_clear_error(rpsf_plan* p);
 RPSF_HIDDEN int rpsf_detail_launch_batch(rpsf_plan* p, const float* d_imgs, float* d_outs, int n_frames, size_t im_stride, size_t out_stride,
                                          const rpsf_geometry& g, hipStream_t st, hipEvent_t ev_k0 = nullptr, hipEvent_t ev_k1 = nullptr);
 RPSF_HIDDEN int rpsf_detail_plan_create_impl(rpsf_plan** out, int device, int patch_size, int n_patches, const int32_t* coords_rc, rpsf_plan* parent,
diff --git a/regularizepsf_amd/csrc/rpsf_saturated.hip b/regularizepsf_amd/csrc/rpsf_saturated.hip
--- a/regularizepsf_amd/csrc/rpsf_saturated.hip
+++ b/regularizepsf_amd/csrc/rpsf_saturated.hip
@@ -182,6 +182,8 @@
   if (pad_mode < 0 || pad_mode > RPSF_PAD_WRAP) return fail(RPSF_E_BADARG, "unknown pad mode");
   if (dilation < 1 || neighborhood_width < 0) return fail(RPSF_E_BADARG, "dilation must be >= 1 and the neighbourhood width >= 0 (other values: the NumPy route)");
   if (!p->have_k) return fail(RPSF_E_STATE, "no transfer kernel installed (call rpsf_plan_set_transfer first)");
+  if (const int jrc = rpsf_detail_join_lanes(p); jrc != RPSF_OK) return jrc;
+  rpsf_detail_clear_error(p);
   return RPSF_OK;
 }
 
@@ -517,6 +519,7 @@
   }
   if (rc != RPSF_OK) return rc;
   HIP_TRY(hipSetDevice(p->device));
+  if (const int jrc = rpsf_detail_join_lanes(p); jrc != RPSF_OK) return jrc;
   hipStream_t st = stream ? reinterpret_cast<hipStream_t>(stream) : p->stream;
   const size_t npix = (size_t)H * W, stage_stride = (npix + 3) / 4 * 4;
   const bool staged = !in.direct || !out.direct;
@@ -708,6 +711,8 @@
   const long PH = (long)height + 4L * p->N, PW = (long)width + 4L * p->N;
   if (PH * PW >= ((long)1 << 31)) return fail(RPSF_E_UNSUPPORTED, "padded frame too large for this entry point");
   HIP_TRY(hipSetDevice(p->device));
+  if (const int jrc = rpsf_detail_join_lanes(p); jrc != RPSF_OK) return jrc;
+  rpsf_detail_clear_error(p);
   if (!p->sat_dev) p->sat_dev.reset(rpsf_sat_create());
   SatDevice* sd = p->sat_dev.get();
   const SatCall call{height, width, p->N, pad_mode, dilation, neighborhood_width, threshold, 0, 0, 1};
@@ -777,6 +782,8 @@
                   (size_t)(height - 1) * mask_row_stride + (size_t)(width - 1) * mask_col_stride + 1 > mask_frame_bytes))
     return fail(RPSF_E_BADARG, "mask: the strides do not fit mask_frame_bytes");
   HIP_TRY(hipSetDevice(p->device));
+  if (const int jrc = rpsf_detail_join_lanes(p); jrc != RPSF_OK) return jrc;
+  rpsf_detail_clear_error(p);
   DevBuf<uint8_t> d_masks;
   std::vector<rpsf_view> views((size_t)n_masks);
   if (n_masks) HIP_TRY(d_masks.upload(masks_in_host, mask_frame_bytes * n_masks));
```

After: 96000 Mpixels/s, median of 6. 3.9% higher.
